# openfheorg/openfhe-boolean-circuit-evaluator

Hardware: AMD Instinct MI355X
Metric: encrypted gate-bootstraps/sec (whole node), AES-128 Bristol ckt STD128 GINX (higher is better)
Workload: dtype u32

## Files before the change

include/bce_gpu.h:

```cpp
#ifndef BCE_GPU_H
#define BCE_GPU_H

#include <stdint.h>

#ifdef __cplusplus
extern "C" {
#endif

typedef struct bce_ctx bce_ctx;

enum bce_paramset {
    BCE_TOY = 0, BCE_MEDIUM = 1, BCE_STD128_AP = 2, BCE_STD128_APOPT = 3, BCE_STD128 = 4,
    BCE_STD128_OPT = 5, BCE_STD192 = 6, BCE_STD192_OPT = 7, BCE_STD256 = 8, BCE_STD256_OPT = 9
};
enum bce_method { BCE_AP = 1, BCE_GINX = 2 };
enum bce_op {
    BCE_OR = 0, BCE_AND = 1, BCE_NOR = 2, BCE_NAND = 3, BCE_XOR_FAST = 4, BCE_XNOR_FAST = 5,
    BCE_OP_NOT = 16,
    BCE_OP_REFRESH = 17,
    BCE_OP_COPY = 18
};
enum bce_status {
    BCE_OK = 0, BCE_ERR_ARG = 1, BCE_ERR_NO_DEVICE = 2, BCE_ERR_HIP = 3, BCE_ERR_NO_KEYS = 4,
    BCE_ERR_POOL = 5, BCE_ERR_UNSUPPORTED = 6, BCE_ERR_STATE = 7
};
enum bce_encrypt_mode { BCE_FRESH = 0, BCE_BOOTSTRAPPED = 1 };

enum { BCE_P_n = 0, BCE_P_N, BCE_P_q, BCE_P_Q, BCE_P_qKS, BCE_P_baseKS, BCE_P_dKS, BCE_P_baseG, BCE_P_dG,
       BCE_P_baseR, BCE_P_dR, BCE_P_method, BCE_P_psi, BCE_P_COUNT };

typedef struct bce_gate_desc {
    uint32_t op;
    uint32_t in0;
    uint32_t in1;
    uint32_t out;
    uint32_t neg0;
    uint32_t neg1;
} bce_gate_desc;

#define BCE_PAIR(op, op2) ((uint32_t)(op) | (((uint32_t)(op2) + 1u) << 8))

enum bce_br_kernel {
    BCE_BR_WAVE_PER_TRANSFORM = 0,
    BCE_BR_SPLIT_X1 = 1,
    BCE_BR_SPLIT_X2 = 2,
    BCE_BR_WORD64 = 3,
    BCE_BR_DAG = 4,
    BCE_BR_GRAPH = 5,
    BCE_BR_KERNELS = 6
};

typedef struct bce_timing {
    double   blind_rotate_ms;
    double   tail_ms;
    uint64_t blind_rotate_launches;
    uint64_t bootstraps;
    double   br_ms[BCE_BR_KERNELS];
    uint64_t br_launches[BCE_BR_KERNELS];
    uint64_t br_bootstraps[BCE_BR_KERNELS];
    uint64_t fused_tail_launches;
} bce_timing;

int bce_ctx_create(int paramset, int method, int device, bce_ctx** out);
int bce_ctx_create_custom(uint32_t n, uint32_t N, uint64_t q, uint64_t Q, uint64_t qKS, uint32_t baseKS,
                          uint32_t baseG, uint32_t baseR, int method, int device, bce_ctx** out);
void bce_ctx_destroy(bce_ctx*);
const char* bce_last_error(const bce_ctx*);
int bce_get_params(const bce_ctx*, uint64_t out[BCE_P_COUNT]);

int bce_keygen(bce_ctx*, const uint8_t seed[32]);
int bce_import_keys(bce_ctx*, const int32_t* s, const int32_t* z, const uint64_t* bsk, uint64_t bsk_words,
                    const uint32_t* ksk, uint64_t ksk_words);
int bce_import_keys_eval(bce_ctx*, const int32_t* s, const int32_t* z, const uint64_t* bsk_eval, uint64_t bsk_words,
                         const uint32_t* ksk, uint64_t ksk_words);
int bce_export_bsk_eval(bce_ctx*, uint64_t* bsk_eval);
int bce_import_keys_file(bce_ctx*, const char* path);
int bce_export_keys_file(bce_ctx*, const char* path);
uint64_t bce_bsk_words(const bce_ctx*);
uint64_t bce_ksk_words(const bce_ctx*);
int bce_export_sk(const bce_ctx*, int32_t* s, int32_t* z);
int bce_export_bsk(bce_ctx*, uint64_t* bsk);
int bce_export_ksk(bce_ctx*, uint32_t* ksk);

int bce_pool_reserve(bce_ctx*, uint32_t slots);
uint32_t bce_pool_slots(const bce_ctx*);
int bce_lwe_write(bce_ctx*, const uint32_t* slots, uint32_t count, const uint64_t* cts);
int bce_lwe_read(bce_ctx*, const uint32_t* slots, uint32_t count, uint64_t* cts);

int bce_encrypt_bits(bce_ctx*, const uint8_t* bits, const uint32_t* slots, uint32_t count,
                     uint64_t enc_index_base, int mode);
int bce_set_encrypt_seed(bce_ctx*, const uint8_t seed[32]);
int bce_decrypt_bits(bce_ctx*, const uint32_t* slots, uint32_t count, uint8_t* bits);

int bce_eval_gates(bce_ctx*, uint32_t n_desc, const bce_gate_desc* descs);
int bce_eval_gates_strided(bce_ctx*, uint32_t n_desc, const bce_gate_desc* descs, uint32_t instances,
                           uint32_t slot_stride);
int bce_synchronize(bce_ctx*);

typedef struct bce_plan bce_plan;
int bce_plan_create(bce_ctx*, uint32_t n_steps, const uint32_t* step_sizes, const bce_gate_desc* descs,
                    uint32_t instances, uint32_t slot_stride, uint32_t slot_base, bce_plan** out);
int bce_plan_run_step(bce_ctx*, bce_plan*, uint32_t step);
int bce_plan_run(bce_ctx*, bce_plan*);
void bce_plan_destroy(bce_ctx*, bce_plan*);

enum { BCE_CHECK_LOG_CAP = 4096 };
typedef struct bce_check_report { uint64_t checked, mismatches, repaired; int64_t sum_err; uint64_t sum_sq_err;
                                  uint32_t max_abs_err, log_count; } bce_check_report;
typedef struct bce_check_entry  { uint32_t tag, index, instance, slot; int32_t err; uint8_t got, expect, pad[2]; } bce_check_entry;
int bce_check_slots(bce_ctx*, uint32_t count, const uint32_t* slots, const uint8_t* expect, uint32_t instances,
                    uint32_t slot_stride, int repair, uint32_t tag);
int bce_plan_set_checks(bce_ctx*, bce_plan*, const uint32_t* check_sizes , const uint32_t* slots, int repair);
int bce_plan_set_expected(bce_ctx*, bce_plan*, const uint8_t* expect);
int bce_check_reset(bce_ctx*);
int bce_check_get(bce_ctx*, bce_check_report*, bce_check_entry* log, uint32_t log_cap);

typedef struct bce_dag bce_dag;
int bce_dag_supported(const bce_ctx*);
int bce_dag_create(bce_ctx*, uint32_t n_tasks, const bce_gate_desc* tasks, const uint8_t* prio, bce_dag** out);
int bce_dag_run(bce_ctx*, bce_dag*, uint32_t instances, uint32_t slot_stride, uint32_t slot_base);
void bce_dag_destroy(bce_ctx*, bce_dag*);
int bce_dag_set_checks(bce_ctx*, bce_dag*, uint32_t n_checks, const uint32_t* tasks , int repair);
int bce_dag_set_expected(bce_ctx*, bce_dag*, uint32_t instances, const uint8_t* expect );
int bce_dag_set_limits(bce_ctx*, int workgroups_per_cu, int placement, uint32_t lazy_us, uint32_t stall_ms);
int bce_dag_last_run(bce_ctx*, uint64_t out[7]);
int bce_dag_debug_block_task(bce_dag*, uint32_t t);

int bce_timing_reset(bce_ctx*);
int bce_timing_get(bce_ctx*, bce_timing* out);
int bce_timing_set_events(bce_ctx*, int on);
uint64_t bce_bytes_per_bootstrap(const bce_ctx*);
int bce_bytes_per_bootstrap_parts(const bce_ctx*, uint64_t out[3]);
uint32_t bce_forward_transforms_per_step(const bce_ctx*);
uint32_t bce_forward_units(const bce_ctx*);
uint32_t bce_forward_mfma(const bce_ctx*);
uint32_t bce_lazy_arithmetic(const bce_ctx*);
int bce_forward_mfma_tables(uint64_t Q, uint32_t N, uint32_t gBits, uint32_t dG, uint64_t* psi, uint32_t* M6, uint32_t* C,
                            uint32_t* table, uint32_t* w14, uint64_t* bounds);
int bce_launch_capacity(const bce_ctx*, uint32_t* lone, uint32_t* full);

int bce_rccl_available(void);
int bce_rccl_version(void);
int bce_rccl_unique_id(uint8_t out[128]);
int bce_rccl_init(bce_ctx*, const uint8_t uid[128], int rank, int world);
int bce_rccl_allgather(bce_ctx*, const void* dev_send, void* dev_recv, uint64_t bytes);
int bce_rccl_shutdown(bce_ctx*);
int bce_rccl_comm_info(bce_ctx*, int out[3]);

int bce_debug_eval_stages(bce_ctx*, uint32_t n_desc, const bce_gate_desc* descs, uint64_t* acc,
                          uint64_t* lweN, uint64_t* ks);
int bce_debug_tail(bce_ctx*, uint32_t count, const uint64_t* acc, const uint32_t* out_slots, uint64_t* lweN,
                   uint64_t* ks);
int bce_debug_ntt(bce_ctx*, uint64_t* polys, uint32_t count, int inverse);

#ifdef __cplusplus
}
#endif
#endif
```

openfhe-boolean-circuit-evaluator_amd/__init__.py:

```python
import ctypes as C
import os

import numpy as np

from . import build as _build

_HERE = os.path.dirname(os.path.abspath(__file__))
LIB_PATH = os.path.join(_HERE, "libbce_amd.so")

TOY, MEDIUM, STD128_AP, STD128_APOPT, STD128, STD128_OPT, STD192, STD192_OPT, STD256, STD256_OPT = range(10)
AP, GINX = 1, 2
OR, AND, NOR, NAND, XOR_FAST, XNOR_FAST = range(6)
OP_NOT, OP_REFRESH, OP_COPY = 16, 17, 18


def PAIR(op, op2):
    return int(op) | ((int(op2) + 1) << 8)


FRESH, BOOTSTRAPPED = 0, 1
OK, ERR_ARG, ERR_NO_DEVICE, ERR_HIP, ERR_NO_KEYS, ERR_POOL, ERR_UNSUPPORTED, ERR_STATE = range(8)
P_NAMES = ["n", "N", "q", "Q", "qKS", "baseKS", "dKS", "baseG", "dG", "baseR", "dR", "method", "psi"]

PARAMSET_BY_NAME = {"TOY": TOY, "MEDIUM": MEDIUM, "STD128": STD128, "STD128_OPT": STD128_OPT,
                    "STD192": STD192, "STD192_OPT": STD192_OPT}
METHOD_BY_NAME = {"AP": AP, "GINX": GINX}


class BceError(RuntimeError):
    def __init__(self, code, msg):
        super().__init__("bce status %d: %s" % (code, msg))
        self.code = code


class GateDesc(C.Structure):
    _fields_ = [("op", C.c_uint32), ("in0", C.c_uint32), ("in1", C.c_uint32),
                ("out", C.c_uint32), ("neg0", C.c_uint32), ("neg1", C.c_uint32)]


BR_KERNEL_NAMES = ["k_blind_rotate (one wave per transform)", "k_blind_rotate_lat<4,2> (split transform, 1 workgroup/CU)",
                   "k_blind_rotate_lat<4,4> (split transform, 2 workgroups/CU)", "k_blind_rotate64 (64-bit modulus)",
                   "k_bootstrap_dag (persistent, dependency-driven, tail fused)",
                   "captured step schedule (bce_plan_run: one hipGraph launch, timed as one)"]
BR_KERNELS = len(BR_KERNEL_NAMES)


class Timing(C.Structure):
    _fields_ = [("blind_rotate_ms", C.c_double), ("tail_ms", C.c_double),
                ("blind_rotate_launches", C.c_uint64), ("bootstraps", C.c_uint64),
                ("br_ms", C.c_double * BR_KERNELS), ("br_launches", C.c_uint64 * BR_KERNELS), ("br_bootstraps", C.c_uint64 * BR_KERNELS),
                ("fused_tail_launches", C.c_uint64)]


class CheckReport(C.Structure):
    _fields_ = [("checked", C.c_uint64), ("mismatches", C.c_uint64), ("repaired", C.c_uint64), ("sum_err", C.c_int64),
                ("sum_sq_err", C.c_uint64), ("max_abs_err", C.c_uint32), ("log_count", C.c_uint32)]


class CheckEntry(C.Structure):
    _fields_ = [("tag", C.c_uint32), ("index", C.c_uint32), ("instance", C.c_uint32), ("slot", C.c_uint32),
                ("err", C.c_int32), ("got", C.c_uint8), ("expect", C.c_uint8), ("pad", C.c_uint8 * 2)]


CHECK_LOG_CAP = 4096


def _report_dict(r, q):
    d = {k: int(getattr(r, k)) for k, _ in CheckReport._fields_}
    d["noise_rms"] = (d["sum_sq_err"] / d["checked"]) ** 0.5 if d["checked"] else 0.0
    d["margin"] = q // 8 - d["max_abs_err"]
    return d


ENGINE_SYMBOLS = [
    "bce_ctx_create", "bce_ctx_create_custom", "bce_ctx_destroy", "bce_last_error", "bce_get_params",
    "bce_keygen", "bce_import_keys", "bce_import_keys_eval", "bce_export_bsk_eval", "bce_import_keys_file", "bce_export_keys_file", "bce_bsk_words", "bce_ksk_words", "bce_export_sk", "bce_export_bsk",
    "bce_export_ksk", "bce_pool_reserve", "bce_pool_slots", "bce_lwe_write", "bce_lwe_read",
    "bce_encrypt_bits", "bce_set_encrypt_seed", "bce_decrypt_bits", "bce_eval_gates", "bce_eval_gates_strided", "bce_synchronize",
    "bce_timing_reset", "bce_timing_get", "bce_timing_set_events", "bce_bytes_per_bootstrap", "bce_bytes_per_bootstrap_parts", "bce_forward_transforms_per_step", "bce_forward_units", "bce_forward_mfma", "bce_lazy_arithmetic", "bce_forward_mfma_tables", "bce_launch_capacity", "bce_rccl_available", "bce_rccl_version", "bce_rccl_unique_id", "bce_rccl_init", "bce_rccl_allgather", "bce_rccl_comm_info",
    "bce_rccl_shutdown", "bce_debug_eval_stages", "bce_debug_ntt", "bce_debug_tail",
    "bce_dag_supported", "bce_dag_create", "bce_dag_run", "bce_dag_destroy", "bce_dag_set_limits", "bce_dag_last_run", "bce_dag_debug_block_task",
    "bce_dag_set_checks", "bce_dag_set_expected",
    "bce_plan_create", "bce_plan_run_step", "bce_plan_run", "bce_plan_destroy",
    "bce_check_slots", "bce_plan_set_checks", "bce_plan_set_expected", "bce_check_reset", "bce_check_get",
]

_lib = None


def build(force=False):
    return _build.build(force=force)


def forward_mfma_tables(Q, N=1024, gBits=7, dG=4):
    import numpy as np
    L = lib()
    psi, w14, bounds = C.c_uint64(), (C.c_uint32 * 2)(), (C.c_uint64 * 4)()
    M6, Cw, tab = np.zeros((64, 64), np.uint32), np.zeros(64, np.uint32), np.zeros((4, 4, 64, 4), np.uint32)
    st = int(L.bce_forward_mfma_tables(int(Q), int(N), int(gBits), int(dG), C.byref(psi), M6.ctypes.data, Cw.ctypes.data, tab.ctypes.data,
                                       C.cast(w14, C.c_void_p), C.cast(bounds, C.c_void_p)))
    if st == 0:
        return 0, None
    return st, {"psi": int(psi.value), "M6": M6, "C": Cw, "table": tab, "w14": (int(w14[0]), int(w14[1])),
                "limb_sum_max": int(bounds[0]), "lo_max": int(bounds[1]), "hi_max": int(bounds[2]), "out_max": int(bounds[3])}


def lib():
    global _lib
    if _lib is not None:
        return _lib
    if not os.path.exists(LIB_PATH):
        raise ImportError("libbce_amd.so is not built: run `python -m openfhe-boolean-circuit-evaluator_amd.build` "
                          "or __graft_entry__.build(); there is no fallback path")
    L = C.CDLL(LIB_PATH)
    vp, u32, u64, i32 = C.c_void_p, C.c_uint32, C.c_uint64, C.c_int
    L.bce_ctx_create.argtypes = [i32, i32, i32, C.POINTER(vp)]
    L.bce_ctx_create_custom.argtypes = [u32, u32, u64, u64, u64, u32, u32, u32, i32, i32, C.POINTER(vp)]
    L.bce_ctx_destroy.argtypes = [vp]
    L.bce_ctx_destroy.restype = None
    L.bce_last_error.argtypes = [vp]
    L.bce_last_error.restype = C.c_char_p
    L.bce_get_params.argtypes = [vp, C.POINTER(u64)]
    L.bce_keygen.argtypes = [vp, C.c_char_p]
    L.bce_import_keys.argtypes = [vp, vp, vp, vp, u64, vp, u64]
    L.bce_import_keys_eval.argtypes = [vp, vp, vp, vp, u64, vp, u64]
    L.bce_export_bsk_eval.argtypes = [vp, vp]
    L.bce_import_keys_file.argtypes = [vp, C.c_char_p]
    L.bce_export_keys_file.argtypes = [vp, C.c_char_p]
    L.bce_bsk_words.argtypes = [vp]
    L.bce_bsk_words.restype = u64
    L.bce_ksk_words.argtypes = [vp]
    L.bce_ksk_words.restype = u64
    L.bce_export_sk.argtypes = [vp, vp, vp]
    L.bce_export_bsk.argtypes = [vp, vp]
    L.bce_export_ksk.argtypes = [vp, vp]
    L.bce_pool_reserve.argtypes = [vp, u32]
    L.bce_pool_slots.argtypes = [vp]
    L.bce_pool_slots.restype = u32
    L.bce_lwe_write.argtypes = [vp, vp, u32, vp]
    L.bce_lwe_read.argtypes = [vp, vp, u32, vp]
    L.bce_encrypt_bits.argtypes = [vp, vp, vp, u32, u64, i32]
    L.bce_set_encrypt_seed.argtypes = [vp, C.c_char_p]
    L.bce_decrypt_bits.argtypes = [vp, vp, u32, vp]
    L.bce_eval_gates.argtypes = [vp, u32, vp]
    L.bce_eval_gates_strided.argtypes = [vp, u32, vp, u32, u32]
    L.bce_synchronize.argtypes = [vp]
    L.bce_timing_reset.argtypes = [vp]
    L.bce_timing_get.argtypes = [vp, C.POINTER(Timing)]
    L.bce_timing_set_events.argtypes = [vp, i32]
    L.bce_bytes_per_bootstrap.argtypes = [vp]
    L.bce_bytes_per_bootstrap.restype = u64
    L.bce_bytes_per_bootstrap_parts.argtypes = [vp, C.POINTER(u64)]
    L.bce_forward_transforms_per_step.argtypes = [vp]
    L.bce_forward_transforms_per_step.restype = C.c_uint32
    L.bce_forward_units.argtypes = [vp]
    L.bce_forward_units.restype = C.c_uint32
    L.bce_forward_mfma.argtypes = [vp]
    L.bce_forward_mfma.restype = C.c_uint32
    L.bce_lazy_arithmetic.argtypes = [vp]
    L.bce_lazy_arithmetic.restype = C.c_uint32
    L.bce_forward_mfma_tables.argtypes = [u64, u32, u32, u32, vp, vp, vp, vp, vp, vp]
    L.bce_forward_mfma_tables.restype = i32
    L.bce_launch_capacity.argtypes = [vp, C.POINTER(C.c_uint32), C.POINTER(C.c_uint32)]
    L.bce_rccl_unique_id.argtypes = [C.c_char_p]
    L.bce_rccl_init.argtypes = [vp, C.c_char_p, i32, i32]
    L.bce_rccl_allgather.argtypes = [vp, vp, vp, u64]
    L.bce_rccl_shutdown.argtypes = [vp]
    L.bce_rccl_comm_info.argtypes = [vp, C.POINTER(C.c_int)]
    L.bce_debug_eval_stages.argtypes = [vp, u32, vp, vp, vp, vp]
    L.bce_debug_ntt.argtypes = [vp, vp, u32, i32]
    L.bce_debug_tail.argtypes = [vp, u32, vp, vp, vp, vp]
    L.bce_dag_supported.argtypes = [vp]
    L.bce_dag_create.argtypes = [vp, u32, vp, vp, C.POINTER(vp)]
    L.bce_dag_run.argtypes = [vp, vp, u32, u32, u32]
    L.bce_dag_destroy.argtypes = [vp, vp]
    L.bce_dag_destroy.restype = None
    L.bce_dag_set_limits.argtypes = [vp, i32, i32, u32, u32]
    L.bce_dag_last_run.argtypes = [vp, C.POINTER(u64)]
    L.bce_dag_debug_block_task.argtypes = [vp, u32]
    L.bce_dag_set_checks.argtypes = [vp, vp, u32, vp, i32]
    L.bce_dag_set_expected.argtypes = [vp, vp, u32, vp]
    L.bce_plan_create.argtypes = [vp, u32, vp, vp, u32, u32, u32, C.POINTER(vp)]
    L.bce_plan_run_step.argtypes = [vp, vp, u32]
    L.bce_plan_run.argtypes = [vp, vp]
    L.bce_plan_destroy.argtypes = [vp, vp]
    L.bce_plan_destroy.restype = None
    L.bce_check_slots.argtypes = [vp, u32, vp, vp, u32, u32, i32, u32]
    L.bce_plan_set_checks.argtypes = [vp, vp, vp, vp, i32]
    L.bce_plan_set_expected.argtypes = [vp, vp, vp]
    L.bce_check_reset.argtypes = [vp]
    L.bce_check_get.argtypes = [vp, C.POINTER(CheckReport), C.POINTER(CheckEntry), u32]
    _lib = L
    return L


def _p(a):
    return a.ctypes.data_as(C.c_void_p) if a is not None else None


def seed_bytes(seed):
    if isinstance(seed, (bytes, bytearray)):
        return bytes(seed).ljust(32, b"\0")[:32]
    return int(seed).to_bytes(32, "little")


def make_descs(descs):
    arr = (GateDesc * len(descs))()
    for i, d in enumerate(descs):
        d = tuple(d) + (0,) * (6 - len(d))
        arr[i] = GateDesc(*d)
    return arr


class BinFHEContext:

    def __init__(self, paramset=STD128_OPT, method=GINX, device=0, custom=None):
        self._L = lib()
        h = C.c_void_p()
        if custom is not None:
            rc = self._L.bce_ctx_create_custom(*custom, method, device, C.byref(h))
        else:
            rc = self._L.bce_ctx_create(paramset, method, device, C.byref(h))
        if rc != OK:
            raise BceError(rc, self._L.bce_last_error(None).decode())
        self.h = h
        buf = (C.c_uint64 * len(P_NAMES))()
        self._L.bce_get_params(self.h, buf)
        self.params = dict(zip(P_NAMES, [int(v) for v in buf]))
        self.n, self.N = self.params["n"], self.params["N"]

    def _ck(self, rc):
        if rc != OK:
            raise BceError(rc, self._L.bce_last_error(self.h).decode())

    def close(self):
        if getattr(self, "h", None):
            self._L.bce_ctx_destroy(self.h)
            self.h = None

    def __del__(self):
        try:
            self.close()
        except Exception:
            pass

    def KeyGen(self, seed=None):
        self._ck(self._L.bce_keygen(self.h, None if seed is None else seed_bytes(seed)))

    BTKeyGen = KeyGen

    def import_keys(self, s, z, bsk, ksk):
        s = np.ascontiguousarray(s, dtype=np.int32)
        z = np.ascontiguousarray(z, dtype=np.int32)
        bsk = np.ascontiguousarray(bsk, dtype=np.uint64)
        ksk = np.ascontiguousarray(ksk, dtype=np.uint32)
        self._ck(self._L.bce_import_keys(self.h, _p(s), _p(z), _p(bsk), bsk.size, _p(ksk), ksk.size))

    def import_keys_eval(self, s, z, bsk_eval, ksk):
        s = np.ascontiguousarray(s, dtype=np.int32)
        z = np.ascontiguousarray(z, dtype=np.int32)
        bsk = np.ascontiguousarray(bsk_eval, dtype=np.uint64)
        ksk = np.ascontiguousarray(ksk, dtype=np.uint32)
        self._ck(self._L.bce_import_keys_eval(self.h, _p(s), _p(z), _p(bsk), bsk.size, _p(ksk), ksk.size))

    def export_bsk_eval(self):
        out = np.zeros(self._L.bce_bsk_words(self.h), dtype=np.uint64)
        self._ck(self._L.bce_export_bsk_eval(self.h, _p(out)))
        return out

    def import_keys_file(self, path):
        self._ck(self._L.bce_import_keys_file(self.h, os.fsencode(path)))

    def export_keys_file(self, path):
        self._ck(self._L.bce_export_keys_file(self.h, os.fsencode(path)))

    def export_sk(self):
        s = np.zeros(self.n, dtype=np.int32)
        z = np.zeros(self.N, dtype=np.int32)
        self._ck(self._L.bce_export_sk(self.h, _p(s), _p(z)))
        return s, z

    def export_bsk(self):
        out = np.zeros(self._L.bce_bsk_words(self.h), dtype=np.uint64)
        self._ck(self._L.bce_export_bsk(self.h, _p(out)))
        return out

    def export_ksk(self):
        out = np.zeros(self._L.bce_ksk_words(self.h), dtype=np.uint32)
        self._ck(self._L.bce_export_ksk(self.h, _p(out)))
        return out

    def pool_reserve(self, slots):
        self._ck(self._L.bce_pool_reserve(self.h, int(slots)))

    def lwe_write(self, slots, cts):
        slots = np.ascontiguousarray(slots, dtype=np.uint32)
        cts = np.ascontiguousarray(cts, dtype=np.uint64)
        assert cts.size == slots.size * (self.n + 1)
        self._ck(self._L.bce_lwe_write(self.h, _p(slots), slots.size, _p(cts)))

    def lwe_read(self, slots):
        slots = np.ascontiguousarray(slots, dtype=np.uint32)
        out = np.zeros((slots.size, self.n + 1), dtype=np.uint64)
        self._ck(self._L.bce_lwe_read(self.h, _p(slots), slots.size, _p(out)))
        return out

    def set_encrypt_seed(self, seed):
        self._ck(self._L.bce_set_encrypt_seed(self.h, None if seed is None else seed_bytes(seed)))

    def Encrypt(self, bits, slots, enc_index_base=0, mode=FRESH):
        bits = np.ascontiguousarray(bits, dtype=np.uint8)
        slots = np.ascontiguousarray(slots, dtype=np.uint32)
        assert bits.size == slots.size
        self._ck(self._L.bce_encrypt_bits(self.h, _p(bits), _p(slots), slots.size, int(enc_index_base), mode))

# ... 25 lines not shown
    def timing_set_events(self, on):
        self._ck(self._L.bce_timing_set_events(self.h, int(bool(on))))

    def timing(self):
        t = Timing()
        self._ck(self._L.bce_timing_get(self.h, C.byref(t)))
        return {"blind_rotate_ms": t.blind_rotate_ms, "tail_ms": t.tail_ms,
                "blind_rotate_launches": int(t.blind_rotate_launches), "bootstraps": int(t.bootstraps),
                "fused_tail_launches": int(t.fused_tail_launches),
                "by_kernel": [{"kernel": BR_KERNEL_NAMES[k], "ms": t.br_ms[k], "launches": int(t.br_launches[k]),
                               "bootstraps": int(t.br_bootstraps[k])} for k in range(BR_KERNELS)]}

    def bytes_per_bootstrap(self):
        return int(self._L.bce_bytes_per_bootstrap(self.h))

    def dag_supported(self):
        return bool(self._L.bce_dag_supported(self.h))

    def dag_create(self, tasks, prio=None):
        arr = (GateDesc * len(tasks))()
        for i, t in enumerate(tasks):
            arr[i] = GateDesc(*(tuple(t) + (0, 0))[:6])
        pr = None
        if prio is not None:
            pr = (C.c_uint8 * len(tasks))(*[int(x) for x in prio])
        h = C.c_void_p()
        self._ck(self._L.bce_dag_create(self.h, len(tasks), arr, pr, C.byref(h)))
        return h

    def dag_run(self, dag, instances=1, slot_stride=0, slot_base=0):
        self._ck(self._L.bce_dag_run(self.h, dag, int(instances), int(slot_stride), int(slot_base)))

    def dag_destroy(self, dag):
        self._L.bce_dag_destroy(self.h, dag)

    def dag_set_limits(self, workgroups_per_cu=0, placement=1, lazy_us=20, stall_ms=4000):
        self._ck(self._L.bce_dag_set_limits(self.h, int(workgroups_per_cu), int(placement), int(lazy_us), int(stall_ms)))

    def dag_last_run(self):
        out = (C.c_uint64 * 7)()
        self._ck(self._L.bce_dag_last_run(self.h, out))
        d = {"done": int(out[0]), "lazy_waits": int(out[1]), "abort": int(out[2]), "workgroups_per_cu": int(out[3]),
             "busy_ticks": int(out[4]), "wait_ticks": int(out[5]), "gate_ticks": int(out[6])}
        if out[0]:
            d["ms_per_bootstrap"] = round(out[4] / out[0] / 1e5, 4)
            d["wait_ms_per_bootstrap"] = round(out[5] / out[0] / 1e5, 4)
            d["gate_ms_per_bootstrap"] = round(out[6] / out[0] / 1e5, 4)
        return d

    def plan_create(self, steps, instances=1, slot_stride=0, slot_base=0):
        flat = [t for st in steps for t in st]
        arr = (GateDesc * max(1, len(flat)))()
        for i, t in enumerate(flat):
            arr[i] = GateDesc(*(tuple(t) + (0, 0))[:6])
        sizes = (C.c_uint32 * max(1, len(steps)))(*[len(st) for st in steps])
        h = C.c_void_p()
        self._ck(self._L.bce_plan_create(self.h, len(steps), sizes, arr, int(instances), int(slot_stride), int(slot_base), C.byref(h)))
        return h

    def plan_run_step(self, plan, step):
        self._ck(self._L.bce_plan_run_step(self.h, plan, int(step)))

    def plan_run(self, plan):
        self._ck(self._L.bce_plan_run(self.h, plan))

    def plan_destroy(self, plan):
        self._L.bce_plan_destroy(self.h, plan)

    def check_slots(self, slots, expect, instances=1, slot_stride=0, repair=False, tag=0):
        slots = np.ascontiguousarray(slots, dtype=np.uint32)
        expect = np.ascontiguousarray(expect, dtype=np.uint8)
        assert expect.size == slots.size * int(instances)
        self._ck(self._L.bce_check_slots(self.h, slots.size, _p(slots), _p(expect), int(instances), int(slot_stride), int(bool(repair)), int(tag)))

    def plan_set_checks(self, plan, checks, repair=False):
        sizes = np.array([len(st) for st in checks], dtype=np.uint32)
        slots = np.array([s for st in checks for s in st] or [0], dtype=np.uint32)
        self._ck(self._L.bce_plan_set_checks(self.h, plan, _p(sizes), _p(slots), int(bool(repair))))

    def plan_set_expected(self, plan, expect):
        expect = np.ascontiguousarray(expect, dtype=np.uint8)
        self._ck(self._L.bce_plan_set_expected(self.h, plan, _p(expect)))

    def check_reset(self):
        self._ck(self._L.bce_check_reset(self.h))

    def check_get(self):
        r = CheckReport()
        log = (CheckEntry * CHECK_LOG_CAP)()
        self._ck(self._L.bce_check_get(self.h, C.byref(r), log, CHECK_LOG_CAP))
        keys = ("tag", "index", "instance", "slot", "err", "got", "expect")
        return _report_dict(r, self.params["q"]), [{k: int(getattr(log[i], k)) for k in keys} for i in range(r.log_count)]

    def dag_set_checks(self, dag, tasks, repair=False):
        tasks = np.ascontiguousarray(tasks, dtype=np.uint32).ravel()
        self._ck(self._L.bce_dag_set_checks(self.h, dag, tasks.size, _p(tasks) if tasks.size else None, int(bool(repair))))

    def dag_set_expected(self, dag, expect):
        expect = np.ascontiguousarray(expect, dtype=np.uint8)
        assert expect.ndim == 2
        self._ck(self._L.bce_dag_set_expected(self.h, dag, expect.shape[0], _p(expect)))

    def dag_debug_block_task(self, dag, t):
        self._ck(self._L.bce_dag_debug_block_task(dag, int(t)))

    @staticmethod
    def rccl_available():
        return bool(lib().bce_rccl_available())

    @staticmethod
    def rccl_unique_id():
        buf = C.create_string_buffer(128)
        rc = lib().bce_rccl_unique_id(buf)
        if rc != OK:
            raise BceError(rc, "RCCL is not available (bce_rccl_unique_id)")
        return buf.raw

    def rccl_init(self, uid, rank, world):
        self._ck(self._L.bce_rccl_init(self.h, bytes(uid), int(rank), int(world)))

    def rccl_comm_info(self):
        out = (C.c_int * 3)()
        self._ck(self._L.bce_rccl_comm_info(self.h, out))
        return {"ranks": int(out[0]), "rank": int(out[1]), "device": int(out[2])}

    def rccl_shutdown(self):
        self._ck(self._L.bce_rccl_shutdown(self.h))

    def rccl_allgather(self, dev_send_ptr, dev_recv_ptr, nbytes):
        self._ck(self._L.bce_rccl_allgather(self.h, C.c_void_p(dev_send_ptr), C.c_void_p(dev_recv_ptr), int(nbytes)))

    def bytes_per_bootstrap_parts(self):
        buf = (C.c_uint64 * 3)()
        self._ck(self._L.bce_bytes_per_bootstrap_parts(self.h, buf))
        return {"bsk": int(buf[0]), "ksk": int(buf[1]), "ct": int(buf[2])}

    def is64(self):
        return self.params["Q"] >= (1 << 28)

    def fp64(self):
        return self.is64() and self.params["Q"] < (1 << 39) and os.environ.get("BCE_FP64", "1")[:1] != "0"

    def bsk_word_bytes(self):
        return 8 if self.is64() else 4

    def forward_transforms_per_step(self):
        return int(self._L.bce_forward_transforms_per_step(self.h))

    def forward_units(self):
        return int(self._L.bce_forward_units(self.h))

    def forward_mfma(self):
        return int(self._L.bce_forward_mfma(self.h))

    def lazy_arithmetic(self):
        return int(self._L.bce_lazy_arithmetic(self.h))

    def launch_capacity(self):
        lone, full = C.c_uint32(), C.c_uint32()
        self._ck(self._L.bce_launch_capacity(self.h, C.byref(lone), C.byref(full)))
        return int(lone.value), int(full.value)

    def debug_eval_stages(self, descs):
        arr = make_descs(descs)
        nb = len(arr)
        rows = nb + sum(1 for d in arr if d.op >> 8)
        acc = np.zeros((nb, 2 * self.N), dtype=np.uint64)
        lweN = np.zeros((rows, self.N + 1), dtype=np.uint64)
        ks = np.zeros((rows, self.n + 1), dtype=np.uint64)
        self._ck(self._L.bce_debug_eval_stages(self.h, nb, arr, _p(acc), _p(lweN), _p(ks)))
        return acc, lweN, ks

    def debug_tail(self, acc, out_slots):
        acc = np.ascontiguousarray(acc, dtype=np.uint64).reshape(-1, 2 * self.N)
        slots = np.ascontiguousarray(out_slots, dtype=np.uint32)
        assert slots.size == acc.shape[0]
        lweN = np.zeros((slots.size, self.N + 1), dtype=np.uint64)
        ks = np.zeros((slots.size, self.n + 1), dtype=np.uint64)
        self._ck(self._L.bce_debug_tail(self.h, slots.size, _p(acc), _p(slots), _p(lweN), _p(ks)))
        return lweN, ks

    def debug_ntt(self, polys, inverse=False):
        polys = np.array(polys, dtype=np.uint64, order="C")
        count = polys.size // self.N
        self._ck(self._L.bce_debug_ntt(self.h, _p(polys), count, 1 if inverse else 0))
        return polys


class CircuitInfo(C.Structure):
    _fields_ = [("n_gates", C.c_uint32), ("n_input_gates", C.c_uint32), ("n_wires", C.c_uint32),
                ("n_inputs", C.c_uint32), ("n_input_bits", C.c_uint32 * 2), ("n_output_bits", C.c_uint32),
                ("n_levels", C.c_uint32), ("n_sublaunches", C.c_uint32), ("n_relevel_steps", C.c_uint32),
                ("max_frontier", C.c_uint32), ("slot_stride", C.c_uint32),
                ("n_bootstraps", C.c_uint64)]


class CircuitStats(C.Structure):
    _fields_ = [("total_ms", C.c_double), ("management_ms", C.c_double), ("execution_ms", C.c_double),
                ("bootstraps", C.c_uint64), ("levels", C.c_uint32), ("sublaunches", C.c_uint32),
                ("verify_fixes", C.c_uint32), ("exchanges", C.c_uint32), ("exchanged_cts", C.c_uint64)]


ALLGATHER_FN = C.CFUNCTYPE(C.c_int, C.c_void_p, C.c_uint64, C.c_int)

CIRCUIT_SYMBOLS = [
    "bce_circuit_create", "bce_circuit_destroy", "bce_circuit_last_error", "bce_circuit_read_file",
    "bce_circuit_read_bristol", "bce_circuit_get_info", "bce_circuit_reset", "bce_circuit_rearm", "bce_circuit_set_plaintext",
    "bce_circuit_set_encrypted", "bce_circuit_set_verify", "bce_circuit_get_flags", "bce_circuit_set_batched",
    "bce_circuit_set_encrypt_mode", "bce_circuit_get_encrypt_mode", "bce_circuit_plan_hash", "bce_circuit_set_shard_locality", "bce_circuit_set_xor_fast", "bce_circuit_set_xor_shared", "bce_circuit_xor_shared_active", "bce_circuit_set_relevel", "bce_circuit_get_relevel", "bce_circuit_set_dataflow", "bce_circuit_dataflow_active", "bce_circuit_set_graph", "bce_circuit_graph_active", "bce_circuit_set_device_verify", "bce_circuit_device_verify_active", "bce_circuit_get_check_report", "bce_circuit_dataflow_plan", "bce_circuit_set_balance", "bce_circuit_relevel_steps", "bce_circuit_relevel_descs", "bce_circuit_relevel_publications", "bce_circuit_check_relevel", "bce_circuit_set_instances", "bce_circuit_set_input", "bce_circuit_clock",
    "bce_circuit_get_output", "bce_circuit_get_buses", "bce_circuit_get_counts", "bce_circuit_get_stats", "bce_circuit_dump",
    "bce_circuit_set_exchange", "bce_circuit_enable_rccl", "bce_circuit_exchange_capacity", "bce_assemble_bristol", "bce_pool_gather",
    "bce_pool_scatter",
]

_circ_bound = False


def _bind_circuit():
    global _circ_bound
    L = lib()
    if _circ_bound:
        return L
    vp, u32, u64, i32 = C.c_void_p, C.c_uint32, C.c_uint64, C.c_int
    L.bce_circuit_create.argtypes = [vp, C.POINTER(vp)]
    L.bce_circuit_destroy.argtypes = [vp]
    L.bce_circuit_destroy.restype = None
    L.bce_circuit_last_error.argtypes = [vp]
    L.bce_circuit_last_error.restype = C.c_char_p
    L.bce_circuit_read_file.argtypes = [vp, C.c_char_p]
    L.bce_circuit_read_bristol.argtypes = [vp, C.c_char_p, i32]
    L.bce_circuit_get_info.argtypes = [vp, C.POINTER(CircuitInfo)]
    for name in ("reset", "rearm", "clock"):
        getattr(L, "bce_circuit_" + name).argtypes = [vp]
    for name in ("set_plaintext", "set_encrypted", "set_verify", "set_batched", "set_encrypt_mode", "set_xor_fast", "set_xor_shared", "set_relevel", "dump"):
        getattr(L, "bce_circuit_" + name).argtypes = [vp, i32]
    L.bce_circuit_get_flags.argtypes = [vp, C.POINTER(i32), C.POINTER(i32), C.POINTER(i32)]
    L.bce_circuit_set_instances.argtypes = [vp, u32]
    L.bce_circuit_set_balance.argtypes = [vp, i32, u32, u32]
    L.bce_circuit_set_dataflow.argtypes = [vp, i32]
    L.bce_circuit_set_graph.argtypes = [vp, i32]
    L.bce_circuit_graph_active.argtypes = [vp]
    L.bce_circuit_set_device_verify.argtypes = [vp, i32]
    L.bce_circuit_device_verify_active.argtypes = [vp]
    L.bce_circuit_get_check_report.argtypes = [vp, C.POINTER(CheckReport)]
    L.bce_circuit_get_encrypt_mode.argtypes = [vp]
    L.bce_circuit_get_relevel.argtypes = [vp]
    L.bce_circuit_set_shard_locality.argtypes = [vp, i32]
    L.bce_circuit_plan_hash.argtypes = [vp]
    L.bce_circuit_plan_hash.restype = u64
    L.bce_circuit_dataflow_active.argtypes = [vp]
    L.bce_circuit_xor_shared_active.argtypes = [vp]
    L.bce_circuit_dataflow_plan.argtypes = [vp, vp, vp, u32, C.POINTER(u32)]
    L.bce_circuit_relevel_steps.argtypes = [vp, C.POINTER(u32), u32, C.POINTER(u32)]
    L.bce_circuit_relevel_descs.argtypes = [vp, vp, u32, C.POINTER(u32)]
    L.bce_circuit_relevel_publications.argtypes = [vp, C.POINTER(u32), u32, C.POINTER(u32)]
    L.bce_circuit_check_relevel.argtypes = [vp]
    L.bce_circuit_set_input.argtypes = [vp, u32, vp, u32, vp]
    L.bce_circuit_get_output.argtypes = [vp, u32, vp]
    L.bce_circuit_get_buses.argtypes = [vp, C.POINTER(u32), C.POINTER(u32), u32, C.POINTER(u32), C.POINTER(u32), u32]
    L.bce_circuit_get_counts.argtypes = [vp, C.POINTER(u32 * 6)]
    L.bce_circuit_get_stats.argtypes = [vp, C.POINTER(CircuitStats)]
    L.bce_circuit_set_exchange.argtypes = [vp, u32, u32, i32, ALLGATHER_FN, vp, vp, vp, vp, vp, u64]
    L.bce_circuit_enable_rccl.argtypes = [vp, i32]
    L.bce_circuit_exchange_capacity.argtypes = [vp, u32, i32, i32]
    L.bce_circuit_exchange_capacity.restype = u64
    L.bce_assemble_bristol.argtypes = [C.c_char_p, i32, i32, i32, C.c_char_p, C.c_char_p, u32]
    L.bce_pool_gather.argtypes = [vp, vp, u32, vp]
    L.bce_pool_scatter.argtypes = [vp, vp, u32, vp]
    _circ_bound = True
    return L


def assemble_bristol(in_path, out_path=None, new_flag=False, gen_fan_flag=False, debug_flag=False):
    L = _bind_circuit()
    err = C.create_string_buffer(512)
    rc = L.bce_assemble_bristol(in_path.encode(), int(new_flag), int(gen_fan_flag), int(debug_flag),
                                out_path.encode() if out_path else None, err, 512)
    if rc != OK:
        raise BceError(rc, err.value.decode())


def HexStr2UintVec(inhex):
    out = []
    for ch in reversed(inhex):
        v = int(ch, 16)
        out.extend([(v >> b) & 1 for b in range(4)])
    return out


def BinStr2UintVec(inbin):
    return [int(ch) for ch in reversed(inbin)]


class Circuit:

    def __init__(self, cc=None):
        self._L = _bind_circuit()
        self.cc = cc
        h = C.c_void_p()
        rc = self._L.bce_circuit_create(cc.h if cc is not None else None, C.byref(h))
        if rc != OK:
            raise BceError(rc, "bce_circuit_create failed")
        self.h = h
        self._keep = []

    def _ck(self, rc):
# ... 215 lines not shown
```

openfhe-boolean-circuit-evaluator_amd/csrc/engine.cpp:

```cpp
#include <hip/hip_runtime_api.h>
#include <sys/random.h>

#include <algorithm>
#include <cstdarg>
#include <cstdio>
#include <cstdlib>
#include <cstring>
#include <memory>
#include <mutex>
#include <unordered_set>
#include <string>
#include <vector>

#include "../../include/bce_circuit.h"
#include "../../include/bce_gpu.h"
#include "devmem.hpp"
#include "fwd_mfma.hpp"
#include "host_math.hpp"
#include "kernels.hpp"
#include "keygen.hpp"
#include "prng.hpp"

using namespace bce;

static_assert(sizeof(bce_check_report) == 48 && sizeof(bce_check_entry) == 24, "layout of the check structs (include/bce_gpu.h; the kernel writes them)");

namespace {

thread_local std::string g_create_error;

struct ParamRow { u32 bits, cyclo, n; u64 q, qKS; u32 baseKS, baseG, baseR; };
const ParamRow kParamTable[] = {
    {27, 1024, 64, 512, 0, 25, 1u << 9, 23},
    {28, 2048, 422, 1024, 1u << 14, 1u << 7, 1u << 10, 32},
    {27, 2048, 512, 1024, 1u << 14, 1u << 7, 1u << 9, 32},
    {27, 2048, 502, 1024, 1u << 14, 1u << 7, 1u << 9, 32},
    {27, 2048, 512, 1024, 1u << 14, 1u << 7, 1u << 7, 32},
    {27, 2048, 502, 1024, 1u << 14, 1u << 7, 1u << 7, 32},
    {37, 4096, 1024, 1024, 1u << 19, 28, 1u << 13, 32},
    {37, 4096, 805, 1024, 1u << 15, 32, 1u << 13, 32},
    {29, 4096, 1024, 2048, 1u << 14, 1u << 7, 1u << 8, 46},
    {29, 4096, 990, 2048, 1u << 14, 1u << 7, 1u << 8, 46},
};

struct EventPair { hipEvent_t a, b; int kind; };

bool os_entropy(uint8_t out[32]) {
    size_t got = 0;
    while (got < 32) {
        const ssize_t r = getrandom(out + got, 32 - got, 0);
        if (r <= 0) break;
        got += (size_t)r;
    }
    if (got == 32) return true;
    FILE* f = std::fopen("/dev/urandom", "rb");
    if (!f) return false;
    const size_t n = std::fread(out, 1, 32, f);
    std::fclose(f);
    return n == 32;
}

}

struct bce_plan;
struct bce_dag;
namespace {
std::mutex g_live_mu;
std::unordered_set<const bce_ctx*> g_live;
}

struct bce_ctx {
    std::unordered_set<bce_plan*> plans;
    std::unordered_set<bce_dag*> dags;
    u32 n = 0, N = 0, logN = 0;
    u64 q = 0, Q = 0, qKS = 0, psi = 0;
    u32 baseKS = 0, dKS = 0, baseG = 0, gBits = 0, dG = 0, baseR = 0, dR = 0;
    int method = 0, device = 0;
    std::string err;

    hipStream_t stream = nullptr;
    DevParams P{};
    DevBuf<uint2> d_twf;
    DevBuf<u32> d_fwd_mfma, d_psi, d_psi_r2, d_xcd_gate;
    DevBuf<char> d_bsk;
    DevBuf<ulonglong2> d_tw64;
    DevBuf<double2> d_tw64d;
    bool is64 = false;
    size_t wbytes = 4;
    DevBuf<char> d_ksk;
    u64 bsk_polys = 0;
    bool have_keys = false;
    std::vector<int32_t> s, z;
    uint8_t seed[32] = {0};
    uint8_t enc_seed[32] = {0};
    bool enc_seed_ok = false, enc_deterministic = false;
    uint64_t enc_counter = 0;
    void* rccl_comm = nullptr;
    DevBuf<u32> d_pool;
    u32 pool_slots = 0;
    DevBuf<char> d_acc;
    DevBuf<u64> d_tail_partial;
    bool events_on = true;
    DevBuf<u32> d_io;
    DevBuf<u32, true> h_io;
    static constexpr int kRing = 4;
    StagedUpload ring[kRing];
    int ring_pos = 0;
    DevBuf<int8_t> d_s8;
    DevBuf<char> d_check_mem;
    bce_check_report* d_check() const { return reinterpret_cast<bce_check_report*>(d_check_mem.get()); }
    bce_check_entry* d_check_log() const { return reinterpret_cast<bce_check_entry*>(d_check_mem.get() + sizeof(bce_check_report)); }
    StagedUpload chk_stage;
    std::vector<EventPair> pending, free_events;
    bce_timing timing{};
    DevBuf<DevParams> d_P;
    int dag_wg_per_cu = 0, dag_placement = 1;
    uint32_t dag_lazy_us = 20, dag_stall_ms = 4000;
    struct DagStatus { uint32_t abort, done, lazy_waits, pad; uint64_t busy_ticks, wait_ticks, gate_ticks; };
    static constexpr int kDagRuns = 32;
    DevBuf<DagStatus, true> h_dag_status;
    struct DagStage { DevParams P; DagParams D; };
    DevBuf<DagStage, true> h_dag_stage;
    uint64_t dag_expected[kDagRuns] = {0};
    int dag_wps_used[kDagRuns] = {0};
    int dag_pending = 0;
    uint64_t dag_last[7] = {0, 0, 0, 0, 0, 0, 0};

    int fail(int code, const char* fmt, ...) {
        char buf[512];
        va_list ap;
        va_start(ap, fmt);
        vsnprintf(buf, sizeof buf, fmt, ap);
        va_end(ap);
        err = buf;
        return code;
    }
};

#define HIP_TRY(ctx, call)                                                                      \
    do {                                                                                        \
        hipError_t e_ = (call);                                                                 \
        if (e_ != hipSuccess) return (ctx)->fail(BCE_ERR_HIP, "%s: %s", #call, hipGetErrorString(e_)); \
    } while (0)

namespace {

bool env_off(const char* name) {
    const char* e = std::getenv(name);
    return e && e[0] == '0';
}

struct HostTables {
    std::vector<uint2> twf;
    std::vector<u32> psi, psi_r2;
    std::vector<ulonglong2> tw64;
    std::vector<double2> tw64d;
    FwdMfmaTables fwd;
    bool xcd_gate = false;
};

int derive_ctx(bce_ctx* c, u32 n, u32 N, u64 q, u64 Q, u64 qKS, u32 baseKS, u32 baseG, u32 baseR, int method, int device, u32 cu_count,
               HostTables& T) {
    c->n = n; c->N = N; c->q = q; c->Q = Q; c->qKS = qKS ? qKS : Q;
    c->baseKS = baseKS; c->baseG = baseG; c->baseR = baseR; c->method = method; c->device = device;
    while ((1u << c->logN) < N) ++c->logN;
    while ((1u << c->gBits) < baseG) ++c->gBits;
    c->dKS = digit_count((double)c->qKS, (double)baseKS);
    c->dG = digit_count((double)Q, (double)baseG);
    c->dR = digit_count((double)q, (double)baseR);
    c->is64 = Q >= (1ull << 28);
    c->wbytes = c->is64 ? 8 : 4;

    DevParams& P = c->P;
    P.n = n; P.N = N; P.logN = c->logN; P.q = (u32)q; P.Q = (u32)Q; P.qKS = (u32)c->qKS;
    P.baseKS = baseKS; P.dKS = c->dKS;
    P.ksk_stride = (n + 1 + 63) & ~63u;
    P.ksk_u16 = c->qKS <= 65536 ? 1 : 0;
    P.gBits = c->gBits; P.dG = c->dG; P.baseR = baseR; P.dR = c->dR;
    P.method_ap = method == BCE_AP ? 1 : 0;
    P.factor = (u32)(2 * N / q);
    P.factor_even = (P.factor & 1u) ? 0 : 1;
    P.Q8p1 = (u32)(Q / 8 + 1);
    int bq = bit_length(Q);
    P.red_shift = (u32)std::max(2 * bq + 3 - 32, 0);
    P.red_mu = c->is64 ? 0 : (u32)((((u128)1) << (32 + P.red_shift)) / Q);
    u64 ninv = pow_mod(N, Q - 2, Q);
    P.Ninv = (u32)ninv;
    P.Ninv_s = c->is64 ? 0 : (u32)(((u128)ninv << 32) / Q);
    P.mu32 = (u32)((((u64)1) << 32) / Q);
    P.c32 = (u32)((((u64)1) << 32) % Q);
    {
        const u128 B = 2 * c->logN + 2, R = 2 * c->dG;
        const u128 sum = R * B * Q * Q;
        const bool ok1 = B * Q < ((u128)1 << 32);
        const bool ok2 = sum < ((u128)1 << 64);
        const u128 folded = (sum >> 32) * P.c32 + ((u128)1 << 32);
        const bool ok3 = folded < ((u128)1 << (32 + P.red_shift));
        const bool ok4 = (u128)6 * Q * Q + 2 * Q < ((u128)1 << (32 + P.red_shift)) && (u128)3 * Q < ((u128)1 << 32);
        const u128 rmax = (sum >> 32) + 1 + Q, ymax = 2 * rmax * 2 * Q;
        const bool ok5 = ymax < ((u128)1 << 64) && (ymax >> 32) + 1 + Q <= 2 * (u128)Q && (u128)4 * Q < ((u128)1 << 32);
        P.lazy = (c->is64 || (ok1 && ok2 && ok3 && ok4 && ok5)) ? 1 : 0;
    }
    P.is64 = c->is64 ? 1 : 0;
    P.Q64 = Q;
    {
        const char* var = std::getenv("BCE_VARIANT");
        P.variant = var ? (u32)std::atoi(var) : 0;
        P.cu_count = cu_count;
        P.fuse_tail = env_off("BCE_FUSE_TAIL") ? 0 : 1;
    }
    const char* occ = std::getenv("BCE_OCCUPANCY");
    P.occupancy_target = (occ && occ[0] == '2') ? 2 : 3;
    P.fp64 = (c->is64 && Q < (1ull << 39) && !env_off("BCE_FP64")) ? 1 : 0;
    const KernelClass kc = kernel_class(P);
    P.occupancy_target = kc.occupancy_target;
    P.fp64 = kc.fp64;
    if (kc.error) { g_create_error = kc.error; return BCE_ERR_UNSUPPORTED; }
    if (c->qKS > 0xFFFFFFFFull) { g_create_error = "qKS must fit 32 bits"; return BCE_ERR_UNSUPPORTED; }
    c->psi = min_primitive_root(Q, 2ull * N);

    T.twf.resize(N);
    T.psi.resize(N);
    u64 p = 1;
    for (u32 i = 0; i < N; ++i) {
        T.psi[i] = c->is64 ? 0 : (u32)p;
        u32 r = bit_reverse(i, (int)c->logN);
        u32 pos = r;
        if (r >= 64) {
            const u32 s = 31u - (u32)__builtin_clz(r), sh = s - 6, ii = r - (1u << s);
            pos = (1u << s) + ((ii & ((1u << sh) - 1u)) << 6) + (ii >> sh);
        }
        T.twf[pos] = c->is64 ? make_uint2(0, 0) : make_uint2((u32)p, (u32)(((u128)p << 32) / Q));
        p = mul_mod(p, c->psi, Q);
    }
    const u64 r2modq = c->is64 ? 0 : (u64)((((u128)1) << 64) % Q);
    T.psi_r2.resize(N);
    for (u32 i = 0; i < N; ++i) T.psi_r2[i] = c->is64 ? 0 : (u32)mul_mod(T.psi[i], r2modq, Q);
    {
        const u64 ch = (((u64)1) << 32) / c->qKS;
        if (ch < 8) { g_create_error = "qKS too large for the key-switch gather (needs qKS <= 2^29)"; return BCE_ERR_ARG; }
        P.ks_chunk = (u32)std::min<u64>(ch & ~(u64)7, 1u << 20);
    }
    if (!c->is64) {
        u32 inv = (u32)Q;
        for (int i = 0; i < 5; ++i) inv *= 2u - (u32)Q * inv;
        P.qinv_neg = 0u - inv;
        P.r2_off = (u32)(Q - r2modq);
    }
    {
        u64 I = pow_mod(c->psi, N / 2, Q), v = 1;
        for (int k = 0; k < 4; ++k) {
            P.I4[k] = (u32)v;
            P.I4s[k] = c->is64 ? 0 : (u32)(((u128)v << 32) / Q);
            v = mul_mod(v, I, Q);
        }
        const u64 wl = mul_mod(P.I4[3], ninv, Q);
        P.Winv_last = (u32)wl;
        P.Winv_last_s = c->is64 ? 0 : (u32)(((u128)wl << 32) / Q);
    }
    P.xcd_gate_ticks = 10000;
    T.xcd_gate = !c->is64 && !env_off("BCE_XCD_GATE");
    if (const char* t = std::getenv("BCE_XCD_GATE_US"); t && T.xcd_gate) P.xcd_gate_ticks = (u32)std::atoi(t) * 100u;
    P.Q8p1_64 = Q / 8 + 1;
    P.mu64 = (u64)((((u128)1) << 64) / Q);
    P.c64 = (u64)((((u128)1) << 64) % Q);
    P.Ninv64 = ninv;
    P.Ninv64_s = (u64)(((u128)ninv << 64) / Q);
    if (c->is64) {
        T.tw64.resize(N);
        u64 pw = 1;
        for (u32 i = 0; i < N; ++i) {
            T.tw64[bit_reverse(i, (int)c->logN)] = make_ulonglong2(pw, (u64)(((u128)pw << 64) / Q));
            pw = mul_mod(pw, c->psi, Q);
        }
        if (kc.lds_error) { g_create_error = kc.lds_error; return BCE_ERR_UNSUPPORTED; }
        P.Qd = (double)Q;
        P.invQd = 1.0 / (double)Q;
        P.Ninvd = (double)ninv;
        P.Ninvd_q = (double)ninv / (double)Q;
        T.tw64d.resize(N);
        for (u32 i = 0; i < N; ++i) T.tw64d[i] = make_double2((double)T.tw64[i].x, (double)T.tw64[i].x / (double)Q);
    }
    {
        const u128 Bg = (u128)1 << c->gBits;
        u128 span = 0, pw = 1;
        for (u32 l = 0; l < c->dG; ++l) { span += pw; pw *= Bg; }
        const u128 hi = (Bg / 2 - 1) * span, lo = (Bg / 2) * span;
        const bool exact = (u128)(Q >> 1) <= hi + 1 && (u128)(Q - (Q >> 1)) <= lo;
        const bool product_exact = kc.family != KernelFamily::Fp64 || (Bg / 2) * (u128)Q < ((u128)1 << 53);
        P.fold = (exact && kc.fold_build && product_exact && !env_off("BCE_FOLD")) ? 1 : 0;
        P.fold_ninv = (P.fold && kc.family == KernelFamily::Fp64) ? 1 : 0;
        P.fwd_units = (P.fold && !c->is64 && c->method == BCE_GINX && P.factor_even && !env_off("BCE_FWD_UNITS")) ? 1 : 0;
        P.fwd_mfma = 0; P.w14 = P.w14s = 0;
        if (P.fwd_units && !env_off("BCE_FWD_MFMA")) {
            T.fwd = build_fwd_mfma_tables(Q, N, c->gBits, c->dG, c->psi);
            if (T.fwd.ok) { P.fwd_mfma = 1; P.w14 = T.fwd.w14; P.w14s = T.fwd.w14s; }
        }
    }
    P.pool_stride = n + 1;
    return BCE_OK;
}

template <class T>
hipError_t upload_vector(DevBuf<T>& dst, const std::vector<T>& v) {
    const hipError_t e = dst.alloc(std::max<size_t>(1, v.size()));
    return e != hipSuccess ? e : hipMemcpy(dst.get(), v.data(), v.size() * sizeof(T), hipMemcpyHostToDevice);
}

int upload_ctx(bce_ctx* c, const HostTables& T) {
    DevParams& P = c->P;
    if (hipSetDevice(c->device) != hipSuccess) { g_create_error = "hipSetDevice failed"; return BCE_ERR_HIP; }
    if (hipStreamCreateWithFlags(&c->stream, hipStreamNonBlocking) != hipSuccess) { g_create_error = "hipStreamCreate failed"; return BCE_ERR_HIP; }
    const auto up = [](auto& dst, const auto& v, const char* what) -> bool {
        if (upload_vector(dst, v) == hipSuccess) return true;
        g_create_error = std::string("hipMalloc(") + what + ") failed";
        return false;
    };
    if (!up(c->d_twf, T.twf, "twiddles") || !up(c->d_psi, T.psi, "psi table") || !up(c->d_psi_r2, T.psi_r2, "psi table")) return BCE_ERR_HIP;
    P.tw_f = c->d_twf.get();
    P.psi_tab = c->d_psi.get();
    P.psi_tab_r2 = c->d_psi_r2.get();
    P.xcd_gate = nullptr;
    if (T.xcd_gate) {
        if (c->d_xcd_gate.alloc(16 * 32) != hipSuccess) { g_create_error = "hipMalloc(xcd gate) failed"; return BCE_ERR_HIP; }
        P.xcd_gate = c->d_xcd_gate.get();
    }
    if (c->is64) {
        if (!up(c->d_tw64, T.tw64, "twiddles64") || !up(c->d_tw64d, T.tw64d, "twiddles64d")) return BCE_ERR_HIP;
        P.tw64 = c->d_tw64.get();
        P.tw64d = c->d_tw64d.get();
    }
    P.fwd_mfma_tab = nullptr;
    if (P.fwd_mfma) {
        if (!up(c->d_fwd_mfma, T.fwd.table, "forward matrix table")) return BCE_ERR_HIP;
        P.fwd_mfma_tab = c->d_fwd_mfma.get();
    }
    c->enc_seed_ok = os_entropy(c->enc_seed);
    return BCE_OK;
}

int build_ctx(u32 n, u32 N, u64 q, u64 Q, u64 qKS, u32 baseKS, u32 baseG, u32 baseR, int method, int device,
              bce_ctx** out) {
    if (!out) return BCE_ERR_ARG;
    *out = nullptr;
    if (method != BCE_AP && method != BCE_GINX) { g_create_error = "bad method (expect AP=1 or GINX=2)"; return BCE_ERR_ARG; }
    if (N < 512 || N > 2048 || (N & (N - 1))) { g_create_error = "ring dimension N must be 512, 1024 or 2048"; return BCE_ERR_UNSUPPORTED; }
    if ((q & (q - 1)) || q > 2 * (u64)N || q < 8) { g_create_error = "LWE modulus q must be a power of two dividing 2N"; return BCE_ERR_ARG; }
    if (!is_prime_u64(Q) || (Q - 1) % (2ull * N)) { g_create_error = "Q must be a prime = 1 mod 2N"; return BCE_ERR_ARG; }
    if (Q >= (1ull << 40)) { g_create_error = "ring modulus Q must be below 2^40"; return BCE_ERR_UNSUPPORTED; }
    if (baseG & (baseG - 1)) { g_create_error = "gadget base must be a power of two"; return BCE_ERR_ARG; }
    int ndev = 0;
    if (hipGetDeviceCount(&ndev) != hipSuccess || ndev <= 0) {
        g_create_error = "no HIP device visible: the engine has no CPU fallback";
        return BCE_ERR_NO_DEVICE;
    }
    if (device < 0 || device >= ndev) { g_create_error = "bad device ordinal"; return BCE_ERR_ARG; }
    int cus = 0;
    if (hipDeviceGetAttribute(&cus, hipDeviceAttributeMultiprocessorCount, device) != hipSuccess || cus <= 0) cus = 256;

    struct CtxDeleter { void operator()(bce_ctx* p) const { bce_ctx_destroy(p); } };
    std::unique_ptr<bce_ctx, CtxDeleter> c(new bce_ctx);
    { std::lock_guard<std::mutex> lk(g_live_mu); g_live.insert(c.get()); }
    HostTables T;
    int rc = derive_ctx(c.get(), n, N, q, Q, qKS, baseKS, baseG, baseR, method, device, (u32)cus, T);
    if (rc == BCE_OK) rc = upload_ctx(c.get(), T);
    if (rc != BCE_OK) return rc;
    *out = c.release();
    return BCE_OK;
}

u64 rgsw_rows_total(const bce_ctx* c);
int bsk_words_to_kernel_layout(bce_ctx* c) {
    if (c->P.fold) HIP_TRY(c, launch_fold_gadget(c->P, c->d_bsk.get(), rgsw_rows_total(c) / (2ull * c->dG), +1, c->stream));
    if (!c->P.fp64) { HIP_TRY(c, hipStreamSynchronize(c->stream)); return BCE_OK; }
    HIP_TRY(c, launch_words_u64_f64(reinterpret_cast<u64*>(c->d_bsk.get()), (size_t)c->bsk_polys * c->N, 1, c->stream));
    HIP_TRY(c, hipStreamSynchronize(c->stream));
    return BCE_OK;
}

u64 rgsw_rows_total(const bce_ctx* c) {
    const u64 R = 2ull * c->dG;
    return c->method == BCE_GINX ? (u64)c->n * 2 * R : (u64)c->n * c->baseR * c->dR * R;
}

int alloc_keys(bce_ctx* c) {
    if (!c->d_bsk.get()) {
        c->bsk_polys = rgsw_rows_total(c) * 2;
        HIP_TRY(c, c->d_bsk.alloc(c->wbytes * c->bsk_polys * c->N));
    }
    if (!c->d_ksk.get()) {
        size_t rows = (size_t)c->N * c->baseKS * c->dKS;
        HIP_TRY(c, c->d_ksk.alloc(rows * c->P.ksk_stride * (c->P.ksk_u16 ? 2 : 4)));
    }
    c->P.bsk = reinterpret_cast<const u32*>(c->d_bsk.get());
    c->P.bsk64 = reinterpret_cast<const u64*>(c->d_bsk.get());
    c->P.ksk = c->d_ksk.get();
    return BCE_OK;
}

int upload_ksk(bce_ctx* c, const u32* ksk) {
    const size_t rows = (size_t)c->N * c->baseKS * c->dKS, W = c->n + 1, S = c->P.ksk_stride;
    if (c->P.ksk_u16) {
        std::vector<uint16_t> buf(rows * S, 0);
        for (size_t r = 0; r < rows; ++r)
            for (size_t k = 0; k < W; ++k) buf[r * S + k] = (uint16_t)ksk[r * W + k];
        HIP_TRY(c, hipMemcpy(c->d_ksk.get(), buf.data(), buf.size() * 2, hipMemcpyHostToDevice));
    } else {
        std::vector<u32> buf(rows * S, 0);
        for (size_t r = 0; r < rows; ++r) std::memcpy(&buf[r * S], &ksk[r * W], W * 4);
        HIP_TRY(c, hipMemcpy(c->d_ksk.get(), buf.data(), buf.size() * 4, hipMemcpyHostToDevice));
    }
    return BCE_OK;
}

int upload_secret(bce_ctx* c) {
    const size_t padded = ((size_t)c->n + 63) / 64 * 64;
    std::vector<int8_t> s8(padded, 0);
    for (u32 k = 0; k < c->n; ++k) s8[k] = (int8_t)c->s[k];
    if (!c->d_s8.get()) HIP_TRY(c, c->d_s8.alloc(padded));
    HIP_TRY(c, hipStreamSynchronize(c->stream));
    HIP_TRY(c, hipMemcpy(c->d_s8.get(), s8.data(), padded, hipMemcpyHostToDevice));
    return BCE_OK;
}

int ensure_check(bce_ctx* c) {
    if (c->d_check_mem.get()) return BCE_OK;
    const size_t bytes = sizeof(bce_check_report) + (size_t)kCheckLogCap * sizeof(bce_check_entry);
    DevBuf<char> mem;
    HIP_TRY(c, mem.alloc(bytes));
    if (hipMemset(mem.get(), 0, bytes) != hipSuccess) return c->fail(BCE_ERR_HIP, "hipMemset(check report) failed");
    c->d_check_mem = std::move(mem);
    return BCE_OK;
}

int ensure_acc(bce_ctx* c, size_t boots) {
    const size_t need = boots * 2 * c->N * c->wbytes;
    HIP_TRY(c, c->d_acc.grow(need, std::max(need, 2 * c->d_acc.capacity()), c->stream));
    return BCE_OK;
}

int stage_descs(bce_ctx* c, const bce_gate_desc* d, size_t n, StagedUpload** slot) {
    StagedUpload& r = c->ring[c->ring_pos];
    c->ring_pos = (c->ring_pos + 1) % bce_ctx::kRing;
    const size_t bytes = n * sizeof(bce_gate_desc);
    HIP_TRY(c, r.reserve(bytes, std::max(n, (size_t)1024) * sizeof(bce_gate_desc), nullptr));
    std::memcpy(r.host(), d, bytes);
    HIP_TRY(c, r.copy(bytes, c->stream));
    *slot = &r;
    return BCE_OK;
}
const bce_gate_desc* descs_of(const StagedUpload* slot) { return static_cast<const bce_gate_desc*>(slot->device()); }

EventPair get_events(bce_ctx* c, int kind) {
    EventPair p;
    if (!c->free_events.empty()) {
        p = c->free_events.back();
        c->free_events.pop_back();
    } else {
        hipEventCreate(&p.a);
        hipEventCreate(&p.b);
    }
    p.kind = kind;
    return p;
}

void drain_timing(bce_ctx* c) {
    for (auto& p : c->pending) {
        float ms = 0.f;
        if (hipEventElapsedTime(&ms, p.a, p.b) == hipSuccess) {
            if (p.kind < BCE_BR_KERNELS) { c->timing.blind_rotate_ms += ms; c->timing.br_ms[p.kind] += ms; }
            else c->timing.tail_ms += ms;
        }
        c->free_events.push_back(p);
    }
    c->pending.clear();
}
int drain_if_long(bce_ctx* c) {
    if (c->pending.size() <= 4096) return BCE_OK;
    HIP_TRY(c, hipStreamSynchronize(c->stream));
    drain_timing(c);
    return BCE_OK;
}

int words_to_device(bce_ctx* c, void* dev, const u64* src, size_t words, bool wide) {
    if (wide) {
        HIP_TRY(c, hipMemcpy(dev, src, words * 8, hipMemcpyHostToDevice));
    } else {
        const std::vector<u32> tmp(src, src + words);
// ... 955 lines not shown
        if (two) { p1[i] = writer[g.in1]; read_before[g.in1] = 1; }
        if (p1[i] == p0[i]) p1[i] = -1;
        if (writer[g.out] >= 0) return c->fail(BCE_ERR_ARG, "bce_dag_create: slot %u is written by tasks %d and %u (SSA form required)", g.out, writer[g.out], i);
        if (read_before[g.out]) return c->fail(BCE_ERR_ARG, "bce_dag_create: task %u writes slot %u that an earlier task (or itself) reads", i, g.out);
        writer[g.out] = (int32_t)i;
        for (int32_t p : {p0[i], p1[i]})
            if (p >= 0) { ++dep[i]; ++cons_cnt[p + 1]; lvl[i] = std::max(lvl[i], lvl[p] + 1); }
        depth = std::max(depth, lvl[i]);
    }
    std::vector<u32> cons_off(cons_cnt);
    for (u32 i = 0; i < n_tasks; ++i) cons_off[i + 1] += cons_off[i];
    std::vector<u32> cons(std::max<u32>(1, cons_off[n_tasks])), fill(cons_off.begin(), cons_off.end() - 1);
    for (u32 i = 0; i < n_tasks; ++i)
        for (int32_t p : {p0[i], p1[i]}) if (p >= 0) cons[fill[p]++] = i;
    std::vector<uint8_t> qid(n_tasks, 0);
    if (prio) qid.assign(prio, prio + n_tasks);

    struct Deleter { bce_ctx* c; void operator()(bce_dag* g) const { bce_dag_destroy(c, g); } };
    std::unique_ptr<bce_dag, Deleter> g(new bce_dag, Deleter{c});
    { std::lock_guard<std::mutex> lk(g_live_mu); c->dags.insert(g.get()); }
    g->n_tasks = n_tasks; g->max_slot = max_slot; g->depth = depth; g->h_dep_init = dep;
    for (u32 q = 0; q < kDagQueues; ++q) {
        g->init_off[q] = (u32)g->init_items.size();
        for (u32 i = 0; i < n_tasks; ++i) {
            if (qid[i] != q) continue;
            ++g->qcount[q];
            if (dep[i] == 0) g->init_items.push_back(i);
        }
    }
    g->init_off[kDagQueues] = (u32)g->init_items.size();
    if (g->init_items.empty()) return c->fail(BCE_ERR_ARG, "bce_dag_create: no task is ready at the start");
    HIP_TRY(c, g->d_tasks.alloc(n_tasks));
    HIP_TRY(c, hipMemcpy(g->d_tasks.get(), tasks, (size_t)n_tasks * sizeof(bce_gate_desc), hipMemcpyHostToDevice));
    HIP_TRY(c, upload_vector(g->d_cons_off, cons_off));
    HIP_TRY(c, upload_vector(g->d_cons, cons));
    HIP_TRY(c, upload_vector(g->d_dep_init, dep));
    HIP_TRY(c, upload_vector(g->d_init, g->init_items));
    HIP_TRY(c, upload_vector(g->d_qid, qid));
    HIP_TRY(c, g->d_ctl.alloc(kDagCtlWords));
    HIP_TRY(c, g->d_params.alloc(1));
    *out = g.release();
    return BCE_OK;
}

int bce_dag_debug_block_task(bce_dag* g, uint32_t t) {
    if (!g || t >= g->n_tasks) return BCE_ERR_ARG;
    g->h_dep_init[t] += 1;
    return hipMemcpy(g->d_dep_init.get(), g->h_dep_init.data(), (size_t)g->n_tasks * sizeof(u32), hipMemcpyHostToDevice) == hipSuccess ? BCE_OK : BCE_ERR_HIP;
}

int bce_dag_run(bce_ctx* c, bce_dag* g, uint32_t instances, uint32_t slot_stride, uint32_t slot_base) {
    if (!c || !g) return BCE_ERR_ARG;
    if (instances == 0) return BCE_OK;
    if (!c->have_keys) return c->fail(BCE_ERR_NO_KEYS, "bce_keygen / bce_import_keys has not been called");
    if (g->n_checks && g->expect_instances == 0) return c->fail(BCE_ERR_STATE, "bce_dag_run: the DAG has checks but bce_dag_set_expected has not been called");
    if (g->n_checks && g->expect_instances != instances) return c->fail(BCE_ERR_STATE, "bce_dag_run: %u instances, but the expected bits were set for %u", instances, g->expect_instances);
    if (instances > 1 && slot_stride <= g->max_slot) return c->fail(BCE_ERR_ARG, "bce_dag_run: slot_stride %u does not cover the DAG's slots (0..%u)", slot_stride, g->max_slot);
    if ((u64)slot_base + g->max_slot + (u64)(instances - 1) * slot_stride >= c->pool_slots) return c->fail(BCE_ERR_POOL, "bce_dag_run: slot %llu outside the pool (%u slots)", (unsigned long long)((u64)slot_base + g->max_slot + (u64)(instances - 1) * slot_stride), c->pool_slots);
    const u64 items = (u64)g->n_tasks * instances;
    if (items >= 0xFFFFFFF0ull) return c->fail(BCE_ERR_ARG, "bce_dag_run: %llu bootstraps exceed one run's 32-bit item space", (unsigned long long)items);
    HIP_TRY(c, hipSetDevice(c->device));
    if (c->dag_pending >= bce_ctx::kDagRuns) { const int rc = sync_stream(c); if (rc) return rc; }
    if (!c->d_P.get()) HIP_TRY(c, c->d_P.alloc(1));
    if (!c->h_dag_status.get()) HIP_TRY(c, c->h_dag_status.alloc(bce_ctx::kDagRuns));
    if (!c->h_dag_stage.get()) HIP_TRY(c, c->h_dag_stage.alloc(bce_ctx::kDagRuns));
    HIP_TRY(c, g->d_dep.grow(items, items, c->stream));
    DagParams D{};
    for (u32 q = 0; q < kDagQueues; ++q) {
        const size_t need = (size_t)g->qcount[q] * instances;
        HIP_TRY(c, g->d_slots[q].grow(need, need, c->stream));
        D.slots[q] = g->d_slots[q].get();
        D.qcap[q] = (u32)need;
        D.init_off[q] = g->init_off[q];
    }
    D.init_off[kDagQueues] = g->init_off[kDagQueues];
    D.tasks = g->d_tasks.get(); D.cons_off = g->d_cons_off.get(); D.cons = g->d_cons.get(); D.qid = g->d_qid.get(); D.dep_init = g->d_dep_init.get();
    D.dep = g->d_dep.get(); D.init_items = g->d_init.get(); D.ctl = g->d_ctl.get();
    D.n_tasks = g->n_tasks; D.instances = instances; D.slot_stride = slot_stride; D.slot_base = slot_base;
    if (g->n_checks) {
        if (const int rc = ensure_check(c)) return rc;
        D.chk_of_task = g->d_chk_of_task.get(); D.expect = static_cast<const uint8_t*>(g->expect.device()); D.n_checks = g->n_checks; D.repair = (u32)g->chk_repair;
        D.s8 = c->d_s8.get(); D.report = c->d_check(); D.log = c->d_check_log();
    }
    D.lazy_ticks = c->dag_lazy_us * 100u;
    D.stall_ticks = c->dag_stall_ms * 100000u;
    D.policy = c->dag_placement ? 1u : 0u;
    D.gate_ticks = 15000;
    D.gate_backlog = 8;
    if (const char* e = std::getenv("BCE_DAG_GATE_US")) D.gate_ticks = (u32)std::atoi(e) * 100u;
    if (const char* e = std::getenv("BCE_DAG_GATE_BACKLOG")) D.gate_backlog = (u32)std::atoi(e);
    int wps = c->dag_wg_per_cu == 1 ? 2 : 4;
    if (c->dag_wg_per_cu == 0) {
        const double D = (double)std::max<u32>(1, g->depth), W = (double)items, cus = (double)std::max<u32>(1, c->P.cu_count);
        const double t1 = std::max(D, W / cus), t2 = std::max(1.6 * D, W / (1.26 * cus));
        wps = t1 <= t2 ? 2 : 4;
    }
    if (const char* e = std::getenv("BCE_DAG_WPS")) { if (e[0] == '2') wps = 2; else if (e[0] == '4') wps = 4; }
    if (kernel_class(c->P).wg_per_cu_full == 1) wps = 2;
    if (const char* e = std::getenv("BCE_DAG_PLACE")) D.policy = e[0] == '0' ? 0u : 1u;
    const char* dbg = std::getenv("BCE_DAG_DEBUG");
    if (dbg && dbg[0] == 'd') D.policy |= 2u;
    { const char* e = std::getenv("BCE_DAG_GATE"); if (e ? e[0] != '0' : wps == 4) D.policy |= 4u; }
    { const char* e = std::getenv("BCE_DAG_TICKETS"); if (e && e[0] == '1') D.policy |= 8u; }
    const u32 grid = c->P.cu_count * (wps == 2 ? 1u : 2u);
    const int slot = c->dag_pending++;
    bce_ctx::DagStage& stage = c->h_dag_stage.get()[slot];
    stage.P = c->P;
    stage.D = D;
    HIP_TRY(c, hipMemcpyAsync(c->d_P.get(), &stage.P, sizeof(DevParams), hipMemcpyHostToDevice, c->stream));
    HIP_TRY(c, hipMemcpyAsync(g->d_params.get(), &stage.D, sizeof(DagParams), hipMemcpyHostToDevice, c->stream));
    HIP_TRY(c, launch_dag_rearm(D, c->stream));
    EventPair e0 = get_events(c, BCE_BR_DAG);
    hipEventRecord(e0.a, c->stream);
    if (!(dbg && dbg[0] == 'r')) HIP_TRY(c, launch_bootstrap_dag(c->P, c->d_P.get(), g->d_params.get(), wps, grid, c->stream));
    hipEventRecord(e0.b, c->stream);
    c->pending.push_back(e0);
    c->dag_expected[slot] = items;
    c->dag_wps_used[slot] = wps;
    HIP_TRY(c, hipMemcpyAsync(&c->h_dag_status.get()[slot], g->d_ctl.get() + kDagAbort, sizeof(bce_ctx::DagStatus), hipMemcpyDeviceToHost, c->stream));
    c->timing.br_launches[BCE_BR_DAG] += 1;
    c->timing.br_bootstraps[BCE_BR_DAG] += items;
    c->timing.blind_rotate_launches += 1;
    c->timing.fused_tail_launches += 1;
    c->timing.bootstraps += items;
    return BCE_OK;
}

int bce_timing_reset(bce_ctx* c) {
    if (!c) return BCE_ERR_ARG;
    HIP_TRY(c, hipStreamSynchronize(c->stream));
    drain_timing(c);
    c->timing = bce_timing{};
    return BCE_OK;
}

int bce_timing_set_events(bce_ctx* c, int on) {
    if (!c) return BCE_ERR_ARG;
    c->events_on = on != 0;
    return BCE_OK;
}

int bce_timing_get(bce_ctx* c, bce_timing* out) {
    if (!c || !out) return BCE_ERR_ARG;
    const int rc = sync_stream(c);
    drain_timing(c);
    *out = c->timing;
    return rc;
}

uint32_t bce_forward_transforms_per_step(const bce_ctx* c) { return c ? 2 * c->dG - (c->P.fold ? 2 : 0) : 0; }
uint32_t bce_forward_units(const bce_ctx* c) { return c ? c->P.fwd_units : 0; }
uint32_t bce_forward_mfma(const bce_ctx* c) { return c ? c->P.fwd_mfma : 0; }
uint32_t bce_lazy_arithmetic(const bce_ctx* c) { return c ? c->P.lazy : 0; }
int bce_forward_mfma_tables(uint64_t Q, uint32_t N, uint32_t gBits, uint32_t dG, uint64_t* psi, uint32_t* M6, uint32_t* C, uint32_t* table,
                            uint32_t* w14, uint64_t* bounds) {
    const FwdMfmaTables T = build_fwd_mfma_tables(Q, N, gBits, dG);
    if (T.M6.empty()) return 0;
    if (psi) *psi = T.psi;
    if (M6) std::copy(T.M6.begin(), T.M6.end(), M6);
    if (C) std::copy(T.C.begin(), T.C.end(), C);
    if (table) std::copy(T.table.begin(), T.table.end(), table);
    if (w14) { w14[0] = T.w14; w14[1] = T.w14s; }
    if (bounds) { bounds[0] = T.limb_sum_max; bounds[1] = T.lo_max; bounds[2] = T.hi_max; bounds[3] = T.out_max; }
    return T.ok ? 1 : -1;
}

int bce_launch_capacity(const bce_ctx* c, uint32_t* lone, uint32_t* full) {
    if (!c || !lone || !full) return BCE_ERR_ARG;
    const KernelClass k = kernel_class(c->P);
    *lone = c->P.cu_count * k.wg_per_cu_lone;
    *full = c->P.cu_count * k.wg_per_cu_full;
    return BCE_OK;
}

int bce_bytes_per_bootstrap_parts(const bce_ctx* c, uint64_t out[3]) {
    if (!c || !out) return BCE_ERR_ARG;
    const double rgsws = c->method == BCE_AP ? (double)c->n * c->dR * (c->baseR - 1) / c->baseR : 2.0 * c->n;
    out[0] = (u64)((double)c->wbytes * rgsws * (2 * c->dG) * 2 * c->N);
    out[1] = (c->P.ksk_u16 ? 2ull : 4ull) * c->N * c->dKS * (c->n + 1);
    out[2] = 4ull * 3 * (c->n + 1);
    return BCE_OK;
}

uint64_t bce_bytes_per_bootstrap(const bce_ctx* c) {
    uint64_t parts[3];
    return bce_bytes_per_bootstrap_parts(c, parts) == BCE_OK ? parts[0] + parts[1] + parts[2] : 0;
}

int bce_debug_eval_stages(bce_ctx* c, uint32_t n_desc, const bce_gate_desc* descs, uint64_t* acc, uint64_t* lweN,
                          uint64_t* ks) {
    if (!c) return BCE_ERR_ARG;
    for (u32 i = 0; i < n_desc; ++i)
        if (!(pair_kind(descs[i].op) > 0 || descs[i].op <= BCE_XNOR_FAST || descs[i].op == BCE_OP_REFRESH)) return c->fail(BCE_ERR_ARG, "staged outputs need bootstrapped ops only");
    return eval_impl(c, n_desc, descs, 1, 0, acc, lweN, ks);
}

int bce_debug_tail(bce_ctx* c, uint32_t count, const uint64_t* acc, const uint32_t* out_slots, uint64_t* lweN, uint64_t* ks) {
    if (!c || !acc || !out_slots) return BCE_ERR_ARG;
    if (count == 0) return BCE_OK;
    if (!c->have_keys) return c->fail(BCE_ERR_NO_KEYS, "bce_keygen / bce_import_keys has not been called");
    HIP_TRY(c, hipSetDevice(c->device));
    const size_t words = (size_t)count * 2 * c->N;
    for (size_t i = 0; i < words; ++i)
        if (acc[i] >= c->Q) return c->fail(BCE_ERR_ARG, "accumulator word not reduced mod Q");
    std::vector<bce_gate_desc> d(count);
    for (u32 i = 0; i < count; ++i) {
        if (out_slots[i] >= c->pool_slots) return c->fail(BCE_ERR_POOL, "slot %u outside the pool", out_slots[i]);
        d[i] = bce_gate_desc{BCE_AND, out_slots[i], out_slots[i], out_slots[i], 0, 0};
    }
    DevBuf<char> d_in;
    DevBuf<u32> d_lweN, d_ks;
    DevBuf<u64> d_partial;
    HIP_TRY(c, d_in.alloc(words * c->wbytes));
    HIP_TRY(c, d_lweN.alloc((size_t)count * (c->N + 1)));
    HIP_TRY(c, d_ks.alloc((size_t)count * (c->n + 1)));
    HIP_TRY(c, d_partial.alloc(std::max<size_t>(1, tail_partial_words(c->P, count))));
    int rc = words_to_device(c, d_in.get(), acc, words, c->is64);
    if (rc) return rc;
    StagedUpload* slot = nullptr;
    if ((rc = stage_descs(c, d.data(), count, &slot))) return rc;
    HIP_TRY(c, launch_tail(c->P, descs_of(slot), count, 1, 0, d_in.get(), d_partial.get(), d_lweN.get(), d_ks.get(), c->stream, LaunchEvents{}));
    slot->mark(c->stream);
    HIP_TRY(c, hipStreamSynchronize(c->stream));
    if (lweN && (rc = words_from_device(c, lweN, d_lweN.get(), (size_t)count * (c->N + 1), false))) return rc;
    if (ks && (rc = words_from_device(c, ks, d_ks.get(), (size_t)count * (c->n + 1), false))) return rc;
    return BCE_OK;
}

static int pool_pack(bce_ctx* c, const uint32_t* slots, uint32_t count, void* dev, int to_pool) {
    if (!c || !slots || !dev) return BCE_ERR_ARG;
    if (count == 0) return BCE_OK;
    HIP_TRY(c, hipSetDevice(c->device));
    std::vector<bce_gate_desc> d(count);
    for (u32 i = 0; i < count; ++i) {
        if (slots[i] >= c->pool_slots) return c->fail(BCE_ERR_POOL, "slot %u outside the pool", slots[i]);
        d[i] = bce_gate_desc{BCE_OP_COPY, slots[i], slots[i], slots[i], 0, 0};
    }
    StagedUpload* slot = nullptr;
    int rc = stage_descs(c, d.data(), count, &slot);
    if (rc) return rc;
    HIP_TRY(c, launch_pool_pack(c->P, descs_of(slot), count, (u32*)dev, to_pool, c->stream));
    slot->mark(c->stream);
    return BCE_OK;
}

int bce_pool_gather(bce_ctx* c, const uint32_t* slots, uint32_t count, void* dev_dst) {
    return pool_pack(c, slots, count, dev_dst, 0);
}
int bce_pool_scatter(bce_ctx* c, const uint32_t* slots, uint32_t count, const void* dev_src) {
    return pool_pack(c, slots, count, const_cast<void*>(dev_src), 1);
}

int bce_debug_ntt(bce_ctx* c, uint64_t* polys, uint32_t count, int inverse) {
    if (!c || !polys) return BCE_ERR_ARG;
    HIP_TRY(c, hipSetDevice(c->device));
    const size_t words = (size_t)count * c->N;
    for (size_t i = 0; i < words; ++i)
        if (polys[i] >= c->Q) return c->fail(BCE_ERR_ARG, "poly word not reduced mod Q");
    DevBuf<char> d;
    HIP_TRY(c, d.alloc(words * c->wbytes));
    int rc = words_to_device(c, d.get(), polys, words, c->is64);
    if (!rc) rc = dev_ntt(c, d.get(), count, inverse);
    if (rc) return rc;
    HIP_TRY(c, hipStreamSynchronize(c->stream));
    return words_from_device(c, polys, d.get(), words, c->is64);
}

}
```

openfhe-boolean-circuit-evaluator_amd/csrc/fwd_mfma.hpp:

```cpp
#pragma once
#include <cstdint>
#include <vector>

#include "host_math.hpp"

namespace bce {

constexpr u32 kFwdMfmaLoads = 4;
constexpr u32 kFwdMfmaTableWords = 4 * kFwdMfmaLoads * 64 * 4;

inline u32 fwd_mfma_h_of_k(u32 k) { return (k >> 2) + 16u * (k & 3u); }

struct FwdMfmaTables {
    bool ok = false;
    u64 psi = 0;
    std::vector<u32> M6;
    std::vector<u32> C;
    std::vector<u32> table;
    u32 w14 = 0, w14s = 0;
    u64 limb_sum_max = 0;
    u64 lo_max = 0, hi_max = 0, out_max = 0;
};

inline FwdMfmaTables build_fwd_mfma_tables(u64 Q, u32 N, u32 gBits, u32 dG, u64 psi = 0) {
    FwdMfmaTables T;
    if (N != 1024 || dG != 4 || gBits == 0 || gBits > 7 || Q >= (1ull << 28) || Q < 3 || (Q - 1) % (2ull * N) != 0) return T;
    T.psi = psi ? psi : min_primitive_root(Q, 2ull * N);
    if (pow_mod(T.psi, N, Q) != Q - 1) return T;
    std::vector<u64> tw(64, 0);
    for (u32 i = 0; i < 64; ++i) tw[i] = pow_mod(T.psi, bit_reverse(i, 10), Q);
    T.M6.assign(64 * 64, 0);
    for (u32 e = 0; e < 64; ++e) {
        u64 x[64] = {0};
        x[e] = 1;
        for (int B = 5; B >= 0; --B) {
            const u32 m = 1u << (5 - B);
            for (u32 h = 0; h < 64; ++h) {
                if (h & (1u << B)) continue;
                const u64 w = tw[m + (h >> (B + 1))];
                const u64 X = x[h], Tm = mul_mod(x[h | (1u << B)], w, Q);
                x[h] = (X + Tm) % Q;
                x[h | (1u << B)] = (X + Q - Tm) % Q;
            }
        }
        for (u32 h = 0; h < 64; ++h) T.M6[h * 64 + e] = (u32)x[h];
    }
    T.C.assign(64, 0);
    for (u32 hp = 0; hp < 64; ++hp) {
        u64 s = 0;
        for (u32 h = 0; h < 64; ++h) s = (s + T.M6[hp * 64 + h]) % Q;
        T.C[hp] = (u32)((Q - mul_mod(s, 1ull << (gBits - 1), Q)) % Q);
    }
    const u64 w14 = (1ull << 14) % Q;
    T.w14 = (u32)w14;
    T.w14s = (u32)(((u128)w14 << 32) / Q);
    T.limb_sum_max = 64ull * 127ull * (1ull << (gBits - 1));
    T.hi_max = Q + 129ull * T.limb_sum_max;
    T.lo_max = T.hi_max;
    T.out_max = 2 * Q + T.lo_max;
    T.ok = T.limb_sum_max < (1ull << 31) && 129ull * T.limb_sum_max < Q && T.lo_max < (1ull << 32) && T.out_max <= 13 * Q;
    T.table.assign(kFwdMfmaTableWords, 0);
    for (u32 q = 0; q < 4; ++q)
        for (u32 l = 0; l < 64; ++l) {
            for (u32 v = 0; v < 4; ++v) {
                const u32 hp = 16 * q + 4 * v + ((l & 15u) >> 2), limb = l & 3u;
                for (u32 b = 0; b < 16; ++b) {
                    const u32 byte = (T.M6[hp * 64 + fwd_mfma_h_of_k(16 * (l >> 4) + b)] >> (7 * limb)) & 127u;
                    T.table[((q * kFwdMfmaLoads + v) * 64 + l) * 4 + (b >> 2)] |= byte << (8 * (b & 3u));
                }
            }
        }
    return T;
}

}
```

openfhe-boolean-circuit-evaluator_amd/csrc/kernels.hip:

```cpp
#include <hip/hip_runtime.h>

#include <algorithm>
#include <iterator>
#include <utility>

#include "kernels.hpp"

namespace bce {

#include "phase_prof.hpp"
#include "fused_tail.hpp"
#include "dag_sched.hpp"
#ifdef BCE_PHASE_PROF
__device__ unsigned long long g_phase_prof[BCE_PROF_WAVES * BCE_PROF_SLOTS];
#define BCE_PROF_ARRAY ::bce::g_phase_prof
#endif

__device__ __forceinline__ u32 csub(u32 x, u32 m) { return min(x, x - m); }

__device__ __forceinline__ u32 mul_shoup_lazy(u32 y, uint2 w, u32 Q) {
    u32 qh = __umulhi(w.y, y);
    return w.x * y - qh * Q;
}

__device__ __forceinline__ u64 mad64(u32 a, u32 b, u64 c) {
    u64 r, carry;
    asm("v_mad_u64_u32 %0, %1, %2, %3, %4" : "=v"(r), "=s"(carry) : "v"(a), "v"(b), "v"(c));
    return r;
}
__device__ __forceinline__ u64 mul64(u32 a, u32 b) {
    u64 r, carry;
    asm("v_mad_u64_u32 %0, %1, %2, %3, 0" : "=v"(r), "=s"(carry) : "v"(a), "v"(b));
    return r;
}
__device__ __forceinline__ u32 mul_shoup_lazy3(u32 y, uint2 w, u32 Q) {
    return (u32)mad64(__umulhi(w.y, y), 0u - Q, mul64(y, w.x));
}
__device__ __forceinline__ u64 pair_of(u32 lo) {
    u64 p;
    asm volatile("" : "=v"(p));
    return (p & 0xFFFFFFFF00000000ull) | lo;
}
__device__ __forceinline__ u64 with_lo(u64 pair, u32 lo) { return (pair & 0xFFFFFFFF00000000ull) | lo; }

__device__ __forceinline__ u32 barrett_lazy3(u64 x, u32 Q, u32 shift, u32 mu) {
    return (u32)mad64(__umulhi((u32)(x >> shift), mu), 0u - Q, x);
}

__device__ __forceinline__ u32 barrett_reduce(u64 x, u32 Q, u32 shift, u32 mu) {
    u32 x1 = (u32)(x >> shift);
    u32 qh = __umulhi(x1, mu);
    u32 r = (u32)x - qh * Q;
    r = csub(r, 2 * Q);
    return csub(r, Q);
}

__device__ __forceinline__ u32 barrett_fold(u64 x, u32 c32, u32 Q, u32 shift, u32 mu) {
    return barrett_reduce((u64)(u32)(x >> 32) * c32 + (u32)x, Q, shift, mu);
}

__device__ __forceinline__ u32 phys(u32 j) { return j + ((j >> 6) << 2); }

template <int LOGN>
struct Cfg {
    static constexpr int N = 1 << LOGN;
    static constexpr int LE = LOGN - 6;
    static constexpr int E = 1 << LE;
    static constexpr int NP = N + (N >> 6) * 4;
    static constexpr int F2LO = (6 > LE) ? 6 - LE : 0;
    static_assert(LOGN >= 9 && LOGN <= 11, "supported ring sizes: 512, 1024, 2048");
};

template <u32 M>
__device__ __forceinline__ u32 tw_pos(u32 i) {
    if constexpr (M < 64) {
        return M + i;
    } else {
        constexpr u32 sh = __builtin_ctz(M) - 6;
        return M + ((i & ((1u << sh) - 1u)) << 6) + (i >> sh);
    }
}

__device__ __forceinline__ void block_sync_lds() {
    asm volatile("s_waitcnt lgkmcnt(0)\n\ts_barrier" ::: "memory");
}

__device__ __forceinline__ void wave_sync() {
    __builtin_amdgcn_fence(__ATOMIC_RELEASE, "wavefront");
    __builtin_amdgcn_wave_barrier();
    __builtin_amdgcn_fence(__ATOMIC_ACQUIRE, "wavefront");
}

template <int LOGN, int LO>
__device__ __forceinline__ u32 elem_j(u32 lane, int r) {
    constexpr int LE = Cfg<LOGN>::LE;
    u32 lane_lo = lane & ((1u << LO) - 1u);
    u32 lane_hi = lane >> LO;
    return (lane_hi << (LO + LE)) | ((u32)r << LO) | lane_lo;
}

template <int LOGN, int LO>
__device__ __forceinline__ void load_pass(const u32* poly, u32 lane, u32 (&x)[Cfg<LOGN>::E]) {
    constexpr int E = Cfg<LOGN>::E;
    if constexpr (LO == 0) {
        const uint4* p = reinterpret_cast<const uint4*>(poly + phys(lane * E));
#pragma unroll
        for (int k = 0; k < E / 4; ++k) {
            uint4 v = p[k];
            x[4 * k] = v.x; x[4 * k + 1] = v.y; x[4 * k + 2] = v.z; x[4 * k + 3] = v.w;
        }
    } else {
#pragma unroll
        for (int r = 0; r < E; ++r) x[r] = poly[phys(elem_j<LOGN, LO>(lane, r))];
    }
}

template <int LOGN, int LO>
__device__ __forceinline__ void store_pass(u32* poly, u32 lane, const u32 (&x)[Cfg<LOGN>::E]) {
    constexpr int E = Cfg<LOGN>::E;
    if constexpr (LO == 0) {
        uint4* p = reinterpret_cast<uint4*>(poly + phys(lane * E));
#pragma unroll
        for (int k = 0; k < E / 4; ++k) p[k] = make_uint4(x[4 * k], x[4 * k + 1], x[4 * k + 2], x[4 * k + 3]);
    } else {
#pragma unroll
        for (int r = 0; r < E; ++r) poly[phys(elem_j<LOGN, LO>(lane, r))] = x[r];
    }
}

template <int LOGN, int LO, int B, bool LAZY>
__device__ __forceinline__ void fwd_stage(u32 (&x)[Cfg<LOGN>::E], u32 lane, const uint2* tw, u32 Q) {
    constexpr int LE = Cfg<LOGN>::LE, E = Cfg<LOGN>::E;
    constexpr int rb = B - LO;
    constexpr u32 m = 1u << (LOGN - 1 - B);
    const u32 hi = (lane >> LO) << (LO + LE - B - 1);
    const u32 Q2 = 2 * Q;
#pragma unroll
    for (int r = 0; r < E; ++r) {
        if (r & (1 << rb)) continue;
        uint2 w = tw[tw_pos<m>(hi | (u32)(r >> (rb + 1)))];
        u32 X = LAZY ? x[r] : csub(x[r], Q2);
        u32 T = mul_shoup_lazy(x[r | (1 << rb)], w, Q);
        x[r] = X + T;
        x[r | (1 << rb)] = X + Q2 - T;
    }
}

template <int LOGN, int LO, int B>
__device__ __forceinline__ void fwd_stage_pair(u64 (&x)[Cfg<LOGN>::E], u32 lane, const uint2* tw, u32 Q) {
    constexpr int LE = Cfg<LOGN>::LE, E = Cfg<LOGN>::E;
    constexpr int rb = B - LO;
    constexpr u32 m = 1u << (LOGN - 1 - B);
    const u32 hi = (lane >> LO) << (LO + LE - B - 1);
    const u32 Q2 = 2 * Q, negQ = 0u - Q;
#pragma unroll
    for (int r = 0; r < E; ++r) {
        if (r & (1 << rb)) continue;
        const uint2 w = tw[tw_pos<m>(hi | (u32)(r >> (rb + 1)))];
        const u32 X = (u32)x[r], Y = (u32)x[r | (1 << rb)];
        const u64 t = mad64(__umulhi(Y, w.y), negQ, mad64(Y, w.x, x[r]));
        x[r | (1 << rb)] = with_lo(x[r | (1 << rb)], (X << 1) + Q2 - (u32)t);
        x[r] = t;
    }
}
template <int LOGN>
__device__ __forceinline__ void fwd_first_stage_pair(const u32 (&x)[Cfg<LOGN>::E], u64 (&xp)[Cfg<LOGN>::E], uint2 w, u32 Q) {
    constexpr int E = Cfg<LOGN>::E, Hh = E / 2;
    const u32 Q2 = 2 * Q, negQ = 0u - Q;
#pragma unroll
    for (int r = 0; r < Hh; ++r) {
        const u32 X = x[r], Y = x[r + Hh];
        const u64 t = mad64(__umulhi(Y, w.y), negQ, mad64(Y, w.x, pair_of(X)));
        xp[r] = t;
        xp[r + Hh] = pair_of((X << 1) + Q2 - (u32)t);
    }
}
template <int LOGN, int LO, int BHI, int BLO>
__device__ __forceinline__ void fwd_stages_pair(u64 (&x)[Cfg<LOGN>::E], u32 lane, const uint2* tw, u32 Q) {
    if constexpr (BHI >= BLO) {
        fwd_stage_pair<LOGN, LO, BHI>(x, lane, tw, Q);
        fwd_stages_pair<LOGN, LO, BHI - 1, BLO>(x, lane, tw, Q);
    }
}
template <int LOGN, int LO>
__device__ __forceinline__ void load_pass_pair(const u32* poly, u32 lane, u64 (&x)[Cfg<LOGN>::E]) {
#pragma unroll
    for (int r = 0; r < Cfg<LOGN>::E; ++r) x[r] = pair_of(poly[phys(elem_j<LOGN, LO>(lane, r))]);
}
__device__ __forceinline__ u32 lm_word(u32 lane, int k) { return (u32)k * 256u + lane * 4u; }
template <int LOGN>
__device__ __forceinline__ void load_lm(const u32* poly, u32 lane, u32 (&x)[Cfg<LOGN>::E]) {
#pragma unroll
    for (int k = 0; k < Cfg<LOGN>::E / 4; ++k) {
        const uint4 v = *reinterpret_cast<const uint4*>(poly + lm_word(lane, k));
        x[4 * k] = v.x; x[4 * k + 1] = v.y; x[4 * k + 2] = v.z; x[4 * k + 3] = v.w;
    }
}
template <int LOGN, int LO>
__device__ __forceinline__ void store_pass_pair(u32* poly, u32 lane, const u64 (&x)[Cfg<LOGN>::E]) {
#pragma unroll
    for (int r = 0; r < Cfg<LOGN>::E; ++r) poly[phys(elem_j<LOGN, LO>(lane, r))] = (u32)x[r];
}

constexpr int GS_CAP = 16;
constexpr int gs_bound(int r, int rb0, int rb) {
    int b = 2;
    for (int s = rb0; s < rb; ++s) {
        if ((r >> s) & 1) b = 2;
        else b = (2 * b > GS_CAP) ? b : 2 * b;
    }
    return b;
}

template <int LOGN, int LO, int B, int RB0, bool LAST, int R>
__device__ __forceinline__ void inv_bfly(u32 (&x)[Cfg<LOGN>::E], u32 hi, const uint2* tw, u32 Q, uint2 ninv, uint2 wlast) {
    constexpr int rb = B - LO;
    if constexpr ((R & (1 << rb)) == 0) {
        constexpr u32 m = 1u << (LOGN - 1 - B);
        constexpr int S = R | (1 << rb);
        constexpr int b0 = gs_bound(R, RB0, rb);
        constexpr bool cap = 2 * b0 > GS_CAP;
        constexpr u32 b = cap ? b0 / 2 : b0;
        u32 X = x[R], Y = x[S];
        if constexpr (cap) { X = csub(X, b * Q); Y = csub(Y, b * Q); }
        if constexpr (LAST) {
            x[R] = csub(mul_shoup_lazy3(X + Y, ninv, Q), Q);
            x[S] = csub(mul_shoup_lazy3(X + b * Q - Y, wlast, Q), Q);
        } else {
            const uint2 f = tw[tw_pos<m>((m - 1) - (hi | (u32)(R >> (rb + 1))))];
            x[R] = X + Y;
            x[S] = mul_shoup_lazy3(Y + b * Q - X, f, Q);
        }
    }
}
template <int LOGN, int LO, int B, int RB0, bool LAST, int... R>
__device__ __forceinline__ void inv_stage_seq(u32 (&x)[Cfg<LOGN>::E], u32 lane, const uint2* tw, u32 Q, uint2 ninv,
                                              uint2 wlast, std::integer_sequence<int, R...>) {
    constexpr int LE = Cfg<LOGN>::LE;
    const u32 hi = (lane >> LO) << (LO + LE - B - 1);
    (inv_bfly<LOGN, LO, B, RB0, LAST, R>(x, hi, tw, Q, ninv, wlast), ...);
}
template <int LOGN, int LO, int BLO, int BHI, int RB0, bool LASTPASS>
__device__ __forceinline__ void inv_stages(u32 (&x)[Cfg<LOGN>::E], u32 lane, const uint2* tw, u32 Q, uint2 ninv, uint2 wlast) {
// ... 36 lines not shown
            fwd_stages_pair<LOGN, 6, LOGN - 1, 6>(xp, lane, twf, Q);
        }
        store_pass_pair<LOGN, 6>(poly, lane, xp);
        wave_sync();
        load_pass_pair<LOGN, C::F2LO>(poly, lane, xp);
        fwd_stages_pair<LOGN, C::F2LO, 5, C::F2LO>(xp, lane, twf, Q);
        store_pass_pair<LOGN, C::F2LO>(poly, lane, xp);
        wave_sync();
        load_pass<LOGN, 0>(poly, lane, x);
        fwd_stages<LOGN, 0, C::F2LO - 1, 0, LAZY>(x, lane, twf, Q);
    } else {
        if constexpr (LM_IN) load_lm<LOGN>(poly, lane, x);
        else load_pass<LOGN, 6>(poly, lane, x);
        fwd_stages<LOGN, 6, LOGN - 1, 6, LAZY>(x, lane, twf, Q);
        store_pass<LOGN, 6>(poly, lane, x);
        wave_sync();
        load_pass<LOGN, C::F2LO>(poly, lane, x);
        fwd_stages<LOGN, C::F2LO, 5, C::F2LO, LAZY>(x, lane, twf, Q);
        if constexpr (C::F2LO > 0) {
            store_pass<LOGN, C::F2LO>(poly, lane, x);
            wave_sync();
            load_pass<LOGN, 0>(poly, lane, x);
            fwd_stages<LOGN, 0, C::F2LO - 1, 0, LAZY>(x, lane, twf, Q);
        }
    }
    if constexpr (NORM || !LAZY) {
#pragma unroll
        for (int r = 0; r < C::E; ++r) {
            if constexpr (LAZY) {
                u32 v = x[r] - __umulhi(x[r], mu32) * Q;
                x[r] = csub(csub(v, 2 * Q), Q);
            } else {
                x[r] = csub(csub(x[r], 2 * Q), Q);
            }
        }
    }
    store_pass<LOGN, 0>(poly, lane, x);
    wave_sync();
}

__device__ __forceinline__ void ntt_forward_wave_low8(u32* poly, const uint2* twf, u32 lane, u32 Q) {
    constexpr int LOGN = 10;
    {
        u64 xp[16];
        load_pass_pair<LOGN, 4>(poly, lane, xp);
        fwd_stages_pair<LOGN, 4, 7, 4>(xp, lane, twf, Q);
        store_pass_pair<LOGN, 4>(poly, lane, xp);
    }
    wave_sync();
    u32 x[16];
    u64 xp[16];
    load_pass<LOGN, 0>(poly, lane, x);
    fwd_first_stage_pair<LOGN>(x, xp, twf[tw_pos<64>(lane)], Q);
    fwd_stages_pair<LOGN, 0, 2, 0>(xp, lane, twf, Q);
#pragma unroll
    for (int r = 0; r < 16; ++r) x[r] = (u32)xp[r];
    store_pass<LOGN, 0>(poly, lane, x);
    wave_sync();
}
__device__ __forceinline__ void fwd_bfly_pair(u64& xa, u64& xb, uint2 w, u32 Q) {
    const u32 X = (u32)xa, Y = (u32)xb;
    const u64 t = mad64(__umulhi(Y, w.y), 0u - Q, mad64(Y, w.x, xa));
    xb = with_lo(xb, (X << 1) + 2 * Q - (u32)t);
    xa = t;
}
__device__ __forceinline__ void ntt_forward_half_low8(u32* row, u32 h, const uint2* twf, u32 lane, u32 Q) {
    asm volatile("" : "+v"(lane));
    u64 xp[8];
    {
        const u32 l8 = lane >> 5, j0 = (h << 9) | (l8 << 8) | (lane & 31u);
        u32* const p = row + phys(j0);
#pragma unroll
        for (int r = 0; r < 8; ++r) xp[r] = pair_of(p[(r >> 1) * 68 + (r & 1) * 32]);
        const u32 i7 = (h << 1) | l8;
        const uint2 w7 = twf[tw_pos<4>(i7)];
#pragma unroll
        for (int r = 0; r < 4; ++r) fwd_bfly_pair(xp[r], xp[r + 4], w7, Q);
#pragma unroll
        for (int g = 0; g < 2; ++g) {
            const uint2 w6 = twf[tw_pos<8>((i7 << 1) | g)];
            fwd_bfly_pair(xp[4 * g], xp[4 * g + 2], w6, Q);
            fwd_bfly_pair(xp[4 * g + 1], xp[4 * g + 3], w6, Q);
        }
#pragma unroll
        for (int g = 0; g < 4; ++g) fwd_bfly_pair(xp[2 * g], xp[2 * g + 1], twf[tw_pos<16>((i7 << 2) | g)], Q);
#pragma unroll
        for (int r = 0; r < 8; ++r) p[(r >> 1) * 68 + (r & 1) * 32] = (u32)xp[r];
    }
    wave_sync();
    {
        const u32 lh = lane >> 2, j0 = (h << 9) | (lh << 5) | (lane & 3u);
        u32* const p = row + phys(j0);
#pragma unroll
        for (int r = 0; r < 8; ++r) xp[r] = pair_of(p[4 * r]);
        const u32 i4 = (h << 4) | lh;
        const uint2 w4 = twf[tw_pos<32>(i4)];
#pragma unroll
        for (int r = 0; r < 4; ++r) fwd_bfly_pair(xp[r], xp[r + 4], w4, Q);
#pragma unroll
        for (int g = 0; g < 2; ++g) {
            const uint2 w3 = twf[tw_pos<64>((i4 << 1) | g)];
            fwd_bfly_pair(xp[4 * g], xp[4 * g + 2], w3, Q);
            fwd_bfly_pair(xp[4 * g + 1], xp[4 * g + 3], w3, Q);
        }
#pragma unroll
        for (int g = 0; g < 4; ++g) fwd_bfly_pair(xp[2 * g], xp[2 * g + 1], twf[tw_pos<128>((i4 << 2) | g)], Q);
#pragma unroll
        for (int r = 0; r < 8; ++r) p[4 * r] = (u32)xp[r];
    }
    wave_sync();
    {
        const u32 j0 = (h << 9) | (lane << 3);
        uint4* const p = reinterpret_cast<uint4*>(row + phys(j0));
        const uint4 v0 = p[0], v1 = p[1];
        xp[0] = pair_of(v0.x); xp[1] = pair_of(v0.y); xp[2] = pair_of(v0.z); xp[3] = pair_of(v0.w);
        xp[4] = pair_of(v1.x); xp[5] = pair_of(v1.y); xp[6] = pair_of(v1.z); xp[7] = pair_of(v1.w);
        const u32 i1 = (((h << 6) | lane) << 1);
#pragma unroll
        for (int g = 0; g < 2; ++g) {
            const uint2 w1 = twf[tw_pos<256>(i1 | g)];
            fwd_bfly_pair(xp[4 * g], xp[4 * g + 2], w1, Q);
            fwd_bfly_pair(xp[4 * g + 1], xp[4 * g + 3], w1, Q);
        }
#pragma unroll
        for (int g = 0; g < 4; ++g) fwd_bfly_pair(xp[2 * g], xp[2 * g + 1], twf[tw_pos<512>((i1 << 1) | g)], Q);
        p[0] = make_uint4((u32)xp[0], (u32)xp[1], (u32)xp[2], (u32)xp[3]);
        p[1] = make_uint4((u32)xp[4], (u32)xp[5], (u32)xp[6], (u32)xp[7]);
    }
    wave_sync();
}
__device__ __forceinline__ u64 mad64_su(u32 a, u32 b_uniform, u64 c) {
    u64 r, carry;
    asm("v_mad_u64_u32 %0, %1, %2, %3, %4" : "=v"(r), "=s"(carry) : "v"(a), "s"(b_uniform), "v"(c));
    return r;
}
__device__ __forceinline__ void fwd_bfly_pair_su(u64& xa, u64& xb, uint2 w_uniform, u32 Q) {
    const u32 X = (u32)xa, Y = (u32)xb;
    const u64 t = mad64(__umulhi(Y, w_uniform.y), 0u - Q, mad64_su(Y, w_uniform.x, xa));
    xb = with_lo(xb, (X << 1) + 2 * Q - (u32)t);
    xa = t;
}
template <bool SU>
__device__ __forceinline__ void fwd_pass4_pair(u64 (&x)[4], uint2 wa, uint2 wb0, uint2 wb1, u32 Q) {
    if constexpr (SU) {
        fwd_bfly_pair_su(x[0], x[2], wa, Q); fwd_bfly_pair_su(x[1], x[3], wa, Q);
        fwd_bfly_pair_su(x[0], x[1], wb0, Q); fwd_bfly_pair_su(x[2], x[3], wb1, Q);
    } else {
        fwd_bfly_pair(x[0], x[2], wa, Q); fwd_bfly_pair(x[1], x[3], wa, Q);
        fwd_bfly_pair(x[0], x[1], wb0, Q); fwd_bfly_pair(x[2], x[3], wb1, Q);
    }
}
typedef int v4i __attribute__((ext_vector_type(4)));
__device__ __forceinline__ u32 xb_group(u32 j, u32 g) { return 64u * j + 16u * ((g ^ (0u - (j >> 2))) & 3u); }
template <bool MFMA>
__device__ __forceinline__ void ntt_forward_quarter3(u32* rows, u32 qr, uint2 w7, uint2 w6a, uint2 w6b, const u32* xb,
                                                     const v4i (&A)[4], uint2 w14, const uint2* twf, u32 lane, u32 Q) {
    constexpr int RS = 2 * Cfg<10>::NP;
    u64 xp[3][4];
    auto pass16 = [&](uint2 wa, uint2 wb0, uint2 wb1) {
        const uint4* const p = reinterpret_cast<const uint4*>(rows + 4 * lane);
        uint4 v[3];
#pragma unroll
        for (int k = 0; k < 3; ++k) v[k] = p[k * (RS / 4)];
#pragma unroll
        for (int k = 0; k < 3; ++k) {
            xp[k][0] = ((u64)v[k].y << 32) | v[k].x; xp[k][2] = pair_of(v[k].y);
            xp[k][1] = ((u64)v[k].w << 32) | v[k].z; xp[k][3] = pair_of(v[k].w);
            fwd_pass4_pair<false>(xp[k], wa, wb0, wb1, Q);
        }
    };
    auto store4 = [&](u32 off) {
        u32* const p = rows + off;
#pragma unroll
        for (int k = 0; k < 3; ++k)
#pragma unroll
            for (int r = 0; r < 4; ++r) p[k * RS + 64 * r] = (u32)xp[k][r];
    };
    if constexpr (!MFMA) {
        {
            const u32* const p = rows + lane;
#pragma unroll
            for (int k = 0; k < 3; ++k)
#pragma unroll
                for (int r = 0; r < 4; ++r) xp[k][r] = pair_of(p[k * RS + 68 * r]);
#pragma unroll
            for (int k = 0; k < 3; ++k) fwd_pass4_pair<true>(xp[k], w7, w6a, w6b, Q);
            store4(((lane & 15u) << 2) | ((lane >> 3) & 2u) | (lane >> 5));
        }
        wave_sync();
        {
            const u32 h = lane >> 4;
            const uint2 w5 = twf[tw_pos<16>(4 * qr + h)];
            const uint4 w4 = *reinterpret_cast<const uint4*>(twf + tw_pos<32>(8 * qr + 2 * h));
            pass16(w5, make_uint2(w4.x, w4.y), make_uint2(w4.z, w4.w));
            store4(((lane >> 4) << 4) | ((lane & 3u) << 2) | ((lane >> 1) & 2u) | ((lane >> 3) & 1u));
        }
        wave_sync();
        {
            const u32 h = (((lane >> 2) & 3u) << 2) | (lane >> 4);
            const uint2* const t = twf + tw_pos<64>(16 * qr + h);
            pass16(t[0], t[64], t[128]);
            store4((((lane >> 2) & 3u) << 4) | ((lane >> 4) << 2) | ((lane & 1u) << 1) | ((lane >> 1) & 1u));
        }
    } else {
        {
            const char* const pb = reinterpret_cast<const char*>(xb) + xb_group(lane & 15u, lane >> 4);
            v4i B[3];
#pragma unroll
            for (int k = 0; k < 3; ++k) B[k] = *reinterpret_cast<const v4i*>(pb + 1024 * k);
            const u32 negQ = 0u - Q;
            const v4i c0 = {(int)Q, 0, (int)Q, 0};
#pragma unroll
            for (int i = 0; i < 4; ++i) {
#pragma unroll
                for (int k = 0; k < 3; ++k) {
                    const v4i s = __builtin_amdgcn_mfma_i32_16x16x64_i8(A[i], B[k], c0, 0, 0, 0);
                    const u32 lo = ((u32)s[1] << 7) + (u32)s[0], hi = ((u32)s[3] << 7) + (u32)s[2];
                    xp[k][i] = mad64(__umulhi(hi, w14.y), negQ, mad64_su(hi, w14.x, ((u64)(u32)s[1] << 32) | lo));
                }
            }
            store4(((lane >> 4) << 4) | ((lane & 3u) << 2) | ((lane >> 1) & 2u) | ((lane >> 3) & 1u));
        }
        wave_sync();
        {
            const u32 h = lane >> 2;
            const uint2* const t = twf + tw_pos<64>(16 * qr + h);
            pass16(t[0], t[64], t[128]);
            store4((h << 2) | ((lane & 1u) << 1) | ((lane >> 1) & 1u));
        }
    }
    wave_sync();
    {
        const u32 h = lane & 15u, g = lane >> 4;
        const uint2* const t = twf + 512 + 128 * g + 16 * qr + h;
        pass16(twf[256 + 64 * g + 16 * qr + h], t[0], t[64]);
        uint4* const p = reinterpret_cast<uint4*>(rows + 16 * h + 4 * g + 4 * (h >> 2));
#pragma unroll
        for (int k = 0; k < 3; ++k) p[k * (RS / 4)] = make_uint4((u32)xp[k][0], (u32)xp[k][1], (u32)xp[k][2], (u32)xp[k][3]);
    }
    wave_sync();
}
__device__ __forceinline__ void fwd_bfly(u32& X, u32& Y, uint2 w, u32 Q) {
    const u64 t = mad64(__umulhi(Y, w.y), 0u - Q, mad64(Y, w.x, pair_of(X)));
    Y = (X << 1) + 2 * Q - (u32)t;
    X = (u32)t;
}

template <int LOGN>
__device__ __forceinline__ void ntt_inverse_wave(const u32* src, u32* tmp, const uint2* twi, u32 lane, u32 Q,
                                                 uint2 ninv, uint2 wlast, u32 mu32, u32 (&x)[Cfg<LOGN>::E]) {
    using C = Cfg<LOGN>;
    constexpr int LE = C::LE;
    constexpr auto regs = std::make_integer_sequence<int, C::E>{};
    load_pass<LOGN, 0>(src, lane, x);
    inv_stages<LOGN, 0, 0, LE - 1, 0, false>(x, lane, twi, Q, ninv, wlast);
    inv_pass_reduce<LOGN, 0, LE>(x, Q, mu32, regs);
    store_pass<LOGN, 0>(tmp, lane, x);
    wave_sync();
    load_pass<LOGN, LE>(tmp, lane, x);
    inv_stages<LOGN, LE, LE, 2 * LE - 1, 0, false>(x, lane, twi, Q, ninv, wlast);
    inv_pass_reduce<LOGN, 0, LE>(x, Q, mu32, regs);
    store_pass<LOGN, LE>(tmp, lane, x);
    wave_sync();
    load_pass<LOGN, 6>(tmp, lane, x);
    inv_stages<LOGN, 6, 2 * LE, LOGN - 1, 2 * LE - 6, true>(x, lane, twi, Q, ninv, wlast);
}

template <int LOGN>
__device__ __forceinline__ u32 psi_pow(__amdgpu_buffer_rsrc_t psi_rsrc, u32 e, u32 Q) {
    constexpr u32 N = 1u << LOGN;
    const u32 v = __builtin_amdgcn_raw_buffer_load_b32(psi_rsrc, (e & (N - 1)) << 2, 0, 0);
    return (e & N) ? Q - v : v;
}

__device__ __forceinline__ uint4 bsk_row(__amdgpu_buffer_rsrc_t rsrc, u32 voff, u32 soff) {
    typedef u32 v4u __attribute__((ext_vector_type(4)));
    const v4u v = __builtin_amdgcn_raw_buffer_load_b128(rsrc, voff, soff, 0);
    return make_uint4(v.x, v.y, v.z, v.w);
}


template <int LOGN, bool LAZY, typename PT>
__device__ __forceinline__ void ginx_mac_tail(const PT& P, __amdgpu_buffer_rsrc_t psi_rsrc, u32 Q, u32 ap, uint2 Ia,
                                              uint2 Ina, u32 p0, const u32* accp, u32* accw, const u64 (&sp)[4],
                                              const u64 (&sn)[4], u32 (&a)[4]) {
    constexpr u32 N = 1u << LOGN;
    const bool odd = ap & 1u;
    const u32 k0 = __brev(p0) >> (32 - LOGN);
    const u32 ex = ((2 * k0 + 1) * ap) & (2 * N - 1);
    u32 mp[4], mn[4];
    mp[0] = psi_pow<LOGN>(psi_rsrc, ex, Q);
    mn[0] = psi_pow<LOGN>(psi_rsrc, (2 * N - ex) & (2 * N - 1), Q);
    mp[2] = csub(mul_shoup_lazy(mp[0], Ia, Q), Q);
    mn[2] = csub(mul_shoup_lazy(mn[0], Ina, Q), Q);
    mp[1] = odd ? Q - mp[0] : mp[0];
    mn[1] = odd ? Q - mn[0] : mn[0];
    mp[3] = odd ? Q - mp[2] : mp[2];
    mn[3] = odd ? Q - mn[2] : mn[2];
    const uint4 a4v = *reinterpret_cast<const uint4*>(accp);
    a[0] = a4v.x; a[1] = a4v.y; a[2] = a4v.z; a[3] = a4v.w;
#pragma unroll
    for (int e = 0; e < 4; ++e) {
        if constexpr (LAZY) {
            const u32 rp = barrett_lazy3((u64)(u32)(sp[e] >> 32) * P.c32 + (u32)sp[e], Q, P.red_shift, P.red_mu);
            const u32 rn = barrett_lazy3((u64)(u32)(sn[e] >> 32) * P.c32 + (u32)sn[e], Q, P.red_shift, P.red_mu);
            a[e] = csub(barrett_lazy3((u64)rp * (mp[e] - 1) + (u64)rn * (mn[e] - 1) + a[e], Q, P.red_shift, P.red_mu), 2 * Q);
        } else {
            const u32 rp = barrett_reduce(sp[e], Q, P.red_shift, P.red_mu);
            const u32 rn = barrett_reduce(sn[e], Q, P.red_shift, P.red_mu);
            a[e] = barrett_reduce((u64)rp * (mp[e] - 1) + (u64)rn * (mn[e] - 1) + a[e], Q, P.red_shift, P.red_mu);
        }
    }
    *reinterpret_cast<uint4*>(accw) = make_uint4(a[0], a[1], a[2], a[3]);
}

__device__ __forceinline__ u32 redc(u64 x, u32 Q, u32 qn) { return (u32)(mad64((u32)x * qn, Q, x) >> 32); }
template <int LOGN, bool EVENF = false, typename PT>
__device__ __forceinline__ void ginx_mac_tail_redc(const PT& P, __amdgpu_buffer_rsrc_t psi_r2_rsrc, u32 Q, u32 ap, u32 p0,
                                                   const u32* accp, u32* accw, const u64 (&sp)[4], const u64 (&sn)[4],
                                                   u32 (&a)[4]) {
    constexpr u32 N = 1u << LOGN;
    const u32 k0 = __brev(p0) >> (32 - LOGN);
    const u32 ex = ((2 * k0 + 1) * ap) & (2 * N - 1);
    const u32 off = P.r2_off, K = Q + 2 * off, qn = P.qinv_neg;
    u32 mp[4], mn[4];
    const u32 p0r = psi_pow<LOGN>(psi_r2_rsrc, ex, Q), n0r = psi_pow<LOGN>(psi_r2_rsrc, (2 * N - ex) & (2 * N - 1), Q);
    mp[0] = p0r + off;
    mn[0] = n0r + off;
    if constexpr (EVENF) {
        const bool neg = ap & 2u;
        mp[2] = neg ? K - mp[0] : mp[0];
        mn[2] = neg ? K - mn[0] : mn[0];
        mp[1] = mp[0]; mn[1] = mn[0]; mp[3] = mp[2]; mn[3] = mn[2];
    } else {
        const bool odd = ap & 1u;
        const u32 a4 = ap & 3u;
        const uint2 Ia = make_uint2(P.I4[a4], P.I4s[a4]);
        const uint2 Ina = make_uint2(P.I4[(4u - a4) & 3u], P.I4s[(4u - a4) & 3u]);
        mp[2] = csub(mul_shoup_lazy(p0r, Ia, Q), Q) + off;
        mn[2] = csub(mul_shoup_lazy(n0r, Ina, Q), Q) + off;
        mp[1] = odd ? K - mp[0] : mp[0];
        mn[1] = odd ? K - mn[0] : mn[0];
        mp[3] = odd ? K - mp[2] : mp[2];
        mn[3] = odd ? K - mn[2] : mn[2];
    }
    const uint4 a4v = *reinterpret_cast<const uint4*>(accp);
    a[0] = a4v.x; a[1] = a4v.y; a[2] = a4v.z; a[3] = a4v.w;
#pragma unroll
    for (int e = 0; e < 4; ++e) {
        const u32 rp = redc(sp[e], Q, qn), rn = redc(sn[e], Q, qn);
        a[e] = csub(redc(mad64(rn, mn[e], mul64(rp, mp[e])), Q, qn) + a[e], 2 * Q);
    }
    *reinterpret_cast<uint4*>(accw) = make_uint4(a[0], a[1], a[2], a[3]);
}

template <int LOGN, bool LAZY, u32 T, typename PT>
__device__ __forceinline__ void bootstrap_prologue(const PT& P, const bce_gate_desc& g, u32 soff, uint2* twf, u32* acc,
                                                   u32* av, u32 tid, u32 lane, u32 wave) {
    using C = Cfg<LOGN>;
    constexpr int N = C::N, NP = C::NP;
    const u32 Q = P.Q, q = P.q, qm = q - 1, n = P.n;
    for (u32 i = tid; i < (u32)N; i += T) twf[i] = P.tw_f[i];
    const u32 op = g.op & 0xFFu;
    {
        const u32* in0 = P.pool + (size_t)(g.in0 + soff) * P.pool_stride;
        const u32* in1 = P.pool + (size_t)(g.in1 + soff) * P.pool_stride;
        const bool two = op <= BCE_XNOR_FAST;
        for (u32 i = tid; i <= n; i += T) {
            u32 v0 = in0[i];
            if (g.neg0) v0 = ((i == n ? (q >> 2) : 0u) - v0) & qm;
            u32 v = v0;
            if (two) {
                u32 v1 = in1[i];
                if (g.neg1) v1 = ((i == n ? (q >> 2) : 0u) - v1) & qm;
                v = (op == BCE_XOR_FAST || op == BCE_XNOR_FAST) ? (2u * (v0 - v1)) & qm : (v0 + v1) & qm;
            } else if (i == n) {
                v = (v0 + (q >> 2)) & qm;
            }
            av[i] = v;
        }
    }
    __syncthreads();
    {
        const u32 b = av[n];
        const u32 q1 = gate_const(op, q), q2 = (q1 + (q >> 1)) & qm;
        const u32 pos = P.Q8p1, neg = Q - P.Q8p1;
        for (u32 j = tid; j < (u32)N; j += T) {
            u32 v = 0;
// ... 121 lines not shown
                for (int e = 0; e < 4; ++e)
                    a[e] = LAZY ? barrett_fold(sp[e], P.c32, Q, P.red_shift, P.red_mu) : barrett_reduce(sp[e], Q, P.red_shift, P.red_mu);
                *reinterpret_cast<uint4*>(acc + c * NP + pp) = make_uint4(a[0], a[1], a[2], a[3]);
            }
            __syncthreads();
            continue;
        }
        const u32 a4 = ap & 3u;
        const uint2 Ia = make_uint2(P.I4[a4], P.I4s[a4]);
        const uint2 Ina = make_uint2(P.I4[(4u - a4) & 3u], P.I4s[(4u - a4) & 3u]);
        for (u32 item = tid; item < 2u * (N / 4); item += T) {
            const u32 c = item / (N / 4), p0 = (item % (N / 4)) * 4;
            const u32 pp = phys(p0);
            const u32 toff = (c * N + p0) * 4u;
            u64 sp[4] = {0, 0, 0, 0}, sn[4] = {0, 0, 0, 0};
            constexpr u32 H = R / 2;
            if constexpr (OCC >= 3) {
#pragma unroll
                for (u32 h = 0; h < 2; ++h) {
                    uint4 kA[H], kB[H];
#pragma unroll
                    for (u32 l = 0; l < H; ++l) kA[l] = bsk_row(rsrc, toff, rowb + (h * H + l) * (2 * N * 4));
#pragma unroll
                    for (u32 l = 0; l < H; ++l) kB[l] = bsk_row(rsrc, toff, rowb + (rgsw + (h * H + l) * 2 * N) * 4);
                    __builtin_amdgcn_sched_barrier(0);
#pragma unroll
                    for (u32 l = 0; l < H; ++l) {
                        const uint4 d = *reinterpret_cast<const uint4*>(dct + (h * H + l) * NP + pp);
                        sp[0] += (u64)d.x * kA[l].x; sp[1] += (u64)d.y * kA[l].y; sp[2] += (u64)d.z * kA[l].z; sp[3] += (u64)d.w * kA[l].w;
                        sn[0] += (u64)d.x * kB[l].x; sn[1] += (u64)d.y * kB[l].y; sn[2] += (u64)d.z * kB[l].z; sn[3] += (u64)d.w * kB[l].w;
                    }
                    __builtin_amdgcn_sched_barrier(0);
                }
            } else {
            uint4 kA[R], kB[H];
#pragma unroll
            for (u32 l = 0; l < R; ++l) kA[l] = bsk_row(rsrc, toff, rowb + l * (2 * N * 4));
#pragma unroll
            for (u32 l = 0; l < H; ++l) kB[l] = bsk_row(rsrc, toff, rowb + (rgsw + l * 2 * N) * 4);
            __builtin_amdgcn_sched_barrier(0);
#pragma unroll
            for (u32 l = 0; l < R; ++l) {
                const uint4 d = *reinterpret_cast<const uint4*>(dct + l * NP + pp);
                sp[0] += (u64)d.x * kA[l].x; sp[1] += (u64)d.y * kA[l].y; sp[2] += (u64)d.z * kA[l].z; sp[3] += (u64)d.w * kA[l].w;
            }
            __builtin_amdgcn_sched_barrier(0);
#pragma unroll
            for (u32 l = 0; l < H; ++l) kA[l] = bsk_row(rsrc, toff, rowb + (rgsw + (H + l) * 2 * N) * 4);
            __builtin_amdgcn_sched_barrier(0);
#pragma unroll
            for (u32 l = 0; l < H; ++l) {
                const uint4 d = *reinterpret_cast<const uint4*>(dct + l * NP + pp);
                sn[0] += (u64)d.x * kB[l].x; sn[1] += (u64)d.y * kB[l].y; sn[2] += (u64)d.z * kB[l].z; sn[3] += (u64)d.w * kB[l].w;
            }
#pragma unroll
            for (u32 l = 0; l < H; ++l) {
                const uint4 d = *reinterpret_cast<const uint4*>(dct + (H + l) * NP + pp);
                sn[0] += (u64)d.x * kA[l].x; sn[1] += (u64)d.y * kA[l].y; sn[2] += (u64)d.z * kA[l].z; sn[3] += (u64)d.w * kA[l].w;
            }
            }
            u32 anew[4];
            ginx_mac_tail<LOGN, LAZY>(P, psi_rsrc, Q, ap, Ia, Ina, p0, acc + c * NP + pp, acc + c * NP + pp, sp, sn, anew);
        }
        BCE_PROF_MARK(4);
        __syncthreads();
        BCE_PROF_MARK(5);
    }
    BCE_PROF_FLUSH();

    if (wave < 2) {
        u32 x[E];
        ntt_inverse_wave<LOGN>(acc + wave * NP, dct + wave * NP, twf, lane, Q, ninv, wlast, P.mu32, x);
        u32* out = acc_out + ((size_t)blockIdx.x * 2 + wave) * N;
#pragma unroll
        for (int r = 0; r < E; ++r) out[((u32)r << 6) | lane] = x[r];
    }
}

__device__ __forceinline__ u32 xlay1(u32 p) { return (p & 15u) + 20u * ((p >> 4) & 3u) + 80u * ((p >> 6) & 3u) + 320u * (p >> 8); }
__device__ __forceinline__ u32 xlay2(u32 p) { return (p & 63u) + 80u * ((p >> 6) & 3u) + 320u * (p >> 8); }

__device__ __forceinline__ void inv_pass4(u32 (&x)[4], uint2 fa, uint2 fb, uint2 fc, u32 Q, u32 mu32) {
    const u32 Q2 = 2 * Q;
    const u32 a0 = x[0] + x[1];
    const u32 a1 = mul_shoup_lazy3(x[1] + Q2 - x[0], fa, Q);
    const u32 a2 = x[2] + x[3];
    const u32 a3 = mul_shoup_lazy3(x[3] + Q2 - x[2], fb, Q);
    const u32 b0 = a0 + a2;
    x[2] = mul_shoup_lazy3(a2 + 2 * Q2 - a0, fc, Q);
    const u32 b1 = a1 + a3;
    x[3] = mul_shoup_lazy3(a3 + Q2 - a1, fc, Q);
    x[0] = b0 - __umulhi(b0, mu32) * Q;
    x[1] = csub(b1, Q2);
}
__device__ __forceinline__ void inv_pass4_last(u32 (&x)[4], uint2 fa, uint2 fb, uint2 ninv, uint2 wlast, u32 Q) {
    const u32 Q2 = 2 * Q;
    const u32 a0 = x[0] + x[1];
    const u32 a1 = mul_shoup_lazy3(x[1] + Q2 - x[0], fa, Q);
    const u32 a2 = x[2] + x[3];
    const u32 a3 = mul_shoup_lazy3(x[3] + Q2 - x[2], fb, Q);
    x[0] = csub(mul_shoup_lazy3(a0 + a2, ninv, Q), Q);
    x[2] = csub(mul_shoup_lazy3(a0 + 2 * Q2 - a2, wlast, Q), Q);
    x[1] = csub(mul_shoup_lazy3(a1 + a3, ninv, Q), Q);
    x[3] = csub(mul_shoup_lazy3(a1 + Q2 - a3, wlast, Q), Q);
}

template <bool REGTW>
struct SplitInv {
    u32 a0, x0, l1, s1, l2, s2, l3, s3, t;
    uint2 fa[REGTW ? 5 : 1], fb[REGTW ? 5 : 1], fc[REGTW ? 4 : 1];
    u32 ia[REGTW ? 1 : 4], ic[REGTW ? 1 : 4];
};
template <bool REGTW>
__device__ __forceinline__ void split_inv_setup(SplitInv<REGTW>& S, const uint2* twf, u32 t) {
    S.t = t;
    S.a0 = phys(4 * t);
    const u32 wb = 48u * (t >> 6);
    S.x0 = S.a0 + wb;
    const u32 pb1 = ((t >> 2) << 4) | (t & 3u), pb2 = ((t >> 4) << 6) | (t & 15u), pb3 = ((t >> 6) << 8) | (t & 63u);
    S.l1 = phys(pb1) + wb; S.s1 = xlay1(pb1);
    S.l2 = xlay1(pb2); S.s2 = xlay2(pb2);
    S.l3 = xlay2(pb3); S.s3 = 320u * (t >> 6) + (t & 63u);
    const u32 u0 = t, u1 = t >> 2, u2 = t >> 4, u3 = t >> 6;
    if constexpr (REGTW) {
        S.fa[0] = twf[tw_pos<512>(511 - 2 * u0)]; S.fb[0] = twf[tw_pos<512>(510 - 2 * u0)]; S.fc[0] = twf[tw_pos<256>(255 - u0)];
        S.fa[1] = twf[tw_pos<128>(127 - 2 * u1)]; S.fb[1] = twf[tw_pos<128>(126 - 2 * u1)]; S.fc[1] = twf[tw_pos<64>(63 - u1)];
        S.fa[2] = twf[tw_pos<32>(31 - 2 * u2)];   S.fb[2] = twf[tw_pos<32>(30 - 2 * u2)];   S.fc[2] = twf[tw_pos<16>(15 - u2)];
        S.fa[3] = twf[tw_pos<8>(7 - 2 * u3)];     S.fb[3] = twf[tw_pos<8>(6 - 2 * u3)];     S.fc[3] = twf[tw_pos<4>(3 - u3)];
        S.fa[4] = twf[tw_pos<2>(1)];              S.fb[4] = twf[tw_pos<2>(0)];
    } else {
        S.ia[0] = tw_pos<512>(511 - 2 * u0); S.ic[0] = tw_pos<256>(255 - u0);
        S.ia[1] = tw_pos<128>(127 - 2 * u1); S.ic[1] = tw_pos<64>(63 - u1);
        S.ia[2] = tw_pos<32>(31 - 2 * u2);   S.ic[2] = tw_pos<16>(15 - u2);
        S.ia[3] = tw_pos<8>(7 - 2 * u3);     S.ic[3] = tw_pos<4>(3 - u3);
    }
}
template <bool REGTW, int K>
__device__ __forceinline__ void split_tw(const SplitInv<REGTW>& S, const uint2* twf, uint2& fa, uint2& fb, uint2& fc) {
    if constexpr (REGTW) { fa = S.fa[K]; fb = S.fb[K]; fc = S.fc[K]; }
    else {
        constexpr u32 M = 512u >> (2 * K);
        fa = twf[S.ia[K]];
        fb = twf[M < 64 ? S.ia[K] - 1 : S.ia[K] - 64];
        fc = twf[S.ic[K]];
    }
}
template <bool REGTW>
__device__ __forceinline__ void split_pass0(const SplitInv<REGTW>& S, const uint2* twf, u32 (&a)[4], u32* xa, u32 Q, u32 mu32) {
    uint2 fa, fb, fc;
    split_tw<REGTW, 0>(S, twf, fa, fb, fc);
    inv_pass4(a, fa, fb, fc, Q, mu32);
    *reinterpret_cast<uint4*>(xa + S.x0) = make_uint4(a[0], a[1], a[2], a[3]);
}
template <bool REGTW, typename F>
__device__ __forceinline__ void split_inverse_rest(const SplitInv<REGTW>& S, const uint2* twf, u32* xa, u32* xb, u32 Q, u32 mu32,
                                                   uint2 ninv, uint2 wlast, u32 (&x)[4], F&& at_pass) {
    uint2 fa, fb, fc;
    wave_sync();
    at_pass(std::integral_constant<int, 1>{});
#pragma unroll
    for (int r = 0; r < 4; ++r) x[r] = xa[S.l1 + 4 * r];
    split_tw<REGTW, 1>(S, twf, fa, fb, fc);
    inv_pass4(x, fa, fb, fc, Q, mu32);
#pragma unroll
    for (int r = 0; r < 4; ++r) xb[S.s1 + 4 * r] = x[r];
    wave_sync();
    at_pass(std::integral_constant<int, 2>{});
#pragma unroll
    for (int r = 0; r < 4; ++r) x[r] = xb[S.l2 + 20 * r];
    split_tw<REGTW, 2>(S, twf, fa, fb, fc);
    inv_pass4(x, fa, fb, fc, Q, mu32);
#pragma unroll
    for (int r = 0; r < 4; ++r) xa[S.s2 + 16 * r] = x[r];
    wave_sync();
    at_pass(std::integral_constant<int, 3>{});
#pragma unroll
    for (int r = 0; r < 4; ++r) x[r] = xa[S.l3 + 80 * r];
    split_tw<REGTW, 3>(S, twf, fa, fb, fc);
    inv_pass4(x, fa, fb, fc, Q, mu32);
#pragma unroll
    for (int r = 0; r < 4; ++r) xb[S.s3 + 64 * r] = x[r];
    block_sync_lds();
    at_pass(std::integral_constant<int, 4>{});
#pragma unroll
    for (int r = 0; r < 4; ++r) x[r] = xb[S.t + 320 * r];
    if constexpr (REGTW) inv_pass4_last(x, S.fa[4], S.fb[4], ninv, wlast, Q);
    else inv_pass4_last(x, twf[tw_pos<2>(1)], twf[tw_pos<2>(0)], ninv, wlast, Q);
}

enum class Fwd {
    Rows,
    RowsAndHalves,
    Quarters,
    QuartersMfma,
};
template <int WPS_, bool AP_, bool FUSE_, Fwd FWD_>
struct LatVariant {
    static constexpr int LOGN = 10, DG = 4, WPS = WPS_;
    static constexpr bool AP = AP_, FUSE = FUSE_, FOLD = FWD_ != Fwd::Rows;
    static constexpr bool MFMA = FWD_ == Fwd::QuartersMfma, QUNITS = MFMA || FWD_ == Fwd::Quarters;
    static constexpr bool EVENF = QUNITS;
    static constexpr bool REGTW = WPS <= 2;
    static constexpr u32 R = 2 * DG, T = 64 * R;
    static constexpr u32 PR = REGTW ? R : R / 2;
    static_assert(WPS == 2 || WPS == 4, "one or two workgroups per CU");
    static_assert(!QUNITS || (WPS == 4 && !AP), "quarter units (folded key by construction): two workgroups per CU, GINX");
};
struct LatLds {
    static constexpr u32 N = Cfg<10>::N, NP = Cfg<10>::NP, R = 8, XB = 1280;
    static constexpr u32 twf = 0;
    static constexpr u32 acc = twf + 2 * N;
    static constexpr u32 dct = acc + 2 * NP;
    static constexpr u32 xab = dct + R * NP;
    static constexpr u32 xbm = xab + 4 * XB;
    static constexpr u32 av(bool mfma) { return xbm + (mfma ? 6 * 256 : 0); }
    static constexpr size_t bytes(bool mfma, u32 n) { return (av(mfma) + ((n + 1 + 3) & ~3u)) * sizeof(u32); }
    static constexpr size_t tail_bytes = (xbm - dct) * sizeof(u32);
};
template <class V, bool PERSIST, typename PT>
__device__ __forceinline__ void lat_bootstrap(const PT& P, const bce_gate_desc g, const u32 soff, const u32 boot, u32* smem,
                                              u32* __restrict__ acc_out, u32* __restrict__ dbg_lweN, u32* __restrict__ dbg_ks) {
    constexpr int LOGN = V::LOGN, DG = V::DG, WPS = V::WPS;
    constexpr bool AP = V::AP, FUSE = V::FUSE, FOLD = V::FOLD, QUNITS = V::QUNITS, MFMA = V::MFMA;
    using C = Cfg<LOGN>;
    constexpr int N = C::N, NP = C::NP;
    constexpr u32 R = V::R, T = V::T, PR = V::PR, XB = LatLds::XB;
    constexpr bool REGTW = V::REGTW;
    uint2* twf = reinterpret_cast<uint2*>(smem + LatLds::twf);
    u32 *acc = smem + LatLds::acc, *dct = smem + LatLds::dct, *xab = smem + LatLds::xab, *xbm = smem + LatLds::xbm, *av = smem + LatLds::av(MFMA);

    u32 tid_ = threadIdx.x;
    if constexpr (PERSIST) asm volatile("" : "+v"(tid_));
    const u32 tid = tid_;
    const u32 lane = tid & 63;
    const u32 wave = __builtin_amdgcn_readfirstlane(tid >> 6);
    const u32 Q = P.Q, q = P.q, qm = q - 1, n = P.n;
    if constexpr (WPS >= 4 && !PERSIST) {
        if (P.xcd_gate != nullptr && wave == 0) {
            const u32 xcc = __builtin_amdgcn_s_getreg((31u << 11) | 20u) & 15u;
            u32* const gate = P.xcd_gate + 32u * xcc;
            const u32 slots = max(2u, 2u * (P.cu_count >> 3));
            const u32 mine = (gridDim.x + 7u - xcc) >> 3;
            const u32 t = u_add(gate, 1u);
            const u32 full = (t / slots + 1u) * slots, target = full < mine ? full : mine;
            const u64 t0 = __builtin_amdgcn_s_memrealtime();
            while (u_ld(gate) < target && __builtin_amdgcn_s_memrealtime() - t0 < P.xcd_gate_ticks) __builtin_amdgcn_s_sleep(8);
        }
    }
    bootstrap_prologue<LOGN, true, T>(P, g, soff, twf, acc, av, tid, lane, wave);

    const u32 c = wave >> 2;
    SplitInv<REGTW> S;
    split_inv_setup(S, twf, tid & 255u);
    u32* const accc = acc + c * NP;
    u32* const xa = xab + c * 2 * XB;
    u32* const xb = xa + XB;

    const uint2 ninv = make_uint2(P.Ninv, P.Ninv_s), wlast = make_uint2(P.Winv_last, P.Winv_last_s);
    constexpr u32 rgsw = R * 2 * N;
    const __amdgpu_buffer_rsrc_t rsrc =
        __builtin_amdgcn_make_buffer_rsrc(const_cast<u32*>(P.bsk), 0, AP ? 0x7FFFFFFF : (int)(n * 2 * rgsw * 4), 0x00020000);
    const __amdgpu_buffer_rsrc_t psi_rsrc = __builtin_amdgcn_make_buffer_rsrc(const_cast<u32*>(P.psi_tab_r2), 0, N * 4, 0x00020000);
    const u32 gb = P.gBits, Qh = Q >> 1;
    u32 off = 0;
    for (u32 l = 0; l < (u32)DG; ++l) off |= 1u << (l * gb + gb - 1);
    const u32 offm = off - Q, bias = Q - (1u << (gb - 1));
    const __amdgpu_buffer_rsrc_t mrsrc = __builtin_amdgcn_make_buffer_rsrc(const_cast<u32*>(P.fwd_mfma_tab), 0, MFMA ? 4 * 4 * 1024 : 0, 0x00020000);
    const u32 psel0 = 0x0c0c0400u, psel1 = 0x05040100u;
    const u32 mc = tid / (N / 4), mp0 = (tid % (N / 4)) * 4, mpp = phys(mp0);
    const u32 dig0 = phys(S.t);
    const uint2 w9 = twf[1], w8a = twf[2], w8b = twf[3];
    uint2 q7 = make_uint2(0, 0), q6a = q7, q6b = q7;
    if constexpr (QUNITS && !MFMA) {
        const uint2 a = twf[tw_pos<4>(wave & 3u)], b = twf[tw_pos<8>(2 * (wave & 3u))], d = twf[tw_pos<8>(2 * (wave & 3u) + 1)];
        q7 = make_uint2(__builtin_amdgcn_readfirstlane(a.x), __builtin_amdgcn_readfirstlane(a.y));
        q6a = make_uint2(__builtin_amdgcn_readfirstlane(b.x), __builtin_amdgcn_readfirstlane(b.y));
        q6b = make_uint2(__builtin_amdgcn_readfirstlane(d.x), __builtin_amdgcn_readfirstlane(d.y));
    }
    {
        const uint4 v = *reinterpret_cast<const uint4*>(accc + S.a0);
        u32 a[4] = {v.x, v.y, v.z, v.w};
        split_pass0(S, twf, a, xa, Q, P.mu32);
    }

    BCE_PROF_INIT();
    const u32 nsteps = AP ? n * P.dR : n;
    u32 cb = 0;
    if constexpr (WPS >= 4) __builtin_amdgcn_s_setprio(2);
    for (u32 step = 0; step < nsteps; ++step) {
        u32 ap = 0, rowb;
        if constexpr (!AP) {
            ap = ((q - av[step]) & qm) * P.factor;
            if (ap == 0) continue;
            rowb = step * (2 * rgsw * 4);
        } else {
            const u32 i = step / P.dR, kd = step - i * P.dR;
            u32 aI = (q - av[i]) & qm;
            for (u32 t = 0; t < kd; ++t) aI /= P.baseR;
            const u32 a0 = aI % P.baseR;
            if (a0 == 0) continue;
            rowb = (((i * P.baseR + a0) * P.dR + kd) * rgsw) * 4u;
        }
        uint4 kA[R], kB[R];
        v4i mA[4];
        auto request_rows = [&](auto kc) {
            constexpr u32 k = decltype(kc)::value - 1, G = PR / 4;
            BCE_PROF_MARK(8 + k);
#pragma unroll
            for (u32 l = k * G; l < (k + 1) * G; ++l) {
                kA[l] = bsk_row(rsrc, tid * 16u, rowb + l * (2 * N * 4));
                if constexpr (!AP) kB[l] = bsk_row(rsrc, tid * 16u, rowb + (rgsw + l * 2 * N) * 4);
            }
            if constexpr (MFMA && k == 3) {
#pragma unroll
                for (u32 v = 0; v < 4; ++v) mA[v] = __builtin_bit_cast(v4i, bsk_row(mrsrc, lane * 16u, ((wave & 3u) * 4u + v) * 1024u));
            }
        };
        {
            u32 x[4], u[4];
            split_inverse_rest(S, twf, xa, xb, Q, P.mu32, ninv, wlast, x, request_rows);
#pragma unroll
            for (int r = 0; r < 4; ++r) u[r] = x[r] + ((x[r] < Qh) ? off : offm);
            if constexpr (MFMA) {
#pragma unroll
                for (int r = 0; r < 4; ++r) u[r] ^= off;
            }
#pragma unroll
            for (u32 l = FOLD ? 1 : 0; l < (u32)DG; ++l) {
                if constexpr (MFMA) {
                    const u32 e01 = __builtin_amdgcn_perm((u32)__builtin_amdgcn_sbfe((int)u[1], l * gb, gb), (u32)__builtin_amdgcn_sbfe((int)u[0], l * gb, gb), psel0);
                    const u32 e23 = __builtin_amdgcn_perm((u32)__builtin_amdgcn_sbfe((int)u[3], l * gb, gb), (u32)__builtin_amdgcn_sbfe((int)u[2], l * gb, gb), psel0);
                    const u32 d = __builtin_amdgcn_perm(e23, e01, psel1);
                    const u32 G = S.t >> 4;
                    xbm[(3 * c + l - 1) * 256 + (xb_group(S.t & 15u, G >> 2) >> 2) + (G & 3u)] = d;
                    continue;
                }
                u32 v[4];
#pragma unroll
                for (int r = 0; r < 4; ++r) v[r] = __builtin_amdgcn_ubfe(u[r], l * gb, gb) + bias;
                fwd_bfly(v[0], v[2], w9, Q);
                fwd_bfly(v[1], v[3], w9, Q);
                fwd_bfly(v[0], v[1], w8a, Q);
                fwd_bfly(v[2], v[3], w8b, Q);
#pragma unroll
                for (int r = 0; r < 4; ++r) dct[(2 * l + c) * NP + dig0 + 272 * r] = v[r];
            }
        }
        BCE_PROF_MARK(0);
        block_sync_lds();
        BCE_PROF_MARK(1);
        if constexpr (WPS >= 4) { if (FOLD && wave >= 4) __builtin_amdgcn_s_setprio(1); else __builtin_amdgcn_s_setprio(0); }
#ifndef BCE_SKIP_FWD
        if constexpr (QUNITS) {
            ntt_forward_quarter3<MFMA>(dct + (2 + c) * NP + 272u * (wave & 3u), wave & 3u, q7, q6a, q6b, xbm + 3 * c * 256, mA,
                                       make_uint2(P.w14, P.w14s), twf, lane, Q);
        } else if constexpr (FOLD) {
            if (wave < 4) ntt_forward_wave_low8(dct + (2 + wave) * NP, twf, lane, Q);
            else ntt_forward_half_low8(dct + (6 + ((wave - 4) >> 1)) * NP, (wave - 4) & 1u, twf, lane, Q);
        } else {
            ntt_forward_wave_low8(dct + wave * NP, twf, lane, Q);
        }
#endif
        if constexpr (WPS >= 4) __builtin_amdgcn_s_setprio(2);
        BCE_PROF_MARK(2);
        if constexpr (PR < R) {
#pragma unroll
            for (u32 l = PR; l < R; ++l) kA[l] = bsk_row(rsrc, tid * 16u, rowb + l * (2 * N * 4));
#pragma unroll
            for (u32 l = PR; l < R; ++l) if constexpr (!AP) kB[l] = bsk_row(rsrc, tid * 16u, rowb + (rgsw + l * 2 * N) * 4);
        }
        block_sync_lds();
        BCE_PROF_MARK(3);
        {
            u64 sp[4] = {0, 0, 0, 0}, sn[4] = {0, 0, 0, 0};
#pragma unroll
            for (u32 l = 0; l < R; ++l) {
#ifdef BCE_SKIP_MAC
                const uint4 d = make_uint4(l + tid, l, tid, 1u);
#else
                const uint4 d = *reinterpret_cast<const uint4*>((FOLD && l < 2 ? acc + cb : dct) + l * NP + mpp);
#endif
                sp[0] += (u64)d.x * kA[l].x; sp[1] += (u64)d.y * kA[l].y; sp[2] += (u64)d.z * kA[l].z; sp[3] += (u64)d.w * kA[l].w;
                if constexpr (!AP) {
                    sn[0] += (u64)d.x * kB[l].x; sn[1] += (u64)d.y * kB[l].y; sn[2] += (u64)d.z * kB[l].z; sn[3] += (u64)d.w * kB[l].w;
                }
            }
            u32 anew[4];
            const u32* const accr = acc + cb + mc * NP + mpp;
            u32* const accw = acc + (FOLD ? 2 * NP - cb : 0) + mc * NP + mpp;
            if constexpr (AP) {
#pragma unroll
                for (int e = 0; e < 4; ++e) anew[e] = barrett_fold(sp[e], P.c32, Q, P.red_shift, P.red_mu);
                *reinterpret_cast<uint4*>(accw) = make_uint4(anew[0], anew[1], anew[2], anew[3]);
            } else {
                ginx_mac_tail_redc<LOGN, V::EVENF>(P, psi_rsrc, Q, ap, mp0, accr, accw, sp, sn, anew);
            }
            if constexpr (FOLD) cb = 2 * NP - cb;
            split_pass0(S, twf, anew, xa, Q, P.mu32);
        }
        BCE_PROF_MARK(4);
        wave_sync();
        BCE_PROF_MARK(5);
    }
    BCE_PROF_FLUSH();
    {
        u32 x[4];
        split_inverse_rest(S, twf, xa, xb, Q, P.mu32, ninv, wlast, x, [](auto) {});
        if (acc_out) {
            u32* out = acc_out + ((size_t)boot * 2 + c) * N + S.t;
#pragma unroll
            for (int r = 0; r < 4; ++r) out[256 * r] = x[r];
        }
        if constexpr (FUSE) {
#pragma unroll
            for (int r = 0; r < 4; ++r) acc[c * N + S.t + 256 * r] = x[r];
        }
    }
    if constexpr (FUSE) {
        if constexpr (WPS >= 4) __builtin_amdgcn_s_setprio(0);
        __syncthreads();
        u32* rowidx = dct;
        u64* red = reinterpret_cast<u64*>(dct + ((N * P.dKS + 3) & ~3u));
        u32* outp = P.pool + (size_t)(g.out + soff) * P.pool_stride;
        if (P.ksk_u16) fused_tail<uint16_t, T>(P, acc, rowidx, red, outp, boot, dbg_lweN, dbg_ks);
        else fused_tail<u32, T>(P, acc, rowidx, red, outp, boot, dbg_lweN, dbg_ks);
        if constexpr (!PERSIST) {
            if (g.op >> 8) {
                __syncthreads();
                const u32 e = pair_rotation(P, g.op), row = boot + gridDim.x;
                if (P.ksk_u16) fused_tail<uint16_t, T>(P, acc, rowidx, red, outp + P.pool_stride, row, dbg_lweN, dbg_ks, e);
                else fused_tail<u32, T>(P, acc, rowidx, red, outp + P.pool_stride, row, dbg_lweN, dbg_ks, e);
            }
        }
    }
}

template <class V>
__global__ __launch_bounds__(V::T, V::WPS) void k_blind_rotate_lat(DevParams P, const bce_gate_desc* __restrict__ descs, u32 n_desc,
                                                                   u32 slot_stride, u32* __restrict__ acc_out,
                                                                   u32* __restrict__ dbg_lweN, u32* __restrict__ dbg_ks) {
    extern __shared__ __align__(16) u32 smem[];
    lat_bootstrap<V, false>(P, descs[blockIdx.x % n_desc], (blockIdx.x / n_desc) * slot_stride, blockIdx.x, smem, acc_out, dbg_lweN, dbg_ks);
}

bool fused_tail_fits(const DevParams& P) {
    const size_t N = P.N;
    const size_t VW = P.ksk_u16 ? 8 : 4, G = (P.n + VW) / VW, Gv = G < 512 ? G : 512, RW = (Gv + 63) / 64, SL = 8 / RW;
    const size_t need = ((N * P.dKS + 3) & ~(size_t)3) * 4 + SL * Gv * VW * 8;
    return (size_t)P.n + 1 <= 512 * VW && RW <= 8 && need <= LatLds::tail_bytes;
}

struct LatBuild { int wps; bool ap; Fwd fwd; };
constexpr bool operator==(const LatBuild& a, const LatBuild& b) { return a.wps == b.wps && a.ap == b.ap && a.fwd == b.fwd; }
constexpr LatBuild kLatBuilds[] = {
    {2, false, Fwd::Rows}, {2, true, Fwd::Rows}, {2, false, Fwd::RowsAndHalves}, {2, true, Fwd::RowsAndHalves},
    {4, false, Fwd::Rows}, {4, true, Fwd::Rows}, {4, false, Fwd::RowsAndHalves}, {4, true, Fwd::RowsAndHalves},
    {4, false, Fwd::Quarters}, {4, false, Fwd::QuartersMfma},
};
LatBuild lat_variant(const DevParams& P, bool x1) {
    const bool ap = P.method_ap != 0, quarters = P.fwd_units && !ap && !x1;
    const Fwd fwd = !P.fold ? Fwd::Rows : !quarters ? Fwd::RowsAndHalves : P.fwd_mfma ? Fwd::QuartersMfma : Fwd::Quarters;
    return {x1 ? 2 : 4, ap, fwd};
}
size_t blind_rotate_lat_lds_bytes(const DevParams& P, const LatBuild& v) { return LatLds::bytes(v.fwd == Fwd::QuartersMfma, P.n); }
template <size_t I = 0, class F>
auto lat_kernel(const LatBuild& v, F of) -> decltype(of(std::integral_constant<size_t, 0>{})) {
    if constexpr (I == std::size(kLatBuilds)) return nullptr;
    else return kLatBuilds[I] == v ? of(std::integral_constant<size_t, I>{}) : lat_kernel<I + 1>(v, of);
}

struct WaveBuild { int logn, dg; bool lazy; int occ; bool ap; };
constexpr bool operator==(const WaveBuild& a, const WaveBuild& b) {
    return a.logn == b.logn && a.dg == b.dg && a.lazy == b.lazy && a.occ == b.occ && a.ap == b.ap;
}
constexpr WaveBuild kWaveBuilds[] = {
    {9, 3, true, 3, false},  {9, 3, true, 2, false},  {9, 3, false, 2, false},  {9, 3, true, 3, true},  {9, 3, true, 2, true},  {9, 3, false, 2, true},
    {9, 4, true, 3, false},  {9, 4, true, 2, false},  {9, 4, false, 2, false},  {9, 4, true, 3, true},  {9, 4, true, 2, true},  {9, 4, false, 2, true},
    {10, 3, true, 3, false}, {10, 3, true, 2, false}, {10, 3, false, 2, false}, {10, 3, true, 3, true}, {10, 3, true, 2, true}, {10, 3, false, 2, true},
    {10, 4, true, 3, false}, {10, 4, true, 2, false}, {10, 4, false, 2, false}, {10, 4, true, 3, true}, {10, 4, true, 2, true}, {10, 4, false, 2, true},
    {11, 3, true, 2, false}, {11, 3, false, 2, false}, {11, 3, true, 2, true}, {11, 3, false, 2, true},
    {11, 4, true, 3, false}, {11, 4, true, 2, false}, {11, 4, false, 2, false}, {11, 4, true, 3, true}, {11, 4, true, 2, true}, {11, 4, false, 2, true},
};
WaveBuild wave_variant(const DevParams& P) {
    return {(int)P.logN, (int)P.dG, P.lazy != 0, (P.lazy && P.occupancy_target >= 3) ? 3 : 2, P.method_ap != 0};
}
using BrKernel = void (*)(DevParams, const bce_gate_desc*, u32, u32, u32*);
template <size_t I = 0>
BrKernel wave_kernel(const WaveBuild& v) {
    if constexpr (I == std::size(kWaveBuilds)) return nullptr;
    else {
        constexpr WaveBuild b = kWaveBuilds[I];
        return b == v ? k_blind_rotate<b.logn, b.dg, b.lazy, b.occ, b.ap> : wave_kernel<I + 1>(v);
    }
}
size_t blind_rotate_lds_bytes(const DevParams& P) {
    const size_t N = P.N, NP = N + (N >> 6) * 4, R = 2 * P.dG;
    return (2 * N + (2 + R) * NP + ((P.n + 1 + 3) & ~3u)) * sizeof(u32);
}

KernelClass kernel_class(const DevParams& P) {
    const u32 occupancy = (P.occupancy_target == 2 || 3 * blind_rotate_lds_bytes(P) > kLdsBytesPerCu) ? 2 : 3;
    KernelClass k{};
    if (P.is64) {
        k = kernel_class64(P);
        k.occupancy_target = occupancy;
        return k;
    }
    k.occupancy_target = occupancy;
    if (P.dG < 3 || P.dG > 4 || (P.logN == 11 && P.dG != 3)) k.error = kDigitCountError;
    const bool ap = P.method_ap != 0;
    const bool split = P.variant != 1 && P.logN == 10 && P.dG == 4 && P.lazy;
    k.family = split ? KernelFamily::SplitTransform : KernelFamily::WavePerTransform;
    if (split) {
        k.fold_build = std::any_of(std::begin(kLatBuilds), std::end(kLatBuilds), [ap](const LatBuild& b) { return b.ap == ap && b.fwd != Fwd::Rows; });
        k.dag = fused_tail_fits(P);
        k.wg_per_cu_lone = lat_variant(P, true).wps / 2;
        k.wg_per_cu_full = lat_variant(P, false).wps / 2;
        k.lds_bytes = blind_rotate_lat_lds_bytes(P, lat_variant(P, false));
    } else {
        k.wg_per_cu_lone = 1;
        k.wg_per_cu_full = k.occupancy_target;
        k.lds_bytes = blind_rotate_lds_bytes(P);
    }
    return k;
}

__global__ void k_dag_rearm(DagRearm D) {
    const size_t stride = (size_t)gridDim.x * blockDim.x, i0 = (size_t)blockIdx.x * blockDim.x + threadIdx.x;
    const size_t items = (size_t)D.n_tasks * D.instances;
    for (size_t i = i0; i < items; i += stride) D.dep[i] = D.dep_init[i % D.n_tasks];
    for (u32 q = 0; q < kDagQueues; ++q) {
        const u32 ninit = (D.init_off[q + 1] - D.init_off[q]) * D.instances;
        for (size_t j = i0; j < D.qcap[q]; j += stride) {
            u32 v = 0;
            if (j < ninit) {
                const u32 ti = (u32)(j / D.instances), k = (u32)(j % D.instances);
                v = k * D.n_tasks + D.init_items[D.init_off[q] + ti] + 1u;
            }
            D.slots[q][j] = v;
        }
        if (i0 == 0) { D.ctl[q] = 0; D.ctl[kDagQueues + q] = ninit; D.ctl[kDagIdleCus] = 0; }
    }
    for (size_t j = i0 + kDagAbort; j < kDagCtlWords; j += stride) D.ctl[j] = 0;
}

template <class V>
__global__ __launch_bounds__(V::T, V::WPS) void k_bootstrap_dag(const DevParams* Pp, const DagParams* Dp) {
    extern __shared__ __align__(16) u32 smem[];
    dag_worker(Pp, Dp, smem, [&](ConstDagParams& D, u32 t, u32 k) {
        lat_bootstrap<V, true>(*as_constant<ConstDevParams>(Pp), D.tasks[t], D.slot_base + k * D.slot_stride, 0, smem + kDagMailboxWords,
                               nullptr, nullptr, nullptr);
    });
}

hipError_t launch_dag_rearm(const DagRearm& D, hipStream_t s) {
    hipLaunchKernelGGL(k_dag_rearm, dim3(1024), dim3(256), 0, s, D);
    return hipGetLastError();
}

hipError_t launch_bootstrap_dag(const DevParams& P, const DevParams* d_P, const DagParams* d_params, int wps, u32 grid, hipStream_t s) {
    if (!dag_kernel_available(P)) return hipErrorInvalidValue;
    if (P.is64) return launch_bootstrap_dag64(P, d_P, d_params, grid, s);
    using DagKernel = void (*)(const DevParams*, const DagParams*);
    const LatBuild v = lat_variant(P, wps <= 2);
    const DagKernel k = lat_kernel(v, [](auto i) -> DagKernel {
        constexpr LatBuild b = kLatBuilds[i];
        return k_bootstrap_dag<LatVariant<b.wps, b.ap, true, b.fwd>>;
    });
    if (!k) return hipErrorInvalidValue;
    const size_t lds = blind_rotate_lat_lds_bytes(P, v) + kDagMailboxWords * 4;
    return launch_kernel_lds(k, dim3(grid), dim3(512), lds, s, LaunchEvents{}, d_P, d_params);
}

hipError_t launch_blind_rotate(const DevParams& P, const bce_gate_desc* d, u32 n_desc, u32 instances, u32 slot_stride,
                               void* acc_out, hipStream_t s, int* kernel_id, u32* dbg_lweN, u32* dbg_ks, bool* tail_fused, LaunchEvents ev) {
    if (tail_fused) *tail_fused = false;
    if (P.is64) {
        if (kernel_id) *kernel_id = BCE_BR_WORD64;
        return launch_blind_rotate64(P, d, n_desc, instances, slot_stride, static_cast<u64*>(acc_out), s, dbg_lweN, dbg_ks, tail_fused, ev);
    }
    if (kernel_id) *kernel_id = BCE_BR_WAVE_PER_TRANSFORM;
    const KernelClass kc = kernel_class(P);
    if (P.fold && !kc.fold_build) return hipErrorInvalidValue;
    u32* const acc = static_cast<u32*>(acc_out);
    const dim3 grid(n_desc * instances), block(128 * P.dG);
    if (kc.family == KernelFamily::SplitTransform) {
        using LatKernel = void (*)(DevParams, const bce_gate_desc*, u32, u32, u32*, u32*, u32*);
        const bool alone = (P.variant == 2) || (P.variant == 0 && grid.x <= P.cu_count);
        const bool x1 = alone && P.variant != 3;
        const LatBuild v = lat_variant(P, x1);
        const bool fuse = !x1 && tail_fused && P.fuse_tail && fused_tail_fits(P);
        const LatKernel lk = lat_kernel(v, [fuse](auto i) -> LatKernel {
            constexpr LatBuild b = kLatBuilds[i];
            if constexpr (b.wps >= 4) { if (fuse) return k_blind_rotate_lat<LatVariant<b.wps, b.ap, true, b.fwd>>; }
            return k_blind_rotate_lat<LatVariant<b.wps, b.ap, false, b.fwd>>;
        });
        if (!lk) return hipErrorInvalidValue;
        if (kernel_id) *kernel_id = x1 ? BCE_BR_SPLIT_X1 : BCE_BR_SPLIT_X2;
        if (tail_fused) *tail_fused = fuse;
        DevParams Pl = P;
        if (x1 || grid.x <= 2 * P.cu_count) Pl.xcd_gate = nullptr;
        if (Pl.xcd_gate) {
            const hipError_t e = hipMemsetAsync(Pl.xcd_gate, 0, 16 * 32 * sizeof(u32), s);
            if (e != hipSuccess) return e;
        }
        return launch_kernel_lds(lk, grid, block, blind_rotate_lat_lds_bytes(P, v), s, ev, Pl, d, n_desc, slot_stride, acc,
                                 fuse ? dbg_lweN : nullptr, fuse ? dbg_ks : nullptr);
    }
    const BrKernel kern = wave_kernel(wave_variant(P));
    if (!kern) return hipErrorInvalidValue;
    return launch_kernel_lds(kern, grid, block, kc.lds_bytes, s, ev, P, d, n_desc, slot_stride, acc);
}


template <typename KT, typename AW, bool PAIR>
__global__ __launch_bounds__(256) void k_tail_gather(DevParams P, u32 S, const AW* __restrict__ acc_in,
                                                     u64* __restrict__ partial, u32* __restrict__ dbg_lweN,
                                                     const bce_gate_desc* __restrict__ descs, u32 n_desc) {
    extern __shared__ __align__(16) u32 smem[];
    constexpr u32 VW = 16 / sizeof(KT);
    const u32 N = P.N, n = P.n, qKS = P.qKS, B = P.baseKS, D = P.dKS;
    const u64 Q = sizeof(AW) == 8 ? P.Q64 : (u64)P.Q;
    const u32 tid = threadIdx.x, lane = tid & 63;
    const u32 wave = __builtin_amdgcn_readfirstlane(tid >> 6);
    const u32 boot = blockIdx.x / S, s = blockIdx.x - boot * S;
    u32 rot = 0, dbg_row = boot;
    if constexpr (PAIR) {
        const u32 op = descs[boot % n_desc].op;
        if (!(op >> 8)) return;
        rot = pair_rotation(P, op);
        dbg_row = boot + gridDim.x / S;
    }
    const u32 ni = N / S, i0 = s * ni, LR = ni * D;
    u32* rowidx = smem;
    u64* red = reinterpret_cast<u64*>(smem + ((LR + 3) & ~3u));
    const AW* a0 = acc_in + (size_t)boot * 2 * N;

    for (u32 ii = tid; ii < ni; ii += 256) {
        const u32 i = i0 + ii;
        const u64 v = rotated_coef(a0, i == 0 ? 0 : N - i, rot, N, Q, i != 0);
        u32 at = round_qQ(v, qKS, Q);
        if (dbg_lweN) dbg_lweN[(size_t)dbg_row * (N + 1) + i] = at;
        for (u32 j = 0; j < D; ++j) {
            rowidx[ii * D + j] = (i * B + at % B) * D + j;
            at /= B;
        }
    }
    __syncthreads();

    const KT* __restrict__ ksk = reinterpret_cast<const KT*>(P.ksk);
    const u32 G = (n + VW) / VW;
    const u32 Gv = G < 256 ? G : 256;
    const u32 RW = (Gv + 63) / 64, SL = 4 / RW;
    const u32 slice = wave / RW, group = (wave - slice * RW) * 64 + lane;
    u64 tot[VW];
#pragma unroll
    for (u32 e = 0; e < VW; ++e) tot[e] = 0;
    if (slice < SL && group < Gv) {
        const u32 CH = P.ks_chunk;
        constexpr u32 U = 8;
        u32 r = slice;
        while (r < LR) {
            u32 run[VW];
#pragma unroll
            for (u32 e = 0; e < VW; ++e) run[e] = 0;
            const u32 rend = (LR - r > CH * SL) ? r + CH * SL : LR;
            for (; r + (U - 1) * SL < rend; r += U * SL) {
                uint4 v[U];
#pragma unroll
                for (u32 u = 0; u < U; ++u) {
                    const u32 row = __builtin_amdgcn_readfirstlane(rowidx[r + u * SL]);
                    v[u] = reinterpret_cast<const uint4*>(ksk + (size_t)row * P.ksk_stride)[group];
                }
#pragma unroll
                for (u32 u = 0; u < U; ++u) {
                    if constexpr (sizeof(KT) == 2) {
                        run[0] += v[u].x & 0xFFFFu; run[1] += v[u].x >> 16; run[2] += v[u].y & 0xFFFFu; run[3] += v[u].y >> 16;
                        run[4] += v[u].z & 0xFFFFu; run[5] += v[u].z >> 16; run[6] += v[u].w & 0xFFFFu; run[7] += v[u].w >> 16;
                    } else {
                        run[0] += v[u].x; run[1] += v[u].y; run[2] += v[u].z; run[3] += v[u].w;
                    }
                }
            }
            for (; r < rend; r += SL) {
                const u32 row = __builtin_amdgcn_readfirstlane(rowidx[r]);
                const uint4 v = reinterpret_cast<const uint4*>(ksk + (size_t)row * P.ksk_stride)[group];
                if constexpr (sizeof(KT) == 2) {
                    run[0] += v.x & 0xFFFFu; run[1] += v.x >> 16; run[2] += v.y & 0xFFFFu; run[3] += v.y >> 16;
                    run[4] += v.z & 0xFFFFu; run[5] += v.z >> 16; run[6] += v.w & 0xFFFFu; run[7] += v.w >> 16;
                } else {
                    run[0] += v.x; run[1] += v.y; run[2] += v.z; run[3] += v.w;
                }
            }
#pragma unroll
            for (u32 e = 0; e < VW; ++e) tot[e] += run[e];
        }
#pragma unroll
        for (u32 e = 0; e < VW; ++e) red[(size_t)slice * Gv * VW + group * VW + e] = tot[e];
    }
    __syncthreads();
    u64* out = partial + ((size_t)boot * S + s) * (n + 1);
    for (u32 k = tid; k < Gv * VW && k <= n; k += 256) {
        u64 sum = 0;
        for (u32 sl = 0; sl < SL; ++sl) sum += red[(size_t)sl * Gv * VW + k];
        out[k] = sum;
    }
    for (u32 k = Gv * VW; k <= n; ++k) {
        __syncthreads();
        u64 sum = 0;
        for (u32 r = tid; r < LR; r += 256) sum += (u64)ksk[(size_t)rowidx[r] * P.ksk_stride + k];
        red[tid] = sum;
        __syncthreads();
        if (tid == 0) {
            u64 t = 0;
            for (u32 i = 0; i < 256; ++i) t += red[i];
            out[k] = t;
        }
    }
}

template <typename AW, bool PAIR>
__global__ __launch_bounds__(256) void k_tail_finish(DevParams P, const bce_gate_desc* __restrict__ descs, u32 n_desc, u32 slot_stride,
                                                     u32 S, const AW* __restrict__ acc_in, const u64* __restrict__ partial,
                                                     u32* __restrict__ dbg_lweN, u32* __restrict__ dbg_ks) {
    const u32 N = P.N, n = P.n, qKS = P.qKS;
    const u64 Q = sizeof(AW) == 8 ? P.Q64 : (u64)P.Q;
    const u64 Q8p1 = sizeof(AW) == 8 ? P.Q8p1_64 : (u64)P.Q8p1;
    const u32 boot = blockIdx.x;
    const bce_gate_desc g = descs[boot % n_desc];
    u32 rot = 0, dbg_row = boot;
    if constexpr (PAIR) {
        if (!(g.op >> 8)) return;
        rot = pair_rotation(P, g.op);
        dbg_row = boot + gridDim.x;
    }
    u32* out = P.pool + (size_t)(g.out + (PAIR ? 1u : 0u) + (boot / n_desc) * slot_stride) * P.pool_stride;
    const u64* part = partial + (size_t)boot * S * (n + 1);
    for (u32 k = threadIdx.x; k <= n; k += 256) {
        u64 sum = 0;
        for (u32 s = 0; s < S; ++s) sum += part[(size_t)s * (n + 1) + k];
        const u32 sm = (u32)(sum % qKS);
        u32 base = 0;
        if (k == n) {
            u64 b = rotated_coef(acc_in + (size_t)boot * 2 * N + N, 0, rot, N, Q, false) + Q8p1;
            b = b >= Q ? b - Q : b;
            base = round_qQ(b, qKS, Q);
            if (dbg_lweN) dbg_lweN[(size_t)dbg_row * (N + 1) + N] = base;
        }
// ... 256 lines not shown
```

openfhe-boolean-circuit-evaluator_amd/csrc/kernels.hpp:

```cpp
#pragma once
#include <hip/hip_runtime_api.h>
#include <hip/hip_ext.h>

#include <tuple>

#include <cstdint>

#include "../../include/bce_gpu.h"

namespace bce {

using u32 = uint32_t;
using u64 = uint64_t;

struct DevParams {
    u32 n, N, logN;
    u32 q;
    u32 Q;
    u32 qKS;
    u32 baseKS, dKS;
    u32 ksk_stride;
    u32 ksk_u16;
    u32 ks_chunk;
    u32 gBits, dG;
    u32 baseR, dR;
    u32 method_ap;
    u32 factor;
    u32 Q8p1;
    u32 red_shift;
    u32 red_mu;
    u32 Ninv, Ninv_s;
    u32 Winv_last, Winv_last_s;
    u32 mu32;
    u32 lazy;
    u32 c32;
    u32 occupancy_target;
    u32 variant;
    u32 cu_count;
    u32* xcd_gate;
    u32 xcd_gate_ticks;
    u32 fuse_tail;
    u32 fold_ninv;
    u32 fold;
    u32 fwd_units;
    u32 factor_even;
    u32 I4[4], I4s[4];
    const uint2* tw_f;
    const u32* psi_tab;
    const u32* psi_tab_r2;
    u32 qinv_neg;
    u32 r2_off;
    const u32* bsk;
    u32 is64;
    u64 Q64, Q8p1_64;
    u64 mu64;
    u64 c64;
    u64 Ninv64, Ninv64_s;
    const ulonglong2* tw64;
    const u64* bsk64;
    u32 fp64;
    double Qd, invQd;
    double Ninvd, Ninvd_q;
    const double2* tw64d;
    const void* ksk;
    u32* pool;
    u32 pool_stride;
    u32 fwd_mfma;
    u32 w14, w14s;
    const u32* fwd_mfma_tab;
};

constexpr size_t kLdsBytesPerCu = 160 * 1024;
enum class KernelFamily {
    WavePerTransform,
    SplitTransform,
    Int64,
    Fp64,
};
struct KernelClass {
    KernelFamily family;
    const char* error;
    const char* lds_error;
    bool fold_build;
    bool dag;
    u32 fp64;
    u32 occupancy_target;
    u32 wg_per_cu_lone, wg_per_cu_full;
    size_t lds_bytes;
};
KernelClass kernel_class(const DevParams& P);

constexpr u32 kDagQueues = 4;
constexpr u32 kDagCtlStride = 32;
constexpr u32 kDagCuKeys = 4096;
constexpr u32 kDagAbort = kDagQueues * kDagCtlStride;
constexpr u32 kDagDone = kDagAbort + 1;
constexpr u32 kDagLazyWaits = kDagAbort + 2;
constexpr u32 kDagBusyTicks = kDagAbort + 4;
constexpr u32 kDagWaitTicks = kDagAbort + 6;
constexpr u32 kDagIdleCus = 8;
constexpr u32 kDagCuArrive = kDagAbort + 32;
constexpr u32 kDagCuBusy = kDagCuArrive + kDagCuKeys;
constexpr u32 kDagGate = kDagCuBusy + kDagCuKeys;
constexpr u32 kDagCohortRing = 64;
constexpr u32 kDagCohort = kDagGate + 16 * 32;
constexpr u32 kDagGateWaits = kDagAbort + 8;
constexpr u32 kDagCtlWords = kDagCohort + 16 * kDagCohortRing * 2;
struct DagRearm {
    const bce_gate_desc* tasks;
    const u32* cons_off;
    const u32* cons;
    const uint8_t* qid;
    const u32* dep_init;
    u32* dep;
    u32* slots[kDagQueues];
    u32 qcap[kDagQueues];
    const u32* init_items;
    u32 init_off[kDagQueues + 1];
    u32* ctl;
    u32 n_tasks, instances, slot_stride, slot_base;
    u32 lazy_ticks;
    u32 stall_ticks;
    u32 policy;
    u32 gate_ticks;
    u32 gate_backlog;
};
struct DagParams : DagRearm {
    const u32* chk_of_task;
    const uint8_t* expect;
    u32 n_checks;
    u32 repair;
    const int8_t* s8;
    bce_check_report* report;
    bce_check_entry* log;
};
hipError_t launch_dag_rearm(const DagRearm& D, hipStream_t s);
hipError_t launch_bootstrap_dag(const DevParams& P, const DevParams* d_P, const DagParams* d_params, int wps, u32 grid,
                                hipStream_t s);
inline bool dag_kernel_available(const DevParams& P) { return kernel_class(P).dag; }

struct LaunchEvents {
    hipEvent_t start = nullptr, stop = nullptr;
};
template <typename... KA, typename... A>
inline hipError_t launch_with_events(void (*kern)(KA...), dim3 grid, dim3 block, size_t lds, hipStream_t s, LaunchEvents ev, A... args) {
    static_assert(sizeof...(KA) == sizeof...(A), "argument count");
    std::tuple<KA...> held{static_cast<KA>(args)...};
    void* ptrs[sizeof...(KA)];
    std::apply([&](auto&... a) { size_t i = 0; ((ptrs[i++] = (void*)&a), ...); }, held);
    return hipExtLaunchKernel(reinterpret_cast<const void*>(kern), grid, block, ptrs, lds, s, ev.start, ev.stop, 0);
}
template <typename... KA, typename... A>
inline hipError_t launch_kernel(void (*kern)(KA...), dim3 grid, dim3 block, size_t lds, hipStream_t s, LaunchEvents ev, A... args) {
    if (ev.start || ev.stop) return launch_with_events(kern, grid, block, lds, s, ev, args...);
    hipLaunchKernelGGL(kern, grid, block, lds, s, static_cast<KA>(args)...);
    return hipGetLastError();
}
template <typename... KA, typename... A>
inline hipError_t launch_kernel_lds(void (*kern)(KA...), dim3 grid, dim3 block, size_t lds, hipStream_t s, LaunchEvents ev, A... args) {
    const hipError_t e = hipFuncSetAttribute(reinterpret_cast<const void*>(kern), hipFuncAttributeMaxDynamicSharedMemorySize, (int)lds);
    return e != hipSuccess ? e : launch_kernel(kern, grid, block, lds, s, ev, args...);
}

hipError_t launch_blind_rotate(const DevParams& P, const bce_gate_desc* d_descs, u32 n_desc, u32 instances,
                               u32 slot_stride, void* acc_out, hipStream_t s, int* kernel_id = nullptr,
                               u32* dbg_lweN = nullptr, u32* dbg_ks = nullptr, bool* tail_fused = nullptr, LaunchEvents ev = {});

size_t tail_partial_words(const DevParams& P, u32 boots);
hipError_t launch_tail(const DevParams& P, const bce_gate_desc* d_descs, u32 n_desc, u32 instances, u32 slot_stride,
                       const void* acc_in , u64* partial, u32* dbg_lweN, u32* dbg_ks,
                       hipStream_t s, LaunchEvents ev = {}, bool pairs = false);

hipError_t launch_words_u64_f64(u64* words, size_t count, int to_double, hipStream_t s);

hipError_t launch_lwe_unary(const DevParams& P, const bce_gate_desc* d_descs, u32 n_desc, u32 instances,
                            u32 slot_stride, hipStream_t s);

hipError_t launch_pool_pack(const DevParams& P, const bce_gate_desc* d_descs, u32 count, u32* buf, int to_pool,
                            hipStream_t s);

constexpr u32 kCheckLogCap = 4096;
constexpr u32 kCheckWaves = 4;
hipError_t launch_lwe_check(const DevParams& P, const int8_t* d_s, const u32* d_slots, const uint8_t* d_expect, u32 count,
                            u32 expect_stride, u32 instances, u32 slot_stride, int repair, u32 tag, bce_check_report* d_report,
                            bce_check_entry* d_log, hipStream_t s);

hipError_t launch_ntt_batch(const DevParams& P, void* polys, u32 count, int inverse, hipStream_t s);

hipError_t launch_fold_gadget(const DevParams& P, void* bsk, u64 rgsw, int dir, hipStream_t s);

hipError_t launch_pointwise_mac(const DevParams& P, void* b, const void* a, const void* z, u32 count, u32 b_step,
                                hipStream_t s);


constexpr const char* kDigitCountError = "gadget digit count must be 3 or 4 (N = 2048: 3, or 4 with a ring modulus of 28..30 bits)";
KernelClass kernel_class64(const DevParams& P);
hipError_t launch_bootstrap_dag64(const DevParams& P, const DevParams* d_P, const DagParams* d_params, u32 grid, hipStream_t s);
hipError_t launch_blind_rotate64(const DevParams& P, const bce_gate_desc* d_descs, u32 n_desc, u32 instances, u32 slot_stride,
                                 u64* acc_out, hipStream_t s, u32* dbg_lweN, u32* dbg_ks, bool* tail_fused, LaunchEvents ev);
hipError_t launch_ntt_batch64(const DevParams& P, u64* polys, u32 count, int inverse, hipStream_t s);
hipError_t launch_pointwise_mac64(const DevParams& P, u64* b, const u64* a, const u64* z, u32 count, u32 b_step, hipStream_t s);

}
```

Baseline: 193,700.

## Replace LDS round-trips in NTT stages with cross-lane permlane register exchanges

Adds an XREG path that uses permlane32/permlane16 swaps to do the data transpose between NTT passes in registers instead of storing to and reloading from LDS. It covers the MFMA forward quarter transform, with a transposed matrix table so the MFMA output lands in the right lanes, and the last inverse NTT pass. This drops the LDS traffic and one wave sync in those stages. It is on by default with an environment switch to turn it off, and adds more kernel instantiations plus reliance on gfx950 permlane builtins.

```diff
diff --git a/include/bce_gpu.h b/include/bce_gpu.h
--- a/include/bce_gpu.h
+++ b/include/bce_gpu.h
@@ -138,6 +138,8 @@
 int bce_forward_mfma_tables(uint64_t Q, uint32_t N, uint32_t gBits, uint32_t dG, uint64_t* psi, uint32_t* M6, uint32_t* C,
                             uint32_t* table, uint32_t* w14, uint64_t* bounds);
 int bce_launch_capacity(const bce_ctx*, uint32_t* lone, uint32_t* full);
+uint32_t bce_exchange_in_registers(const bce_ctx*);
+int bce_forward_mfma_table_transposed(uint64_t Q, uint32_t N, uint32_t gBits, uint32_t dG, uint32_t* table_t);
 
 int bce_rccl_available(void);
 int bce_rccl_version(void);
diff --git a/openfhe-boolean-circuit-evaluator_amd/__init__.py b/openfhe-boolean-circuit-evaluator_amd/__init__.py
--- a/openfhe-boolean-circuit-evaluator_amd/__init__.py
+++ b/openfhe-boolean-circuit-evaluator_amd/__init__.py
@@ -77,7 +77,7 @@
     "bce_keygen", "bce_import_keys", "bce_import_keys_eval", "bce_export_bsk_eval", "bce_import_keys_file", "bce_export_keys_file", "bce_bsk_words", "bce_ksk_words", "bce_export_sk", "bce_export_bsk",
     "bce_export_ksk", "bce_pool_reserve", "bce_pool_slots", "bce_lwe_write", "bce_lwe_read",
     "bce_encrypt_bits", "bce_set_encrypt_seed", "bce_decrypt_bits", "bce_eval_gates", "bce_eval_gates_strided", "bce_synchronize",
-    "bce_timing_reset", "bce_timing_get", "bce_timing_set_events", "bce_bytes_per_bootstrap", "bce_bytes_per_bootstrap_parts", "bce_forward_transforms_per_step", "bce_forward_units", "bce_forward_mfma", "bce_lazy_arithmetic", "bce_forward_mfma_tables", "bce_launch_capacity", "bce_rccl_available", "bce_rccl_version", "bce_rccl_unique_id", "bce_rccl_init", "bce_rccl_allgather", "bce_rccl_comm_info",
+    "bce_timing_reset", "bce_timing_get", "bce_timing_set_events", "bce_bytes_per_bootstrap", "bce_bytes_per_bootstrap_parts", "bce_forward_transforms_per_step", "bce_forward_units", "bce_forward_mfma", "bce_lazy_arithmetic", "bce_forward_mfma_tables", "bce_forward_mfma_table_transposed", "bce_exchange_in_registers", "bce_launch_capacity", "bce_rccl_available", "bce_rccl_version", "bce_rccl_unique_id", "bce_rccl_init", "bce_rccl_allgather", "bce_rccl_comm_info",
     "bce_rccl_shutdown", "bce_debug_eval_stages", "bce_debug_ntt", "bce_debug_tail",
     "bce_dag_supported", "bce_dag_create", "bce_dag_run", "bce_dag_destroy", "bce_dag_set_limits", "bce_dag_last_run", "bce_dag_debug_block_task",
     "bce_dag_set_checks", "bce_dag_set_expected",
@@ -103,6 +103,13 @@
         return 0, None
     return st, {"psi": int(psi.value), "M6": M6, "C": Cw, "table": tab, "w14": (int(w14[0]), int(w14[1])),
                 "limb_sum_max": int(bounds[0]), "lo_max": int(bounds[1]), "hi_max": int(bounds[2]), "out_max": int(bounds[3])}
+
+
+def forward_mfma_table_transposed(Q, N=1024, gBits=7, dG=4):
+    import numpy as np
+    tab = np.zeros((4, 4, 64, 4), np.uint32)
+    st = int(lib().bce_forward_mfma_table_transposed(int(Q), int(N), int(gBits), int(dG), tab.ctypes.data))
+    return st, (tab if st else None)
 
 
 def lib():
@@ -161,6 +168,10 @@
     L.bce_lazy_arithmetic.restype = C.c_uint32
     L.bce_forward_mfma_tables.argtypes = [u64, u32, u32, u32, vp, vp, vp, vp, vp, vp]
     L.bce_forward_mfma_tables.restype = i32
+    L.bce_forward_mfma_table_transposed.argtypes = [u64, u32, u32, u32, vp]
+    L.bce_forward_mfma_table_transposed.restype = i32
+    L.bce_exchange_in_registers.argtypes = [vp]
+    L.bce_exchange_in_registers.restype = C.c_uint32
     L.bce_launch_capacity.argtypes = [vp, C.POINTER(C.c_uint32), C.POINTER(C.c_uint32)]
     L.bce_rccl_unique_id.argtypes = [C.c_char_p]
     L.bce_rccl_init.argtypes = [vp, C.c_char_p, i32, i32]
@@ -492,6 +503,9 @@
 
     def forward_mfma(self):
         return int(self._L.bce_forward_mfma(self.h))
+
+    def exchange_in_registers(self):
+        return int(self._L.bce_exchange_in_registers(self.h))
 
     def lazy_arithmetic(self):
         return int(self._L.bce_lazy_arithmetic(self.h))
diff --git a/openfhe-boolean-circuit-evaluator_amd/csrc/engine.cpp b/openfhe-boolean-circuit-evaluator_amd/csrc/engine.cpp
--- a/openfhe-boolean-circuit-evaluator_amd/csrc/engine.cpp
+++ b/openfhe-boolean-circuit-evaluator_amd/csrc/engine.cpp
@@ -81,7 +81,7 @@
     hipStream_t stream = nullptr;
     DevParams P{};
     DevBuf<uint2> d_twf;
-    DevBuf<u32> d_fwd_mfma, d_psi, d_psi_r2, d_xcd_gate;
+    DevBuf<u32> d_fwd_mfma, d_fwd_mfma_t, d_psi, d_psi_r2, d_xcd_gate;
     DevBuf<char> d_bsk;
     DevBuf<ulonglong2> d_tw64;
     DevBuf<double2> d_tw64d;
@@ -297,6 +297,7 @@
             if (T.fwd.ok) { P.fwd_mfma = 1; P.w14 = T.fwd.w14; P.w14s = T.fwd.w14s; }
         }
     }
+    P.xchg_regs = env_off("BCE_XCHG_REGS") ? 0 : 1;
     P.pool_stride = n + 1;
     return BCE_OK;
 }
@@ -334,6 +335,11 @@
     if (P.fwd_mfma) {
         if (!up(c->d_fwd_mfma, T.fwd.table, "forward matrix table")) return BCE_ERR_HIP;
         P.fwd_mfma_tab = c->d_fwd_mfma.get();
+    }
+    P.fwd_mfma_tab_t = nullptr;
+    if (P.fwd_mfma && P.xchg_regs) {
+        if (!up(c->d_fwd_mfma_t, T.fwd.table_t, "transposed forward matrix table")) return BCE_ERR_HIP;
+        P.fwd_mfma_tab_t = c->d_fwd_mfma_t.get();
     }
     c->enc_seed_ok = os_entropy(c->enc_seed);
     return BCE_OK;
@@ -1595,6 +1601,13 @@
 uint32_t bce_forward_units(const bce_ctx* c) { return c ? c->P.fwd_units : 0; }
 uint32_t bce_forward_mfma(const bce_ctx* c) { return c ? c->P.fwd_mfma : 0; }
 uint32_t bce_lazy_arithmetic(const bce_ctx* c) { return c ? c->P.lazy : 0; }
+uint32_t bce_exchange_in_registers(const bce_ctx* c) { return c ? c->P.xchg_regs : 0; }
+int bce_forward_mfma_table_transposed(uint64_t Q, uint32_t N, uint32_t gBits, uint32_t dG, uint32_t* table_t) {
+    const FwdMfmaTables T = build_fwd_mfma_tables(Q, N, gBits, dG);
+    if (T.M6.empty()) return 0;
+    if (table_t) std::copy(T.table_t.begin(), T.table_t.end(), table_t);
+    return T.ok ? 1 : -1;
+}
 int bce_forward_mfma_tables(uint64_t Q, uint32_t N, uint32_t gBits, uint32_t dG, uint64_t* psi, uint32_t* M6, uint32_t* C, uint32_t* table,
                             uint32_t* w14, uint64_t* bounds) {
     const FwdMfmaTables T = build_fwd_mfma_tables(Q, N, gBits, dG);
diff --git a/openfhe-boolean-circuit-evaluator_amd/csrc/fwd_mfma.hpp b/openfhe-boolean-circuit-evaluator_amd/csrc/fwd_mfma.hpp
--- a/openfhe-boolean-circuit-evaluator_amd/csrc/fwd_mfma.hpp
+++ b/openfhe-boolean-circuit-evaluator_amd/csrc/fwd_mfma.hpp
@@ -17,6 +17,7 @@
     std::vector<u32> M6;
     std::vector<u32> C;
     std::vector<u32> table;
+    std::vector<u32> table_t;
     u32 w14 = 0, w14s = 0;
     u64 limb_sum_max = 0;
     u64 lo_max = 0, hi_max = 0, out_max = 0;
@@ -70,6 +71,14 @@
                 }
             }
         }
+    T.table_t.assign(kFwdMfmaTableWords, 0);
+    for (u32 q = 0; q < 4; ++q)
+        for (u32 limb = 0; limb < 4; ++limb)
+            for (u32 l = 0; l < 64; ++l)
+                for (u32 b = 0; b < 16; ++b) {
+                    const u32 byte = (T.M6[(16 * q + (l & 15u)) * 64 + fwd_mfma_h_of_k(16 * (l >> 4) + b)] >> (7 * limb)) & 127u;
+                    T.table_t[((q * kFwdMfmaLoads + limb) * 64 + l) * 4 + (b >> 2)] |= byte << (8 * (b & 3u));
+                }
     return T;
 }
 
diff --git a/openfhe-boolean-circuit-evaluator_amd/csrc/kernels.hip b/openfhe-boolean-circuit-evaluator_amd/csrc/kernels.hip
--- a/openfhe-boolean-circuit-evaluator_amd/csrc/kernels.hip
+++ b/openfhe-boolean-circuit-evaluator_amd/csrc/kernels.hip
@@ -89,6 +89,19 @@
     __builtin_amdgcn_fence(__ATOMIC_RELEASE, "wavefront");
     __builtin_amdgcn_wave_barrier();
     __builtin_amdgcn_fence(__ATOMIC_ACQUIRE, "wavefront");
+}
+
+__device__ __forceinline__ void lane_swap32(u32& a, u32& b) {
+    const auto r = __builtin_amdgcn_permlane32_swap(a, b, false, false);
+    a = r[0]; b = r[1];
+}
+__device__ __forceinline__ void lane_swap16(u32& a, u32& b) {
+    const auto r = __builtin_amdgcn_permlane16_swap(a, b, false, false);
+    a = r[0]; b = r[1];
+}
+__device__ __forceinline__ void lane_xchg54(u32 (&x)[4]) {
+    lane_swap32(x[0], x[2]); lane_swap32(x[1], x[3]);
+    lane_swap16(x[0], x[1]); lane_swap16(x[2], x[3]);
 }
 
 template <int LOGN, int LO>
@@ -431,7 +444,7 @@
 }
 typedef int v4i __attribute__((ext_vector_type(4)));
 __device__ __forceinline__ u32 xb_group(u32 j, u32 g) { return 64u * j + 16u * ((g ^ (0u - (j >> 2))) & 3u); }
-template <bool MFMA>
+template <bool MFMA, bool XREG = false>
 __device__ __forceinline__ void ntt_forward_quarter3(u32* rows, u32 qr, uint2 w7, uint2 w6a, uint2 w6b, const u32* xb,
                                                      const v4i (&A)[4], uint2 w14, const uint2* twf, u32 lane, u32 Q) {
     constexpr int RS = 2 * Cfg<10>::NP;
@@ -481,6 +494,33 @@
             pass16(t[0], t[64], t[128]);
             store4((((lane >> 2) & 3u) << 4) | ((lane >> 4) << 2) | ((lane & 1u) << 1) | ((lane >> 1) & 1u));
         }
+    } else if constexpr (XREG) {
+        const u32 m = lane & 15u;
+        const char* const pa = reinterpret_cast<const char*>(xb) + xb_group(4u * (m & 3u) + (m >> 2), lane >> 4);
+        v4i D[3];
+#pragma unroll
+        for (int k = 0; k < 3; ++k) D[k] = *reinterpret_cast<const v4i*>(pa + 1024 * k);
+        const u32 negQ = 0u - Q;
+        const v4i cq = {(int)Q, (int)Q, (int)Q, (int)Q}, cz = {0, 0, 0, 0};
+        const uint2* const t = twf + tw_pos<64>(16 * qr + m);
+        const uint2 w3 = t[0], w2a = t[64], w2b = t[128];
+#pragma unroll
+        for (int k = 0; k < 3; ++k) {
+            v4i s[4];
+#pragma unroll
+            for (int i = 0; i < 4; ++i) s[i] = __builtin_amdgcn_mfma_i32_16x16x64_i8(D[k], A[i], (i & 1) ? cz : cq, 0, 0, 0);
+#pragma unroll
+            for (int r = 0; r < 4; ++r) {
+                const u32 lo = ((u32)s[1][r] << 7) + (u32)s[0][r], hi = ((u32)s[3][r] << 7) + (u32)s[2][r];
+                const u32 next = (r & 1) ? (u32)s[0][r] : (u32)s[1][r + 1];
+                xp[k][r] = mad64(__umulhi(hi, w14.y), negQ, mad64_su(hi, w14.x, ((u64)next << 32) | lo));
+            }
+            fwd_pass4_pair<false>(xp[k], w3, w2a, w2b, Q);
+            u32 y[4] = {(u32)xp[k][0], (u32)xp[k][1], (u32)xp[k][2], (u32)xp[k][3]};
+            lane_xchg54(y);
+#pragma unroll
+            for (int r = 0; r < 4; ++r) xp[k][r] = with_lo(xp[k][r], y[r]);
+        }
     } else {
         {
             const char* const pb = reinterpret_cast<const char*>(xb) + xb_group(lane & 15u, lane >> 4);
@@ -508,11 +548,17 @@
             store4((h << 2) | ((lane & 1u) << 1) | ((lane >> 1) & 1u));
         }
     }
-    wave_sync();
+    if constexpr (!(MFMA && XREG)) wave_sync();
     {
         const u32 h = lane & 15u, g = lane >> 4;
         const uint2* const t = twf + 512 + 128 * g + 16 * qr + h;
-        pass16(twf[256 + 64 * g + 16 * qr + h], t[0], t[64]);
+        if constexpr (MFMA && XREG) {
+            const uint2 w1 = twf[256 + 64 * g + 16 * qr + h], w0a = t[0], w0b = t[64];
+#pragma unroll
+            for (int k = 0; k < 3; ++k) fwd_pass4_pair<false>(xp[k], w1, w0a, w0b, Q);
+        } else {
+            pass16(twf[256 + 64 * g + 16 * qr + h], t[0], t[64]);
+        }
         uint4* const p = reinterpret_cast<uint4*>(rows + 16 * h + 4 * g + 4 * (h >> 2));
 #pragma unroll
         for (int k = 0; k < 3; ++k) p[k * (RS / 4)] = make_uint4((u32)xp[k][0], (u32)xp[k][1], (u32)xp[k][2], (u32)xp[k][3]);
@@ -940,7 +986,7 @@
     inv_pass4(a, fa, fb, fc, Q, mu32);
     *reinterpret_cast<uint4*>(xa + S.x0) = make_uint4(a[0], a[1], a[2], a[3]);
 }
-template <bool REGTW, typename F>
+template <bool XREG, bool REGTW, typename F>
 __device__ __forceinline__ void split_inverse_rest(const SplitInv<REGTW>& S, const uint2* twf, u32* xa, u32* xb, u32 Q, u32 mu32,
                                                    uint2 ninv, uint2 wlast, u32 (&x)[4], F&& at_pass) {
     uint2 fa, fb, fc;
@@ -958,12 +1004,19 @@
     for (int r = 0; r < 4; ++r) x[r] = xb[S.l2 + 20 * r];
     split_tw<REGTW, 2>(S, twf, fa, fb, fc);
     inv_pass4(x, fa, fb, fc, Q, mu32);
-#pragma unroll
-    for (int r = 0; r < 4; ++r) xa[S.s2 + 16 * r] = x[r];
-    wave_sync();
-    at_pass(std::integral_constant<int, 3>{});
-#pragma unroll
-    for (int r = 0; r < 4; ++r) x[r] = xa[S.l3 + 80 * r];
+    if constexpr (XREG) {
+        wave_sync();
+        at_pass(std::integral_constant<int, 3>{});
+        asm volatile("" : "+v"(x[0]), "+v"(x[1]), "+v"(x[2]), "+v"(x[3]) : : "memory");
+        lane_xchg54(x);
+    } else {
+#pragma unroll
+        for (int r = 0; r < 4; ++r) xa[S.s2 + 16 * r] = x[r];
+        wave_sync();
+        at_pass(std::integral_constant<int, 3>{});
+#pragma unroll
+        for (int r = 0; r < 4; ++r) x[r] = xa[S.l3 + 80 * r];
+    }
     split_tw<REGTW, 3>(S, twf, fa, fb, fc);
     inv_pass4(x, fa, fb, fc, Q, mu32);
 #pragma unroll
@@ -982,10 +1035,10 @@
     Quarters,
     QuartersMfma,
 };
-template <int WPS_, bool AP_, bool FUSE_, Fwd FWD_>
+template <int WPS_, bool AP_, bool FUSE_, Fwd FWD_, bool XREG_ = true>
 struct LatVariant {
     static constexpr int LOGN = 10, DG = 4, WPS = WPS_;
-    static constexpr bool AP = AP_, FUSE = FUSE_, FOLD = FWD_ != Fwd::Rows;
+    static constexpr bool AP = AP_, FUSE = FUSE_, FOLD = FWD_ != Fwd::Rows, XREG = XREG_;
     static constexpr bool MFMA = FWD_ == Fwd::QuartersMfma, QUNITS = MFMA || FWD_ == Fwd::Quarters;
     static constexpr bool EVENF = QUNITS;
     static constexpr bool REGTW = WPS <= 2;
@@ -1009,7 +1062,7 @@
 __device__ __forceinline__ void lat_bootstrap(const PT& P, const bce_gate_desc g, const u32 soff, const u32 boot, u32* smem,
                                               u32* __restrict__ acc_out, u32* __restrict__ dbg_lweN, u32* __restrict__ dbg_ks) {
     constexpr int LOGN = V::LOGN, DG = V::DG, WPS = V::WPS;
-    constexpr bool AP = V::AP, FUSE = V::FUSE, FOLD = V::FOLD, QUNITS = V::QUNITS, MFMA = V::MFMA;
+    constexpr bool AP = V::AP, FUSE = V::FUSE, FOLD = V::FOLD, QUNITS = V::QUNITS, MFMA = V::MFMA, XREG = V::XREG;
     using C = Cfg<LOGN>;
     constexpr int N = C::N, NP = C::NP;
     constexpr u32 R = V::R, T = V::T, PR = V::PR, XB = LatLds::XB;
@@ -1053,7 +1106,8 @@
     u32 off = 0;
     for (u32 l = 0; l < (u32)DG; ++l) off |= 1u << (l * gb + gb - 1);
     const u32 offm = off - Q, bias = Q - (1u << (gb - 1));
-    const __amdgpu_buffer_rsrc_t mrsrc = __builtin_amdgcn_make_buffer_rsrc(const_cast<u32*>(P.fwd_mfma_tab), 0, MFMA ? 4 * 4 * 1024 : 0, 0x00020000);
+    const __amdgpu_buffer_rsrc_t mrsrc =
+        __builtin_amdgcn_make_buffer_rsrc(const_cast<u32*>(XREG ? P.fwd_mfma_tab_t : P.fwd_mfma_tab), 0, MFMA ? 4 * 4 * 1024 : 0, 0x00020000);
     const u32 psel0 = 0x0c0c0400u, psel1 = 0x05040100u;
     const u32 mc = tid / (N / 4), mp0 = (tid % (N / 4)) * 4, mpp = phys(mp0);
     const u32 dig0 = phys(S.t);
@@ -1106,7 +1160,7 @@
         };
         {
             u32 x[4], u[4];
-            split_inverse_rest(S, twf, xa, xb, Q, P.mu32, ninv, wlast, x, request_rows);
+            split_inverse_rest<XREG>(S, twf, xa, xb, Q, P.mu32, ninv, wlast, x, request_rows);
 #pragma unroll
             for (int r = 0; r < 4; ++r) u[r] = x[r] + ((x[r] < Qh) ? off : offm);
             if constexpr (MFMA) {
@@ -1140,7 +1194,7 @@
         if constexpr (WPS >= 4) { if (FOLD && wave >= 4) __builtin_amdgcn_s_setprio(1); else __builtin_amdgcn_s_setprio(0); }
 #ifndef BCE_SKIP_FWD
         if constexpr (QUNITS) {
-            ntt_forward_quarter3<MFMA>(dct + (2 + c) * NP + 272u * (wave & 3u), wave & 3u, q7, q6a, q6b, xbm + 3 * c * 256, mA,
+            ntt_forward_quarter3<MFMA, XREG>(dct + (2 + c) * NP + 272u * (wave & 3u), wave & 3u, q7, q6a, q6b, xbm + 3 * c * 256, mA,
                                        make_uint2(P.w14, P.w14s), twf, lane, Q);
         } else if constexpr (FOLD) {
             if (wave < 4) ntt_forward_wave_low8(dct + (2 + wave) * NP, twf, lane, Q);
@@ -1193,7 +1247,7 @@
     BCE_PROF_FLUSH();
     {
         u32 x[4];
-        split_inverse_rest(S, twf, xa, xb, Q, P.mu32, ninv, wlast, x, [](auto) {});
+        split_inverse_rest<XREG>(S, twf, xa, xb, Q, P.mu32, ninv, wlast, x, [](auto) {});
         if (acc_out) {
             u32* out = acc_out + ((size_t)boot * 2 + c) * N + S.t;
 #pragma unroll
@@ -1238,17 +1292,20 @@
     return (size_t)P.n + 1 <= 512 * VW && RW <= 8 && need <= LatLds::tail_bytes;
 }
 
-struct LatBuild { int wps; bool ap; Fwd fwd; };
-constexpr bool operator==(const LatBuild& a, const LatBuild& b) { return a.wps == b.wps && a.ap == b.ap && a.fwd == b.fwd; }
+struct LatBuild { int wps; bool ap; Fwd fwd; bool xreg = true; };
+constexpr bool operator==(const LatBuild& a, const LatBuild& b) { return a.wps == b.wps && a.ap == b.ap && a.fwd == b.fwd && a.xreg == b.xreg; }
 constexpr LatBuild kLatBuilds[] = {
     {2, false, Fwd::Rows}, {2, true, Fwd::Rows}, {2, false, Fwd::RowsAndHalves}, {2, true, Fwd::RowsAndHalves},
     {4, false, Fwd::Rows}, {4, true, Fwd::Rows}, {4, false, Fwd::RowsAndHalves}, {4, true, Fwd::RowsAndHalves},
     {4, false, Fwd::Quarters}, {4, false, Fwd::QuartersMfma},
+    {2, false, Fwd::RowsAndHalves, false}, {4, false, Fwd::QuartersMfma, false},
 };
+constexpr bool lat_headline(const LatBuild& b) { return !b.ap && (b.wps == 2 ? b.fwd == Fwd::RowsAndHalves : b.fwd == Fwd::QuartersMfma); }
 LatBuild lat_variant(const DevParams& P, bool x1) {
     const bool ap = P.method_ap != 0, quarters = P.fwd_units && !ap && !x1;
     const Fwd fwd = !P.fold ? Fwd::Rows : !quarters ? Fwd::RowsAndHalves : P.fwd_mfma ? Fwd::QuartersMfma : Fwd::Quarters;
-    return {x1 ? 2 : 4, ap, fwd};
+    const LatBuild b{x1 ? 2 : 4, ap, fwd};
+    return {b.wps, b.ap, b.fwd, P.xchg_regs != 0 || !lat_headline(b)};
 }
 size_t blind_rotate_lat_lds_bytes(const DevParams& P, const LatBuild& v) { return LatLds::bytes(v.fwd == Fwd::QuartersMfma, P.n); }
 template <size_t I = 0, class F>
@@ -1353,7 +1410,7 @@
     const LatBuild v = lat_variant(P, wps <= 2);
     const DagKernel k = lat_kernel(v, [](auto i) -> DagKernel {
         constexpr LatBuild b = kLatBuilds[i];
-        return k_bootstrap_dag<LatVariant<b.wps, b.ap, true, b.fwd>>;
+        return k_bootstrap_dag<LatVariant<b.wps, b.ap, true, b.fwd, b.xreg>>;
     });
     if (!k) return hipErrorInvalidValue;
     const size_t lds = blind_rotate_lat_lds_bytes(P, v) + kDagMailboxWords * 4;
@@ -1380,8 +1437,8 @@
         const bool fuse = !x1 && tail_fused && P.fuse_tail && fused_tail_fits(P);
         const LatKernel lk = lat_kernel(v, [fuse](auto i) -> LatKernel {
             constexpr LatBuild b = kLatBuilds[i];
-            if constexpr (b.wps >= 4) { if (fuse) return k_blind_rotate_lat<LatVariant<b.wps, b.ap, true, b.fwd>>; }
-            return k_blind_rotate_lat<LatVariant<b.wps, b.ap, false, b.fwd>>;
+            if constexpr (b.wps >= 4) { if (fuse) return k_blind_rotate_lat<LatVariant<b.wps, b.ap, true, b.fwd, b.xreg>>; }
+            return k_blind_rotate_lat<LatVariant<b.wps, b.ap, false, b.fwd, b.xreg>>;
         });
         if (!lk) return hipErrorInvalidValue;
         if (kernel_id) *kernel_id = x1 ? BCE_BR_SPLIT_X1 : BCE_BR_SPLIT_X2;
diff --git a/openfhe-boolean-circuit-evaluator_amd/csrc/kernels.hpp b/openfhe-boolean-circuit-evaluator_amd/csrc/kernels.hpp
--- a/openfhe-boolean-circuit-evaluator_amd/csrc/kernels.hpp
+++ b/openfhe-boolean-circuit-evaluator_amd/csrc/kernels.hpp
@@ -68,6 +68,8 @@
     u32 fwd_mfma;
     u32 w14, w14s;
     const u32* fwd_mfma_tab;
+    u32 xchg_regs;
+    const u32* fwd_mfma_tab_t;
 };
 
 constexpr size_t kLdsBytesPerCu = 160 * 1024;
```

Result: no change. 193,800 (median of 2 runs) (+0.1%).
